# nlamprian/ICP

Hardware: AMD Instinct MI355X
Metric: ICP iterations/sec at |F|=|M|=16384, |R|=256 (higher is better)
Workload: dtype f32

## Files before the change

### icp_amd/__init__.py

```python
import ctypes as C
import os

import numpy as np

__all__ = ["ICP", "ICPStep", "ICPError", "Memory", "Quality", "Pairs", "PAIR", "ErrorMetric", "Normals", "ICPStepConfigT", "ICPStepConfigW",
           "PowerMode", "ReduceMode", "TransformKind", "ICPBatch", "batch_partition", "power_method", "KernelObject", "kernel_lms", "kernel_reps", "kernel_weights", "kernel_mean", "kernel_devs", "kernel_s", "ReduceScan", "lib", "lib_path", "reduce", "scan", "ReduceConfig", "synth_pair", "synth_cloud_vga", "punch_holes", "HOLES_SCATTERED", "HOLES_CONTIGUOUS", "synth_pair_scene", "SCENE_CURVED", "SCENE_WALL", "device_count", "DIST_ID"]

_HERE = os.path.dirname(os.path.abspath(__file__))
_SO = os.environ.get("ICP_AMD_LIB", os.path.join(_HERE, "libicp_amd.so"))

DIST_ID = np.dtype([("dist", np.float32), ("id", np.uint32)])


class ICPError(RuntimeError):
    def __init__(self, code, msg):
        super().__init__("icp_amd error %d: %s" % (code, msg))
        self.code = code


class ICPStepConfigT:
    EIGEN = 0
    POWER_METHOD = 1


# ... 46 lines not shown
    QUATERNION = 0
    QUATERNION_2 = 1
    MATRIX = 2


class Memory:
    F, M, T, TK, MEANS, S, NN_ID, W, SUM_W, REPS, RBC_N, RBC_O, RBC_PERM, RBC_OWNER, RBC_XP, RID, R, RK, NN, QT, TRIM, \
        NORMALS_F, PLANE_SYSTEM, COLOR_GRAD_F, NORMALS_M, UNIQUE, PAIR_FILTER, RECIPROCAL, REVERSE_ID = range(29)
    D_IN_F, D_IN_M, D_IO_T, H_IO_T = F, M, T, T


class _State(C.Structure):
    _fields_ = [("R", C.c_float * 9), ("q", C.c_float * 4), ("t", C.c_float * 3), ("s", C.c_float),
                ("Rk", C.c_float * 9), ("qk", C.c_float * 4), ("tk", C.c_float * 3), ("sk", C.c_float),
                ("k", C.c_uint32), ("converged", C.c_uint32), ("power_iterations", C.c_uint32),
                ("reserved", C.c_uint32)]


class Quality(C.Structure):
    _fields_ = [("fitness", C.c_double), ("inlier_rmse", C.c_double), ("sum_geo", C.c_double), ("information", C.c_double * 36),
                ("n", C.c_uint32), ("n_moving", C.c_uint32), ("n_inliers", C.c_uint32), ("reserved", C.c_uint32)]

    def information_matrix(self):
        return np.array(self.information, np.float64).reshape(6, 6)


class Pairs:
    EVALUATED = 0
    LAST_ITERATION = 1


PAIR = np.dtype([("moving", "<u4"), ("fixed", "<u4"), ("geo", "<f4"), ("weight", "<f4")])


class _Pair(C.Structure):
    _fields_ = [("moving", C.c_uint32), ("fixed", C.c_uint32), ("geo", C.c_float), ("weight", C.c_float)]


_lib = None


def lib_path():
    return _SO


def lib():
    global _lib
    if _lib is not None:
        return _lib
    if not os.path.exists(_SO):
        raise ICPError(-1, "%s not found: build it with `make` (hipcc --offload-arch=gfx950); "
                           "there is no CPU fallback" % _SO)
    L = C.CDLL(_SO)
    vp, u32, i32, f32, f64 = C.c_void_p, C.c_uint32, C.c_int, C.c_float, C.c_double

    def sig(name, res, *args):
        f = getattr(L, name, None)
        if f is None:
            if "ICP_AMD_LIB" in os.environ:
                return
            raise AttributeError("%s does not export %s" % (_SO, name))
        f.restype = res
        f.argtypes = list(args)

    sig("icp_create", i32, C.POINTER(vp), i32, i32, i32)
    sig("icp_destroy", i32, vp)
    sig("icp_init", i32, vp, u32, u32, f32, f32, u32, f64, f64)
    sig("icp_init_batched", i32, vp, u32, u32, u32, f32, f32, u32, f64, f64)
    sig("icp_write", i32, vp, i32, vp, i32)
    sig("icp_write_b", i32, vp, u32, i32, vp, i32)
    sig("icp_read", i32, vp, i32, vp, C.c_size_t)
    sig("icp_read_b", i32, vp, u32, i32, vp, C.c_size_t)
    sig("icp_mem_size", C.c_size_t, vp, i32)
    sig("icp_device_ptr", i32, vp, i32, C.POINTER(vp))
    sig("icp_adopt_device_buffer", i32, vp, i32, vp)
    sig("icp_build_rbc", i32, vp)
    sig("icp_step", i32, vp, i32)
    sig("icp_run", i32, vp, C.POINTER(u32))
    sig("icp_run_stats", i32, vp, C.POINTER(u32), C.POINTER(u32), C.POINTER(u32))
    sig("icp_set_run_depth", i32, vp, u32, i32)
    sig("icp_run_timeline", i32, vp, C.POINTER(f64))
    sig("icp_set_output_mode", i32, vp, i32)
    sig("icp_launch_stats", i32, vp, C.POINTER(f64), C.POINTER(C.c_uint64), C.POINTER(C.c_uint64), i32)
    sig("icp_run_fixed", i32, vp, u32)
    sig("icp_run_fixed_fresh", i32, vp, u32)
    sig("icp_sync", i32, vp)
    sig("icp_get_alpha", i32, vp, C.POINTER(f32))
    sig("icp_set_alpha", i32, vp, f32)
    sig("icp_get_scaling", i32, vp, C.POINTER(f32))
    sig("icp_set_scaling", i32, vp, f32)
    sig("icp_set_metric_scale", i32, vp, f32)
    sig("icp_get_metric_scale", i32, vp, C.POINTER(f32))
    sig("icp_set_rejection", i32, vp, i32, f32)
    sig("icp_get_rejection", i32, vp, C.POINTER(i32), C.POINTER(f32))
    sig("icp_set_trimming", i32, vp, f32)
    sig("icp_get_trimming", i32, vp, C.POINTER(f32))
    sig("icp_set_unique", i32, vp, i32)
    sig("icp_get_unique", i32, vp, C.POINTER(i32))
    sig("icp_set_reciprocal", i32, vp, i32, C.c_float)
    sig("icp_get_reciprocal", i32, vp, C.POINTER(i32), C.POINTER(C.c_float))
    sig("icp_set_normal_rejection", i32, vp, i32, f32)
    sig("icp_get_normal_rejection", i32, vp, C.POINTER(i32), C.POINTER(f32))
    sig("icp_set_boundary_rejection", i32, vp, u32)
    sig("icp_get_boundary_rejection", i32, vp, C.POINTER(u32))
    sig("icp_set_robust_loss", i32, vp, i32, f32)
    sig("icp_get_robust_loss", i32, vp, C.POINTER(i32), C.POINTER(f32))
    sig("icp_set_error_metric", i32, vp, i32, f32)
    sig("icp_get_error_metric", i32, vp, C.POINTER(i32), C.POINTER(f32))
    sig("icp_set_normals", i32, vp, i32, u32)
    sig("icp_get_normals", i32, vp, C.POINTER(i32), C.POINTER(u32))
    sig("icp_set_color_weight", i32, vp, f32)
    sig("icp_get_color_weight", i32, vp, C.POINTER(f32))
    sig("icp_set_plane_to_plane", i32, vp, f32)
    sig("icp_get_plane_to_plane", i32, vp, C.POINTER(f32))
    sig("icp_set_symmetric", i32, vp, i32)
    sig("icp_get_symmetric", i32, vp, C.POINTER(i32))
    sig("icp_get_max_iterations", i32, vp, C.POINTER(u32))
    sig("icp_set_max_iterations", i32, vp, u32)
    sig("icp_get_angle_threshold", i32, vp, C.POINTER(f64))
    sig("icp_set_angle_threshold", i32, vp, f64)
    sig("icp_get_translation_threshold", i32, vp, C.POINTER(f64))
    sig("icp_set_translation_threshold", i32, vp, f64)
    sig("icp_set_power_mode", i32, vp, i32)
    sig("icp_set_reduce_mode", i32, vp, i32)
    sig("icp_state", i32, vp, C.POINTER(_State))
    sig("icp_state_b", i32, vp, u32, C.POINTER(_State))
    sig("icp_evaluate", i32, vp, f32, C.POINTER(Quality), u32)
    sig("icp_batch_evaluate", i32, vp, u32, f32, C.POINTER(Quality))
    sig("icp_correspondences", i32, vp, i32, f32, C.POINTER(u32), u32)
    sig("icp_correspondences_read", i32, vp, u32, vp, u32, C.POINTER(u32))
    sig("icp_correspondences_device_ptr", i32, vp, u32, C.POINTER(vp), C.POINTER(vp))
    sig("icp_batch_correspondences", i32, vp, u32, i32, f32, vp, u32, C.POINTER(u32))
    sig("icp_write_cloud", i32, vp, i32, vp, i32)
    sig("icp_transform_cloud", i32, vp, vp, vp, u32)
    sig("icp_transform_cloud_ex", i32, vp, i32, vp, vp, vp, u32)
    sig("icp_track_next", i32, vp, vp, i32, C.POINTER(u32), C.POINTER(i32))
    sig("icp_track_reset", i32, vp)
    sig("icp_track_form", i32, vp, C.POINTER(i32))
    sig("icp_track_submit", i32, vp, vp, i32)
    sig("icp_track_collect", i32, vp, C.POINTER(u32), vp, C.POINTER(i32))
    sig("icp_track_staging", i32, vp, u32, C.POINTER(vp))
    sig("icp_batch_create", i32, C.POINTER(vp), C.POINTER(i32), i32, i32, i32)
    sig("icp_batch_destroy", i32, vp)
    sig("icp_batch_init", i32, vp, u32, u32, u32, f32, f32, u32, f64, f64)
    sig("icp_batch_set_modes", i32, vp, i32, i32)
    sig("icp_batch_set_rejection", i32, vp, i32, f32)
    sig("icp_batch_set_trimming", i32, vp, f32)
    sig("icp_batch_set_unique", i32, vp, i32)
    sig("icp_batch_set_reciprocal", i32, vp, i32, C.c_float)
    sig("icp_batch_set_normal_rejection", i32, vp, i32, f32)
    sig("icp_batch_set_boundary_rejection", i32, vp, u32)
    sig("icp_batch_set_robust_loss", i32, vp, i32, f32)
    sig("icp_batch_set_error_metric", i32, vp, i32, f32)
    sig("icp_batch_set_normals", i32, vp, i32, u32)
    sig("icp_batch_set_color_weight", i32, vp, f32)
    sig("icp_batch_set_plane_to_plane", i32, vp, f32)
    sig("icp_batch_set_symmetric", i32, vp, i32)
    sig("icp_batch_write", i32, vp, u32, i32, vp)
    sig("icp_batch_build_rbc", i32, vp)
    sig("icp_batch_run", i32, vp)
    sig("icp_batch_run_fixed", i32, vp, u32, i32)
    sig("icp_batch_state", i32, vp, u32, C.POINTER(_State))
    sig("icp_batch_read", i32, vp, u32, i32, vp, C.c_size_t)
    sig("icp_batch_size", i32, vp, C.POINTER(u32), C.POINTER(u32))
    sig("icp_batch_time_run_fixed", i32, vp, u32, u32, C.POINTER(f64))
    sig("icp_batch_time_run_fixed_slots", i32, vp, u32, u32, u32, C.POINTER(f64), vp)
# ... 668 lines not shown
            for k, name in enumerate(("search", "means", "sij", "finalize")):
                c = t[:, k] * 1e3
                print(" %-10s %10.2f %10.2f %10.2f %10.3f" % (name, c.mean(), c.min(), c.max(), c.sum() / 1e3))
            s = t.sum(1) * 1e3
            print(" %-10s %10.2f %10.2f %10.2f %10.3f" % ("step", s.mean(), s.min(), s.max(), s.sum() / 1e3))
        return t, tot.value

    def time_kernels(self, reps):
        out = (C.c_float * 4)()
        self._chk(self._L.icp_time_kernels(self._h, reps, out))
        return dict(zip(("search", "means", "sij", "finalize"), [float(v) for v in out]))

    def state(self, batch_index=0):
        st = _State()
        self._chk(self._L.icp_state_b(self._h, batch_index, C.byref(st)))
        return st

    def evaluate(self, max_dist=0.0, count=None):
        n = self.batch if count is None else int(count)
        out = (Quality * max(n, 1))()
        self._chk(self._L.icp_evaluate(self._h, _max_dist_arg(max_dist), out, n))
        return list(out)[:n]

    def correspondences(self, source=Pairs.EVALUATED, max_dist=0.0, batch_index=0):
        counts = (C.c_uint32 * self.batch)()
        self._chk(self._L.icp_correspondences(self._h, source, _max_dist_arg(max_dist), counts, self.batch))
        return self.correspondences_read(batch_index)

    def correspondences_read(self, batch_index=0):
        n = C.c_uint32()
        rc = self._L.icp_correspondences_read(self._h, batch_index, None, 0, C.byref(n))
        if rc and not (rc == 1 and n.value):
            self._chk(rc)
        out = np.empty(n.value, PAIR)
        if n.value:
            self._chk(self._L.icp_correspondences_read(self._h, batch_index, _p(out), n.value, C.byref(n)))
        return out

    def _vec(self, name, shape=None):
        a = np.array(getattr(self.state(), name), dtype=np.float32)
        return a.reshape(shape) if shape else a

    R = property(lambda s: s._vec("R", (3, 3)))
    Rk = property(lambda s: s._vec("Rk", (3, 3)))
    q = property(lambda s: s._vec("q"))
    qk = property(lambda s: s._vec("qk"))
    t = property(lambda s: s._vec("t"))
    tk = property(lambda s: s._vec("tk"))
    s = property(lambda s: float(s.state().s))
    sk = property(lambda s: float(s.state().sk))
    k = property(lambda s: int(s.state().k))


class ICP(ICPStep):

    def init(self, m, nr, a=1e2, c=1e-6, max_iterations=40, angle_threshold=0.001,
             translation_threshold=0.01, batch=1):
        self._max_it, self._ang, self._tra = max_iterations, angle_threshold, translation_threshold
        super().init(m, nr, a, c, batch)

    def run(self):
        k = C.c_uint32()
        self._chk(self._L.icp_run(self._h, C.byref(k)))
        return k.value

    def step(self, config=False):
        ICPStep.run(self, config)

    def run_stats(self):
        n, k, d = C.c_uint32(), C.c_uint32(), C.c_uint32()
        self._chk(self._L.icp_run_stats(self._h, C.byref(n), C.byref(k), C.byref(d)))
        return n.value, k.value, d.value

    def run_timeline(self):
        t = (C.c_double * 6)()
        self._chk(self._L.icp_run_timeline(self._h, t))
        return [float(x) for x in t]

    def launch_stats(self, reset=False):
        mx, slow, tot = C.c_double(), C.c_uint64(), C.c_uint64()
        self._chk(self._L.icp_launch_stats(self._h, C.byref(mx), C.byref(slow), C.byref(tot), int(reset)))
        return mx.value, slow.value, tot.value

    def set_output_mode(self, every_iteration=False):
        self._chk(self._L.icp_set_output_mode(self._h, int(every_iteration)))

    def set_run_depth(self, depth=3, adaptive=True):
        self._chk(self._L.icp_set_run_depth(self._h, depth, int(adaptive)))

    def getMaxIterations(self):
        v = C.c_uint32()
        self._chk(self._L.icp_get_max_iterations(self._h, C.byref(v)))
        return v.value

    def setMaxIterations(self, n):
        self._chk(self._L.icp_set_max_iterations(self._h, n))
        self._max_it = n

    def getAngleThreshold(self):
        v = C.c_double()
        self._chk(self._L.icp_get_angle_threshold(self._h, C.byref(v)))
        return v.value

    def setAngleThreshold(self, deg):
        self._chk(self._L.icp_set_angle_threshold(self._h, deg))
        self._ang = deg

    def getTranslationThreshold(self):
        v = C.c_double()
        self._chk(self._L.icp_get_translation_threshold(self._h, C.byref(v)))
        return v.value

    def setTranslationThreshold(self, mm):
        self._chk(self._L.icp_set_translation_threshold(self._h, mm))
        self._tra = mm


def batch_partition(registrations, n_slots, i):
    slot, idx, cnt = C.c_uint32(), C.c_uint32(), C.c_uint32()
    rc = lib().icp_batch_partition(registrations, n_slots, i, C.byref(slot), C.byref(idx), C.byref(cnt))
    if rc:
        raise ICPError(rc, "icp_batch_partition: bad arguments")
    return slot.value, idx.value, cnt.value


class ICPBatch:

    def __init__(self, devices, CR=ICPStepConfigT.POWER_METHOD, CW=ICPStepConfigW.WEIGHTED):
        self._L = lib()
        self._b = C.c_void_p()
        devs = (C.c_int * len(devices))(*devices)
        rc = self._L.icp_batch_create(C.byref(self._b), devs, len(devices), CR, CW)
        if rc:
            msg = self._L.icp_batch_last_error(None).decode()
            self._b = None
            raise ICPError(rc, msg)
        self.m = 0

    def _chk(self, rc):
        if rc:
            raise ICPError(rc, self._L.icp_batch_last_error(self._b).decode())

    def slot_cpus(self, slot):
        buf = C.create_string_buffer(16384)
        self._chk(self._L.icp_batch_slot_cpus(self._b, slot, buf, len(buf)))
        return [int(x) for x in buf.value.decode().split(",") if x]

    def close(self):
        if getattr(self, "_b", None):
            self._L.icp_batch_destroy(self._b)
            self._b = None

    def __del__(self):
        try:
            self.close()
        except Exception:
            pass

    def init(self, registrations, m, nr, a=1e2, c=1e-6, max_iterations=40, angle_threshold=0.001, translation_threshold=0.01):
        self._chk(self._L.icp_batch_init(self._b, registrations, m, nr, a, c, max_iterations, angle_threshold, translation_threshold))
        self.m, self.registrations = m, registrations

    def set_modes(self, reduce_mode, power_mode):
        self._chk(self._L.icp_batch_set_modes(self._b, reduce_mode, power_mode))

    def set_rejection(self, invalid=False, max_dist=None):
# ... 264 lines not shown
```

### icp_amd/csrc/icp_build.hip

```cpp
#include "icp_kernels.h"

static __device__ __forceinline__ void state_restart (icp_reg_state *st) { st->k = 0; st->done = 0; st->pm_iters = 0; }
static __device__ __forceinline__ void state_rotation_from (icp_reg_state *st, const float *T) { float R[9]; icp_quat_to_rot (T, R); for (int i = 0; i < 9; ++i) st->R[i] = R[i]; }

__global__ void k_reset_state (icp_params p, int reset_T)
{
    uint32_t b = blockIdx.x * blockDim.x + threadIdx.x;
    if (b >= p.batch) return;
    icp_reg_state *st = p.st + b;
    if (reset_T) {
        const float T0[8] = { 0, 0, 0, 1, 0, 0, 0, 1 };
        const float I3[9] = { 1, 0, 0, 0, 1, 0, 0, 0, 1 };
        for (int i = 0; i < 8; ++i) { st->T[i] = T0[i]; st->Tk[i] = T0[i]; }
        for (int i = 0; i < 9; ++i) { st->R[i] = I3[i]; st->Rk[i] = I3[i]; }
        for (int i = 0; i < 11; ++i) st->S[i] = 0.f;
        for (int i = 0; i < 8; ++i) st->means[i] = 0.f;
        st->sum_w = 0.0;
    }
    state_restart (st);
}

__global__ void k_set_T (icp_reg_state *st, const float *T8, int reset_k)
{
    if (threadIdx.x != 0) return;
// ... 672 lines not shown
{
    if (threadIdx.x != 0) return;
    bool open = false;
    for (uint32_t spin = 0; spin < max_spins && !open; ++spin) {
        const uint32_t v = __hip_atomic_load (seq, __ATOMIC_ACQUIRE, __HIP_MEMORY_SCOPE_AGENT);
        open = (int32_t) (v - want) >= 0;
        if (!open) __builtin_amdgcn_s_sleep (8);
    }
    if (!open) {
        if (run_flag) *run_flag = epoch;
        if (flag) __hip_atomic_store (flag, 1u, __ATOMIC_RELAXED, __HIP_MEMORY_SCOPE_SYSTEM);
        return;
    }
    if (warm) {
        state_restart (warm);
        float T[4]; for (int i = 0; i < 4; ++i) T[i] = warm->T[i];
        state_rotation_from (warm, T);
    }
}

void icp_launch_gate (const uint32_t *seq, uint32_t want, uint32_t *host_timeout_flag, hipStream_t s, uint32_t max_spins, icp_reg_state *warm, uint32_t *run_flag, uint32_t epoch)
{
    hipLaunchKernelGGL (k_gate, dim3 (1), dim3 (64), 0, s, seq, want, host_timeout_flag, max_spins, warm, run_flag, epoch);
}

__global__ void k_seq_set (uint32_t *seq, uint32_t v) { if (threadIdx.x == 0) __hip_atomic_store (seq, v, __ATOMIC_RELEASE, __HIP_MEMORY_SCOPE_AGENT); }
void icp_launch_seq_set (uint32_t *seq, uint32_t v, hipStream_t s) { hipLaunchKernelGGL (k_seq_set, dim3 (1), dim3 (64), 0, s, seq, v); }

void icp_launch_get_lms (const float *cloud, float *lms, hipStream_t s)
{
    hipLaunchKernelGGL (k_get_lms, dim3 (16384 * 2 / 256), dim3 (256), 0, s,
                        reinterpret_cast<const float4 *> (cloud), reinterpret_cast<float4 *> (lms));
}

void icp_launch_get_lms_band (const float *band, float *lms, hipStream_t s)
{
    hipLaunchKernelGGL (k_get_lms_band, dim3 (16384 * 2 / 256), dim3 (256), 0, s,
                        reinterpret_cast<const float4 *> (band), reinterpret_cast<float4 *> (lms));
}

void icp_launch_transform_cloud (const float *in, float *out, const icp_reg_state *st, uint32_t n, hipStream_t s)
{
    hipLaunchKernelGGL (k_transform_cloud, dim3 ((n + 255) / 256), dim3 (256), 0, s,
                        reinterpret_cast<const float4 *> (in), reinterpret_cast<float4 *> (out), st, n);
}

void icp_launch_transform_cloud_ex (int kind, const float *in, float *out, const float *T, uint32_t n, hipStream_t s)
{
    icp_T16 t {};
    for (int i = 0; i < (kind == 2 ? 16 : 8); ++i) t.v[i] = T[i];
    const float4 *i4 = reinterpret_cast<const float4 *> (in); float4 *o4 = reinterpret_cast<float4 *> (out);
    const dim3 grid ((n + 255) / 256), block (256);
    if (kind == 0) hipLaunchKernelGGL (k_transform_cloud_ex<0>, grid, block, 0, s, i4, o4, t, n);
    else if (kind == 1) hipLaunchKernelGGL (k_transform_cloud_ex<1>, grid, block, 0, s, i4, o4, t, n);
    else hipLaunchKernelGGL (k_transform_cloud_ex<2>, grid, block, 0, s, i4, o4, t, n);
}

static void build_rbc_lists (const icp_params &p, hipStream_t s)
{
    if (icp_build_lists (p)) {
        icp_launch_owner_search (p, s);
        hipLaunchKernelGGL (k_place_lists, dim3 ((p.nb + 3u) / 4u, p.batch), dim3 (256), 0, s, p);
        hipLaunchKernelGGL (k_list_boxes, dim3 (p.nr, p.batch), dim3 (256), 0, s, p);
        return;
    }
    {
        const uint32_t nbr = (p.nr + 63u) / 64u, nbg = (p.n16 + 63u) / 64u, nbt = p.nr > p.tbox ? p.n1k : 0u;
        const uint32_t nblk = (nbr + nbg + nbt + (nbr <= ICP_ORIGIN_SOLO ? 1u : 0u)) * p.batch;
        uint32_t sort_cap = 0u;
        if (p.nr >= 256u && nblk <= 2048u) { sort_cap = 256u; while (sort_cap < p.nr && sort_cap < ICP_OL_SORT_MAX) sort_cap <<= 1; }
        hipLaunchKernelGGL (k_reps_and_boxes, dim3 (nbr + nbg + nbt + (nbr <= ICP_ORIGIN_SOLO ? 1u : 0u), p.batch), dim3 (64), sort_cap * 20u, s, p, nbr, nbg, sort_cap);
    }
    icp_launch_owner_search (p, s);
    hipLaunchKernelGGL (k_chunk_hist, dim3 (p.nchunk, p.batch), dim3 (256), p.nr * sizeof (uint32_t), s, p);
    if (p.nr <= 1024u) hipLaunchKernelGGL (k_count_offsets, dim3 (1, p.batch), dim3 (1024), 0, s, p);
    else {
        hipLaunchKernelGGL (k_count, dim3 ((p.nr + 63) / 64, p.batch), dim3 (1024), 0, s, p);
        hipLaunchKernelGGL (k_offsets, dim3 (1, p.batch), dim3 (1024), 0, s, p);
    }
    hipLaunchKernelGGL (k_place, dim3 (p.nchunk, p.batch), dim3 (1024), 0, s, p);
    hipLaunchKernelGGL (k_list_boxes, dim3 (p.nr, p.batch), dim3 (256), 0, s, p);
}

void icp_launch_build_rbc (const icp_params &p, hipStream_t s)
{
    build_rbc_lists (p, s);
    if (p.nrm_grid) icp_launch_normals_grid (p, s);
}
```

### icp_amd/csrc/icp_capi.hip

```cpp
#include "icp_host.h"

using namespace icp_host;

namespace {

void free_all (icp_context *h)
{
    drop_graphs (h);
    for (void *q : h->dev_allocs) (void) hipFree (q);
    h->dev_allocs.clear ();
    if (h->hF) (void) hipHostFree (h->hF);
    if (h->hM) (void) hipHostFree (h->hM);
    if (h->hT) (void) hipHostFree (h->hT);
    if (h->hState) (void) hipHostFree (h->hState);
    if (h->hMirror) (void) hipHostFree (h->hMirror);
    if (h->hTrackMirror) (void) hipHostFree (h->hTrackMirror);
    h->hState = nullptr; h->hMirror = h->hTrackMirror = nullptr; h->hstate_fresh = false;
    h->run = run_ctl {}; h->track_k_hist[0] = h->track_k_hist[1] = 0; h->track_hist_frame = 0;
    if (h->dCloud) (void) hipFree (h->dCloud);
    if (h->dCloudOut) (void) hipFree (h->dCloudOut);
    h->hF = h->hM = h->hT = nullptr; h->dCloud = h->dCloudOut = nullptr; h->cloud_cap = 0;
    h->dF = h->dM = nullptr; h->ownF = h->ownM = true;
    h->quality = icp_context::quality_buffers {};
    h->pairs = icp_context::pairs_buffers {};
// ... 228 lines not shown
    *out = h;
    return ICP_OK;
}
ICP_CATCH_ALL

int icp_destroy (icp_handle h) try
{
    if (!h) return ICP_EINVAL;
    keeper_stop (h);
    (void) hipSetDevice (h->device);
    if (h->run.active || h->run2.active) (void) run_close_all (h);
    if (h->stream2) (void) hipStreamSynchronize (h->stream2);
    if (h->copy_stream) (void) hipStreamSynchronize (h->copy_stream);
    if (h->stream) (void) hipStreamSynchronize (h->stream);
    free_all (h);
    if (h->dTin) (void) hipFree (h->dTin);
    if (h->ev0) (void) hipEventDestroy (h->ev0);
    if (h->ev1) (void) hipEventDestroy (h->ev1);
    for (int k = 0; k < 2; ++k) if (h->evUp[k]) (void) hipEventDestroy (h->evUp[k]);
    for (int k = 0; k < 2; ++k) if (h->evFrame[k]) (void) hipEventDestroy (h->evFrame[k]);
    for (int k = 0; k < 4; ++k) if (h->evDone[k]) (void) hipEventDestroy (h->evDone[k]);
    for (int k = 0; k < 3; ++k) if (h->evStage[k]) (void) hipEventDestroy (h->evStage[k]);
    if (h->copy_stream) (void) hipStreamDestroy (h->copy_stream);
    if (h->stream2) (void) hipStreamDestroy (h->stream2);
    if (h->stream) (void) hipStreamDestroy (h->stream);
    delete h;
    return ICP_OK;
}
ICP_CATCH_ALL

int icp_init_batched (icp_handle h, uint32_t batch, uint32_t m, uint32_t nr, float a, float c,
                      uint32_t max_iterations, double angle_threshold, double translation_threshold) try
{
    api_guard guard_ (h);
    if (!h) return ICP_EINVAL;
    if (m == 0) return fail (h, ICP_EINVAL, "The sets of landmarks cannot have zero points");
    if (nr == 0) return fail (h, ICP_EINVAL, "The sets of representatives cannot have zero points");
    if (a == 0.f) return fail (h, ICP_EINVAL, "The alpha parameter cannot be equal to zero");
    if (m % 2) return fail (h, ICP_EINVAL, "The number of points in the array must be a multiple of 2");
    if (batch == 0 || batch > 65535u) return fail (h, ICP_EINVAL, "batch must be in [1, 65535]");
    if (max_iterations == 0) return fail (h, ICP_EINVAL, "max_iterations must be positive");
    uint32_t nrx, nry, side;
    if (!reps_grid (m, nr, &nrx, &nry, &side))
        return fail (h, ICP_EINVAL, "nr must be a power of two whose grid tiles the sqrt(m) x sqrt(m) landmark grid");
    if (nr > 32768u) return fail (h, ICP_EINVAL, "nr must be <= 32768");
    if (m > (1u << 20)) return fail (h, ICP_EINVAL, "m must be <= 2^20");
    int rc = set_device (h); if (rc) return rc;
    if ((rc = run_close_all (h))) return rc;
    if (h->copy_stream) HIPCHK (h, hipStreamSynchronize (h->copy_stream));
    if (h->stream2) HIPCHK (h, hipStreamSynchronize (h->stream2));
    if (h->stream) HIPCHK (h, hipStreamSynchronize (h->stream));
    free_all (h);
    icp_params &p = h->p;
    p = icp_params {};
    derive_params (h->opt, p);
    p.check = 0; p.emit = 1;
    p.m = m; p.nr = nr; p.batch = batch; p.side = side; p.nrx = nrx; p.nry = nry;
    p.a = a; p.c = c;
    {
        auto magic = [] (uint32_t d) { return d > 1u ? (uint32_t) ((1ull << 32) / d + 1ull) : 0u; };
        p.side_magic = magic (side); p.cellw_magic = magic (side / nrx); p.cellh_magic = magic (side / nry);
    }
    h->max_iterations = max_iterations; h->angle_threshold = angle_threshold; h->translation_threshold = translation_threshold;
    p.tan_half_thr = std::tan (angle_threshold * M_PI / 360.0);
    p.trans_thr = translation_threshold;
    p.nwg = (m + 127u) / 128u;
    p.nwp = p.nwg; if (p.nwp != 1 && (p.nwp % 4)) p.nwp += 4 - p.nwp % 4;
    uint32_t n4 = m; if (n4 % 4) n4 += 4 - n4 % 4;
    p.G = n4 / 4;
    p.nsp = (p.G + 511u) / 512u; if (p.nsp != 1 && (p.nsp % 4)) p.nsp += 4 - p.nsp % 4;
    p.nchunk = (m + ICP_CHUNK - 1) / ICP_CHUNK;
    p.nb = (m + 63u) / 64u;
    { const uint32_t ng = (p.nb + 127u) / 128u; p.ng_magic = ng > 1u ? (uint32_t) ((1ull << 32) / ng + 1ull) : 0u; }

    const size_t B = batch;
    float *F = nullptr, *M = nullptr;
    if ((rc = dalloc (h, &F, B * m * 8))) return rc;
    if ((rc = dalloc (h, &M, B * m * 8))) return rc;
    h->dF = F; h->dM = M; p.F = F; p.M = M; h->lm[0] = F; h->lm[1] = M;
    p.n16 = (nr + 15u) / 16u;
    p.tbox = icp_tbox_of (p); p.n1k = (nr + p.tbox - 1u) / p.tbox;
    p.s2wave = icp_s2_wave_of (p);
    { const char *e = std::getenv ("ICP_AMD_XCDMAP"); p.xcdmap = e ? (e[0] == '1') : (B == 1u); }
    { const char *e = std::getenv ("ICP_AMD_WARM_SEED"); p.warm_seed = (e && e[0] == '1') ? 1u : 0u; }
    p.gtile = 0u;
    if (nrx % 4u == 0u && nry % 4u == 0u && !std::getenv ("ICP_AMD_STRIP_GROUPS")) { uint32_t lg = 0; while ((4u << lg) < nrx) ++lg; p.gtile = lg + 1u; }
    p.nlb = m / 16u + 2u;
    {
        icp_rbc_set s;
        if ((rc = icp_rbc_for_each (s, p, [&] (const char *, void **q, size_t bytes) { return dalloc (h, reinterpret_cast<char **> (q), bytes); }))) return rc;
        icp_rbc_into (p, s);
    }
    if ((rc = dalloc (h, &p.rid, B * m))) return rc;
    if ((rc = dalloc (h, &p.nn_id, B * m))) return rc;
    if ((rc = dalloc (h, &p.PF, B * m))) return rc;
    if ((rc = dalloc (h, &p.PM, B * m))) return rc;
    if ((rc = dalloc (h, &p.wpart, B * 2 * p.nwp))) return rc;
    if ((rc = dalloc (h, &p.mpart, B * 2 * p.nwg))) return rc;
    if ((rc = dalloc (h, &p.mscr, B * 2 * ((p.nwg + 127u) / 128u)))) return rc;
    if ((rc = dalloc (h, &p.spart, B * 11 * p.nsp * 8))) return rc;
    if ((rc = dalloc (h, &p.mom, icp_mom_layout_of (batch, m, p.nb).total))) return rc;
    if ((rc = write_words (h, OPT_WORDS))) return rc;
    HIPCHK (h, hipMemsetAsync (icp_unique_claims (p), 0xFF, sizeof (unsigned long long) * B * m, h->stream));
    if ((rc = dalloc (h, &p.ml1, B * 18 * ((p.nb + 127u) / 128u)))) return rc;
    if ((rc = dalloc (h, &p.cst, B * 2))) return rc;
    if ((rc = dalloc (h, &p.st, B))) return rc;
    if ((rc = dalloc (h, &p.st_prev, B))) return rc;
    if (!h->dTin) HIPCHK (h, hipMalloc ((void **) &h->dTin, 8 * sizeof (float)));
    HIPCHK (h, hipHostMalloc ((void **) &h->hF, B * m * 8 * sizeof (float), hipHostMallocDefault));
    HIPCHK (h, hipHostMalloc ((void **) &h->hM, B * m * 8 * sizeof (float), hipHostMallocDefault));
    HIPCHK (h, hipHostMalloc ((void **) &h->hT, 64 * sizeof (float), hipHostMallocDefault));
    HIPCHK (h, hipHostMalloc ((void **) &h->hState, B * sizeof (icp_reg_state), hipHostMallocMapped | hipHostMallocCoherent));
    HIPCHK (h, hipHostMalloc ((void **) &h->hMirror, B * sizeof (unsigned long long), hipHostMallocMapped | hipHostMallocCoherent));
    std::memset (h->hMirror, 0, B * sizeof (unsigned long long));
    icp_launch_reset_state (p, h->stream, 1);
    HIPCHK (h, hipGetLastError ());
    HIPCHK (h, hipStreamSynchronize (h->stream));
    h->inited = true; h->built = false;
    return ICP_OK;
}
ICP_CATCH_ALL

int icp_init (icp_handle h, uint32_t m, uint32_t nr, float a, float c, uint32_t max_iterations,
              double angle_threshold, double translation_threshold) try
{
    api_guard guard_ (h);
    return icp_init_batched (h, 1, m, nr, a, c, max_iterations, angle_threshold, translation_threshold);
}
ICP_CATCH_ALL

struct mem_desc { const void *ptr; size_t bytes; const char *plain_write; };
static mem_desc mem_of (const icp_context *h, uint32_t b, int mem)
{
    const icp_params &p = h->p;
    const size_t m = p.m, nr = p.nr;
    const char *st = reinterpret_cast<const char *> (p.st + b);
    switch (mem) {
        case ICP_MEM_F: return { h->dF + b * m * 8, m * 32, nullptr };
        case ICP_MEM_M: return { h->dM + b * m * 8, m * 32, nullptr };
        case ICP_MEM_RBC_XP: return { p.XP + b * m * 8, m * 32, nullptr };
        case ICP_MEM_T: return { st + offsetof (icp_reg_state, T), 32, nullptr };
        case ICP_MEM_TK: return { st + offsetof (icp_reg_state, Tk), 32, nullptr };
        case ICP_MEM_MEANS: return { st + offsetof (icp_reg_state, means), 32, nullptr };
        case ICP_MEM_S: return { st + offsetof (icp_reg_state, S), 44, nullptr };
        case ICP_MEM_SUM_W: return { st + offsetof (icp_reg_state, sum_w), 8, nullptr };
        case ICP_MEM_R: return { st + offsetof (icp_reg_state, R), 36, nullptr };
        case ICP_MEM_RK: return { st + offsetof (icp_reg_state, Rk), 36, nullptr };
        case ICP_MEM_NN_ID: return { p.nn_id + b * m, m * 8, nullptr };
        case ICP_MEM_RBC_PERM: return { p.perm + b * m, m * 4, nullptr };
        case ICP_MEM_RBC_OWNER: return { p.owner + b * m, m * 4, nullptr };
        case ICP_MEM_RID: return { p.rid + b * m, m * 4, nullptr };
        case ICP_MEM_REPS: return { p.R + b * nr * 8, nr * 32, nullptr };
        case ICP_MEM_RBC_N: return { ICP_N_FULL (p, b), nr * 4, nullptr };
        case ICP_MEM_RBC_O: return { p.O + b * nr, nr * 4, nullptr };
        case ICP_MEM_NN: return { p.PF + b * m, m * 16, nullptr };
        case ICP_MEM_QT: return { p.PM + b * m, m * 16, nullptr };
        case ICP_MEM_W: return { reinterpret_cast<const float *> (p.PF + b * m) + 3, m * 4, nullptr };
        case ICP_MEM_TRIM: return { icp_trim_area (p) + 4u * b, 16, nullptr };
        case ICP_MEM_UNIQUE: return { icp_unique_area (p) + 2u * b, 8, nullptr };
        case ICP_MEM_PAIR_FILTER: return { icp_pair_filter_area (p) + 4u * b, 16, nullptr };
        case ICP_MEM_RECIPROCAL: return { icp_reciprocal_area (p) + 4u * b, 16, nullptr };
        case ICP_MEM_REVERSE_ID: return { h->recip.nn_id ? h->recip.nn_id + b * m : nullptr, m * 8, nullptr };
        case ICP_MEM_NORMALS_F: return { icp_normals_f (p) + b * m, m * 16, "ICP_MEM_NORMALS_F" };
        case ICP_MEM_COLOR_GRAD_F: return { icp_color_grad_f (p) + b * m, m * 16, "ICP_MEM_COLOR_GRAD_F" };
        case ICP_MEM_NORMALS_M: return { icp_normals_m (p) + b * m, m * 16, "ICP_MEM_NORMALS_M" };
        case ICP_MEM_PLANE_SYSTEM: return { icp_p2pl_area (p) + (size_t) ICP_P2PL_SYS * b, ICP_P2PL_SYS * sizeof (double), nullptr };
        default: return { nullptr, 0, nullptr };
    }
}

int icp_write_b (icp_handle h, uint32_t b, int mem, const void *host_ptr, int block) try
{
    api_guard guard_ (h);
    int rc = need (h, false); if (rc) return rc;
    if (b >= h->p.batch) return fail (h, ICP_EINVAL, "batch index out of range");
    if ((rc = set_device (h))) return rc;
// ... 7 lines not shown
            note_inputs_change (h);
            HIPCHK (h, hipEventSynchronize (ev));
            if (host_ptr) std::memcpy (stage, host_ptr, fm);
            HIPCHK (h, hipMemcpyAsync (dst, stage, fm, hipMemcpyHostToDevice, h->stream));
            HIPCHK (h, hipEventRecord (ev, h->stream));
            if (mem == ICP_MEM_M) { normals_m_follow (h, b, 1u); HIPCHK (h, hipGetLastError ()); }
            break;
        }
        case ICP_MEM_T: {
            HIPCHK (h, hipEventSynchronize (h->evStage[2]));
            if (host_ptr) std::memcpy (h->hT, host_ptr, 8 * sizeof (float));
            HIPCHK (h, hipMemcpyAsync (h->dTin, h->hT, 8 * sizeof (float), hipMemcpyHostToDevice, h->stream));
            HIPCHK (h, hipEventRecord (h->evStage[2], h->stream));
            { const long long kb = h->k_base; note_enqueue (h); h->k_base = kb; }
            icp_launch_set_T (h->p, b, h->dTin, h->stream);
            HIPCHK (h, hipGetLastError ());
            break;
        }
        default: {
            const mem_desc d = mem_of (h, b, mem);
            if (!d.plain_write)
                return fail (h, ICP_EINVAL, "icp_write: mem must be ICP_MEM_F, ICP_MEM_M, ICP_MEM_T, ICP_MEM_NORMALS_F, ICP_MEM_COLOR_GRAD_F or ICP_MEM_NORMALS_M");
            if (!host_ptr) return fail (h, ICP_EINVAL, std::string ("icp_write: ") + d.plain_write + " needs a source");
            note_inputs_change (h);
            HIPCHK (h, hipStreamSynchronize (h->stream));
            HIPCHK (h, hipMemcpy (const_cast<void *> (d.ptr), host_ptr, d.bytes, hipMemcpyHostToDevice));
        }
    }
    if (block) HIPCHK (h, hipStreamSynchronize (h->stream));
    return ICP_OK;
}
ICP_CATCH_ALL

int icp_write (icp_handle h, int mem, const void *host_ptr, int block) try { api_guard guard_ (h); return icp_write_b (h, 0, mem, host_ptr, block); } ICP_CATCH_ALL

size_t icp_mem_size (icp_handle h, int mem) { return h && h->inited ? mem_of (h, 0, mem).bytes : 0; }

int icp_read_b (icp_handle h, uint32_t b, int mem, void *host_dst, size_t bytes) try
{
    api_guard guard_ (h);
    int rc = need (h, false); if (rc) return rc;
    if (!host_dst) return fail (h, ICP_EINVAL, "icp_read: null destination");
    if (b >= h->p.batch) return fail (h, ICP_EINVAL, "batch index out of range");
    const mem_desc d = mem_of (h, b, mem);
    if (!d.bytes) return fail (h, ICP_EINVAL, "unknown icp_mem value");
    if (bytes > d.bytes) return fail (h, ICP_EINVAL, "icp_read: more bytes requested than the object holds");
    if (!d.ptr) return fail (h, ICP_ESTATE, "icp_read: ICP_MEM_REVERSE_ID: no back search has run since icp_init (icp_set_reciprocal)");
    if ((rc = set_device (h))) return rc;
    const void *src = d.ptr;
    if ((rc = materialize_outputs (h, mem))) return rc;
    if (mem == ICP_MEM_W) {
        size_t rows = bytes / 4;
        HIPCHK (h, hipMemcpy2DAsync (host_dst, 4, src, 16, 4, rows, hipMemcpyDeviceToHost, h->stream));
    } else
        HIPCHK (h, hipMemcpyAsync (host_dst, src, bytes, hipMemcpyDeviceToHost, h->stream));
    HIPCHK (h, hipStreamSynchronize (h->stream));
    return ICP_OK;
}
ICP_CATCH_ALL

int icp_read (icp_handle h, int mem, void *host_dst, size_t bytes) try { api_guard guard_ (h); return icp_read_b (h, 0, mem, host_dst, bytes); } ICP_CATCH_ALL

int icp_device_ptr (icp_handle h, int mem, void **dptr) try
{
    api_guard guard_ (h);
    int rc = need (h, false); if (rc) return rc;
    if (!dptr) return fail (h, ICP_EINVAL, "null pointer");
    const mem_desc d = mem_of (h, 0, mem);
    if (!d.bytes) return fail (h, ICP_EINVAL, "unknown icp_mem value");
    if (!d.ptr) return fail (h, ICP_ESTATE, "icp_device_ptr: ICP_MEM_REVERSE_ID: no back search has run since icp_init (icp_set_reciprocal)");
    if ((rc = set_device (h))) return rc;
    if ((rc = materialize_outputs (h, mem))) return rc;
    *dptr = const_cast<void *> (d.ptr);
    return ICP_OK;
}
ICP_CATCH_ALL

int icp_adopt_device_buffer (icp_handle h, int mem, void *dptr) try
{
    api_guard guard_ (h);
    int rc = need (h, false); if (rc) return rc;
    if (!dptr) return fail (h, ICP_EINVAL, "null pointer");
    if (mem == ICP_MEM_F) { h->dF = static_cast<float *> (dptr); h->p.F = h->dF; h->ownF = false; h->built = false; }
    else if (mem == ICP_MEM_M) { h->dM = static_cast<float *> (dptr); h->p.M = h->dM; h->ownM = false; h->recip.stale = true; }
    else return fail (h, ICP_EINVAL, "only ICP_MEM_F and ICP_MEM_M can be adopted");
    note_inputs_change (h);
    drop_graphs (h);
    return ICP_OK;
}
ICP_CATCH_ALL

int icp_build_rbc (icp_handle h) try
{
    api_guard guard_ (h);
    int rc = need (h, false); if (rc) return rc;
    if ((rc = set_device (h))) return rc;
    if (h->p.nrm_grid && h->p.m % h->p.nrm_grid)
        return fail (h, ICP_ESTATE, "icp_build_rbc: ICP_NORMALS_GRID: m is not a multiple of the grid width");
    if (h->opt.boundary_gw && h->p.m % h->opt.boundary_gw)
        return fail (h, ICP_ESTATE, "icp_build_rbc: icp_set_boundary_rejection: m is not a multiple of the grid width");
    note_inputs_change (h);
    note_enqueue (h);
    icp_launch_build_rbc (h->p, h->stream);
    HIPCHK (h, hipGetLastError ());
    h->built = true; h->k_base = 0;
    if (icp_reciprocal (h->p)) { h->recip.stale = true; if ((rc = reciprocal_ready (h))) return rc; }
    return ICP_OK;
}
ICP_CATCH_ALL

int icp_step (icp_handle h, int config) try
{
    api_guard guard_ (h);
    (void) config;
    int rc = need (h, true); if (rc) return rc;
    if ((rc = set_device (h))) return rc;
    icp_params p = h->p; p.check = 0; p.hmirror = nullptr; p.hstate = nullptr;
    { const long long kb = h->k_base; note_enqueue (h); if (kb >= 0) h->k_base = kb + 1; }
    note_outputs_stored (h);
    icp_launch_iteration (p, h->stream, &h->recip);
    HIPCHK (h, hipGetLastError ());
    return ICP_OK;
}
ICP_CATCH_ALL

int icp_run_fixed (icp_handle h, uint32_t iterations) try
{
    api_guard guard_ (h);
    int rc = need (h, true); if (rc) return rc;
    if (iterations == 0) return ICP_OK;
    if ((rc = set_device (h))) return rc;
    return launch_run (h, iterations, 0);
}
ICP_CATCH_ALL

int icp_run_fixed_fresh (icp_handle h, uint32_t iterations) try
{
    api_guard guard_ (h);
    int rc = need (h, true); if (rc) return rc;
    if (iterations == 0) return icp_reset_transform (h);
    if ((rc = set_device (h))) return rc;
    return launch_run (h, iterations, 0, true);
}
ICP_CATCH_ALL

int icp_run (icp_handle h, uint32_t *k) try
{
    api_guard guard_ (h);
    int rc = need (h, true); if (rc) return rc;
    if ((rc = set_device (h))) return rc;
    if (!h->run_adaptive) {
        if ((rc = launch_run (h, h->max_iterations, 1))) return rc;
        if ((rc = settle (h))) return rc;
        h->stat_launches = h->max_iterations; h->stat_k = h->hState[0].k; h->stat_dead = 0;
    } else {
        if ((rc = run_begin (h, h->run, h->stream, h->p, false, false, h->run_depth + 1u, h->hMirror, h->hState, -1))) return rc;
        if ((rc = run_finish (h))) return rc;
        if ((rc = run_wait_final (h, h->hMirror, h->p.batch, h->run.p.epoch))) return rc;
        h->stat_t[5] = now_s ();
        h->hstate_fresh = true; h->hstate_here = true;
        if (h->p.batch == 1u) h->k_base = h->hState[0].k;
        {
            uint32_t kmax = 0u, all_done = 1u;
            for (uint32_t b = 0; b < h->p.batch; ++b) { kmax = std::max (kmax, h->hState[b].k); all_done &= h->hState[b].done ? 1u : 0u; }
            h->stat_k = kmax;
            const uint32_t ran = kmax > h->run.k0 ? kmax - h->run.k0 : 0u;
            h->stat_dead = all_done ? h->run.enq - std::min (h->run.enq, ran + 1u) : 0u;
        }
    }
    if (k) {
        if (h->hstate_fresh) *k = h->hState[0].k;
        else {
            icp_reg_state st;
            HIPCHK (h, hipMemcpy (&st, h->p.st, sizeof st, hipMemcpyDeviceToHost));
            *k = st.k;
        }
    }
    return ICP_OK;
}
ICP_CATCH_ALL

int icp_run_stats (icp_handle h, uint32_t *launches, uint32_t *k, uint32_t *dead) try
{
    api_guard guard_ (h);
    if (!h) return ICP_EINVAL;
    if (launches) *launches = h->stat_launches;
    if (k) *k = h->stat_k;
    if (dead) *dead = h->stat_dead;
    return ICP_OK;
}
ICP_CATCH_ALL

int icp_launch_stats (icp_handle h, double *max_us, uint64_t *slower_than_10us, uint64_t *total, int reset) try
{
    api_guard guard_ (h);
    if (!h) return ICP_EINVAL;
    if (max_us) *max_us = h->stat_launch_max_us;
    if (slower_than_10us) *slower_than_10us = h->stat_launch_slow;
    if (total) *total = h->stat_launch_total;
    if (reset) { h->stat_launch_max_us = 0.0; h->stat_launch_slow = h->stat_launch_total = 0; }
    return ICP_OK;
}
ICP_CATCH_ALL

int icp_set_output_mode (icp_handle h, int mode) try
{
    api_guard guard_ (h);
    if (!h) return ICP_EINVAL;
    if (mode != ICP_OUTPUTS_LAZY && mode != ICP_OUTPUTS_EVERY_ITERATION) return fail (h, ICP_EINVAL, "unknown output mode");
    h->outputs_lazy = mode == ICP_OUTPUTS_LAZY;
    return ICP_OK;
}
ICP_CATCH_ALL

int icp_run_timeline (icp_handle h, double *us6) try
{
    api_guard guard_ (h);
    if (!h || !us6) return ICP_EINVAL;
    for (int i = 0; i < 6; ++i) us6[i] = (h->stat_t[i] - h->stat_t[0]) * 1e6;
    return ICP_OK;
}
ICP_CATCH_ALL

int icp_set_run_depth (icp_handle h, uint32_t depth, int adaptive) try
{
    api_guard guard_ (h);
    if (!h) return ICP_EINVAL;
    if (depth == 0 || depth > 64u) return fail (h, ICP_EINVAL, "icp_set_run_depth: depth must be in [1, 64]");
    { int rc = set_device (h); if (rc) return rc; if ((rc = run_close_all (h))) return rc; }
    h->run_depth = depth; h->run_adaptive = adaptive ? 1 : 0;
    return ICP_OK;
}
ICP_CATCH_ALL

int icp_sync (icp_handle h) try
{
    api_guard guard_ (h);
    if (!h) return ICP_EINVAL;
    int rc = set_device (h); if (rc) return rc;
    return settle (h);
}
ICP_CATCH_ALL

int icp_get_alpha (icp_handle h, float *a) try { api_guard guard_ (h); if (!h || !a) return ICP_EINVAL; *a = h->p.a; return ICP_OK; } ICP_CATCH_ALL
int icp_set_alpha (icp_handle h, float a) try
{
    api_guard guard_ (h);
    if (!h) return ICP_EINVAL;
    if (a == 0.f) return fail (h, ICP_EINVAL, "The alpha parameter cannot be equal to zero");
    { int rc = outputs_before_change (h); if (rc) return rc; }
    h->p.a = a; ++h->param_gen; return ICP_OK;
}
ICP_CATCH_ALL
int icp_set_metric_scale (icp_handle h, float f_g) try
{
    api_guard guard_ (h);
    if (!h) return ICP_EINVAL;
    if (!(f_g > 0.f) || !std::isfinite (f_g)) return fail (h, ICP_EINVAL, "the metric scale must be positive and finite");
    { int rc = outputs_before_change (h); if (rc) return rc; }
    h->opt.metric_scale = f_g;
    return commit (h, OPT_PARAMS);
}
ICP_CATCH_ALL
int icp_get_metric_scale (icp_handle h, float *f_g) try { api_guard guard_ (h); if (!h || !f_g) return ICP_EINVAL; *f_g = h->opt.metric_scale; return ICP_OK; } ICP_CATCH_ALL
int icp_set_rejection (icp_handle h, int flags, float max_dist) try
{
    api_guard guard_ (h);
    if (flags & ~reject_user_flags) return fail (h, ICP_EINVAL, "icp_set_rejection: unknown flag bits");
    if (!(max_dist >= 0.f)) return fail (h, ICP_EINVAL, "icp_set_rejection: max_dist must be >= 0 (0 or +inf: no distance test)");
    if (!h) return fail (h, ICP_EINVAL, "icp_set_rejection: null handle");
    { int rc = outputs_before_change (h); if (rc) return rc; }
    h->opt.reject_flags = flags; h->opt.reject_max_dist = max_dist;
    return commit (h, OPT_PARAMS);
}
ICP_CATCH_ALL
int icp_get_rejection (icp_handle h, int *flags, float *max_dist) try
{
    api_guard guard_ (h);
    if (!h) return ICP_EINVAL;
    if (flags) *flags = h->opt.reject_flags;
    if (max_dist) *max_dist = h->opt.reject_max_dist;
    return ICP_OK;
}
ICP_CATCH_ALL
int icp_set_trimming (icp_handle h, float keep_fraction) try
{
    api_guard guard_ (h);
// ... 233 lines not shown
    if (!h) return ICP_EINVAL;
    h->angle_threshold = d; h->p.tan_half_thr = std::tan (d * M_PI / 360.0); ++h->param_gen; return ICP_OK;
}
ICP_CATCH_ALL
int icp_get_translation_threshold (icp_handle h, double *d) try { api_guard guard_ (h); if (!h || !d) return ICP_EINVAL; *d = h->translation_threshold; return ICP_OK; } ICP_CATCH_ALL
int icp_set_translation_threshold (icp_handle h, double d) try
{
    api_guard guard_ (h);
    if (!h) return ICP_EINVAL;
    h->translation_threshold = d; h->p.trans_thr = d; ++h->param_gen; return ICP_OK;
}
ICP_CATCH_ALL
int icp_set_power_mode (icp_handle h, int mode) try
{
    api_guard guard_ (h);
    if (!h) return ICP_EINVAL;
    if (mode != ICP_POWER_LITERAL && mode != ICP_POWER_SQUARED) return fail (h, ICP_EINVAL, "unknown power mode");
    h->opt.power_mode = mode;
    return commit (h, OPT_PARAMS);
}
ICP_CATCH_ALL

int icp_set_reduce_mode (icp_handle h, int mode) try
{
    api_guard guard_ (h);
    if (!h) return ICP_EINVAL;
    if (mode != ICP_REDUCE_REFERENCE_ORDER && mode != ICP_REDUCE_FUSED) return fail (h, ICP_EINVAL, "unknown reduce mode");
    { int rc = outputs_before_change (h); if (rc) return rc; }
    h->opt.reduce_mode = mode;
    return commit (h, OPT_ROUTE);
}
ICP_CATCH_ALL

int icp_state_b (icp_handle h, uint32_t b, icp_state_t *out) try
{
    api_guard guard_ (h);
    int rc = need (h, false); if (rc) return rc;
    if (!out) return fail (h, ICP_EINVAL, "null pointer");
    if (b >= h->p.batch) return fail (h, ICP_EINVAL, "batch index out of range");
    if ((rc = set_device (h))) return rc;
    icp_reg_state st;
    if (h->hstate_fresh) {
        if (!h->hstate_here) HIPCHK (h, hipStreamSynchronize (h->stream));
        st = h->hState[b];
    } else {
        HIPCHK (h, hipMemcpyAsync (&st, h->p.st + b, sizeof st, hipMemcpyDeviceToHost, h->stream));
        HIPCHK (h, hipStreamSynchronize (h->stream));
    }
    std::memcpy (out->R, st.R, sizeof st.R); std::memcpy (out->Rk, st.Rk, sizeof st.Rk);
    std::memcpy (out->q, st.T, 16); std::memcpy (out->t, st.T + 4, 12); out->s = st.T[7];
    std::memcpy (out->qk, st.Tk, 16); std::memcpy (out->tk, st.Tk + 4, 12); out->sk = st.Tk[7];
    out->k = st.k; out->converged = st.done; out->power_iterations = st.pm_iters; out->reserved = 0;
    return ICP_OK;
}
ICP_CATCH_ALL

int icp_state (icp_handle h, icp_state_t *out) try { api_guard guard_ (h); return icp_state_b (h, 0, out); } ICP_CATCH_ALL

static int evaluation_ready (icp_context *h, const char *who, uint32_t count)
{
    const std::string w (who);
    if (count == 0) return fail (h, ICP_EINVAL, w + ": count must be at least 1");
    int rc = need (h, false); if (rc) return rc;
    if (count > h->p.batch) return fail (h, ICP_EINVAL, w + ": count is above the handle's batch");
    if (h->track_submitted) return fail (h, ICP_ESTATE, w + ": the handle has tracked frames (the quality of tracked frames is not provided): icp_init or icp_track_reset first");
    if (!h->built) return fail (h, ICP_ESTATE, "icp_build_rbc has not been called");
    return set_device (h);
}

static int evaluation_search (icp_context *h)
{
    const icp_params &p = h->p;
    const size_t n = (size_t) p.batch * p.m;
    icp_context::quality_buffers &Q = h->quality;
    int rc;
    if (!Q.nn_id && (rc = dalloc (h, &Q.nn_id, n))) return rc;
    if (!Q.PF && (rc = dalloc (h, &Q.PF, n))) return rc;
    if (!Q.PM && (rc = dalloc (h, &Q.PM, n))) return rc;
    if (!Q.rid && (rc = dalloc (h, &Q.rid, n))) return rc;
    icp_params q = p;
    q.check = 0; q.emit = 1; q.fused = 0; q.weighted = 0; q.hmirror = nullptr; q.hstate = nullptr; q.dbg = nullptr;
    q.reject = 0u; q.reject_d2 = 0.f; q.reject_max_dist = 0.f; q.trim_keep = 0.f; q.metric = ICP_METRIC_POINT_TO_POINT; q.p2pl_mu = 0.f; q.gicp = 0u;
    q.nn_id = Q.nn_id; q.PF = Q.PF; q.PM = Q.PM; q.rid = Q.rid;
    if (icp_dense (q)) HIPCHK (h, hipMemcpyAsync (Q.rid, p.rid, n * sizeof (uint32_t), hipMemcpyDeviceToDevice, h->stream));
    icp_launch_search (q, h->stream);
    return ICP_OK;
}

int icp_evaluate (icp_handle h, float max_dist, icp_quality_t *out, uint32_t count) try
{
    api_guard guard_ (h);
    if (!h) return ICP_EINVAL;
    if (!out) return fail (h, ICP_EINVAL, "icp_evaluate: null output");
    if (!(max_dist >= 0.f)) return fail (h, ICP_EINVAL, "icp_evaluate: max_dist must be >= 0 (0 or +inf: no distance test)");
    int rc = evaluation_ready (h, "icp_evaluate", count); if (rc) return rc;
    const icp_params &p = h->p;
    const size_t B = p.batch, nblk = icp_p2pl_nblk (p.m);
    icp_context::quality_buffers &Q = h->quality;
    if ((rc = evaluation_search (h))) return rc;
    if (!Q.part && (rc = dalloc (h, &Q.part, B * ICP_QUALITY_TERMS * nblk))) return rc;
    if (!Q.cnt && (rc = dalloc (h, &Q.cnt, B * 2 * nblk))) return rc;
    if (!Q.res && (rc = dalloc (h, &Q.res, B * ICP_QUALITY_RES))) return rc;
    const bool dist_on = max_dist > 0.f && !std::isinf (max_dist);
    icp_launch_quality (Q.PF, Q.PM, p.M, p.m, p.batch, dist_on, dist_on ? (float) ((double) max_dist * (double) max_dist) : 0.f, Q.part, Q.cnt, Q.res, h->stream);
    HIPCHK (h, hipGetLastError ());
    std::vector<double> res (B * ICP_QUALITY_RES);
    HIPCHK (h, hipMemcpyAsync (res.data (), Q.res, res.size () * sizeof (double), hipMemcpyDeviceToHost, h->stream));
    HIPCHK (h, hipStreamSynchronize (h->stream));
    for (uint32_t b = 0; b < count; ++b) {
        const double *r = res.data () + (size_t) b * ICP_QUALITY_RES;
        icp_quality_t &o = out[b];
        uint32_t c[2];
        std::memcpy (c, r + ICP_QUALITY_TERMS, sizeof c);
        o.n = p.m; o.n_moving = c[0]; o.n_inliers = c[1]; o.reserved = 0u;
        o.sum_geo = r[21];
        o.fitness = c[0] ? (double) c[1] / (double) c[0] : 0.0;
        o.inlier_rmse = c[1] ? std::sqrt (r[21] / (double) c[1]) : 0.0;
        int t = 0;
        for (int a = 0; a < 6; ++a)
            for (int cc = a; cc < 6; ++cc, ++t) { o.information[a * 6 + cc] = r[t]; o.information[cc * 6 + a] = r[t]; }
    }
    return ICP_OK;
}
ICP_CATCH_ALL

int icp_correspondences (icp_handle h, int source, float max_dist, uint32_t *counts, uint32_t count) try
{
    api_guard guard_ (h);
    if (!h) return ICP_EINVAL;
    if (source != ICP_PAIRS_EVALUATED && source != ICP_PAIRS_LAST_ITERATION) return fail (h, ICP_EINVAL, "icp_correspondences: unknown source");
    if (!counts) return fail (h, ICP_EINVAL, "icp_correspondences: null counts");
    if (!(max_dist >= 0.f)) return fail (h, ICP_EINVAL, "icp_correspondences: max_dist must be >= 0 (0 or +inf: no distance test)");
    if (source == ICP_PAIRS_LAST_ITERATION && max_dist != 0.f)
        return fail (h, ICP_EINVAL, "icp_correspondences: ICP_PAIRS_LAST_ITERATION takes the pairs the iteration used: max_dist must be 0");
    int rc = evaluation_ready (h, "icp_correspondences", count); if (rc) return rc;
    const icp_params &p = h->p;
    const size_t B = p.batch;
    icp_context::pairs_buffers &P = h->pairs;
    static_assert (sizeof (icp_pair_t) == sizeof (uint4) && sizeof (icp_pair_t) == 16, "a record is one 16-byte store");
    if (source == ICP_PAIRS_LAST_ITERATION && (rc = materialize_outputs (h, ICP_MEM_W))) return rc;
    if (!P.blk && (rc = dalloc (h, &P.blk, B * icp_p2pl_nblk (p.m)))) return rc;
    if (!P.rec && (rc = dalloc (h, &P.rec, B * p.m))) return rc;
    if (!P.count && (rc = dalloc (h, &P.count, B))) return rc;
    P.valid = false;
    if (source == ICP_PAIRS_EVALUATED) {
        if ((rc = evaluation_search (h))) return rc;
        const icp_context::quality_buffers &Q = h->quality;
        const bool dist_on = max_dist > 0.f && !std::isinf (max_dist);
        icp_launch_pairs (source, Q.PF, Q.PM, p.M, Q.nn_id, p.m, p.batch, dist_on, dist_on ? (float) ((double) max_dist * (double) max_dist) : 0.f, P.blk, P.rec, P.count, h->stream);
    } else
        icp_launch_pairs (source, p.PF, p.PM, nullptr, p.nn_id, p.m, p.batch, false, 0.f, P.blk, P.rec, P.count, h->stream);
    HIPCHK (h, hipGetLastError ());
    P.n.assign (B, 0u);
    HIPCHK (h, hipMemcpyAsync (P.n.data (), P.count, B * sizeof (uint32_t), hipMemcpyDeviceToHost, h->stream));
    HIPCHK (h, hipStreamSynchronize (h->stream));
    for (uint32_t b = 0; b < count; ++b) counts[b] = P.n[b];
    P.valid = true;
    return ICP_OK;
}
ICP_CATCH_ALL

int icp_correspondences_read (icp_handle h, uint32_t b, icp_pair_t *host_dst, uint32_t capacity, uint32_t *n) try
{
    api_guard guard_ (h);
    int rc = need (h, false); if (rc) return rc;
    if (b >= h->p.batch) return fail (h, ICP_EINVAL, "batch index out of range");
// ... 288 lines not shown
```

### icp_amd/csrc/icp_host.h

```cpp
#pragma once

#include "../../include/icp_amd.h"
#include "icp_kernels.h"
#include "icp_rbc_set.h"
#include "icp_cguard.h"

#include <atomic>
#include <thread>
#include <mutex>
#include <condition_variable>
#include <chrono>
#include <cmath>
#include <cstdio>
#include <cstdlib>
#include <cstring>
#include <map>
#include <string>
#include <vector>
#include <immintrin.h>

namespace icp_host __attribute__ ((visibility ("hidden"))) {

inline thread_local std::string g_create_error;

// ... 8 lines not shown
    bool end_enqueued = false;
    volatile unsigned long long *mirror = nullptr;
    int track_slot = -1;
    hipStream_t stream = nullptr;
    double t[5] = { 0, 0, 0, 0, 0 };
    double launch_max_us = 0.0; uint32_t launch_slow = 0;
};

struct track_keeper {
    std::thread th;
    std::mutex mx;
    std::condition_variable cv;
    std::atomic<int> state { 0 };
    std::atomic<bool> pause { false }, quit { false };
    bool started = false;
    std::thread::id tid;
    int rc = 0; std::string err;
};
constexpr int ICP_KEEPER_ABORTED = -77;

inline double now_s () { return std::chrono::duration<double> (std::chrono::steady_clock::now ().time_since_epoch ()).count (); }

struct icp_options {
    int rot = ICP_ROT_POWER_METHOD, weighted = 1, power_mode = ICP_POWER_SQUARED, reduce_mode = ICP_REDUCE_FUSED;
    int chain = 1;
    float metric_scale = 1.f;
    int reject_flags = 0; float reject_max_dist = 0.f;
    float trim_keep = 1.f;
    bool unique = false;
    bool reciprocal = false; float reciprocal_gap = 0.f;
    bool normal_on = false; float normal_min_cos = 0.f;
    uint32_t boundary_gw = 0;
    int robust = ICP_ROBUST_NONE; float robust_scale = 0.f;
    int metric = ICP_METRIC_POINT_TO_POINT; float p2pl_mu = 0.f;
    float color_kappa = 0.f;
    float gicp_eps = 0.f;
    bool symmetric = false;
    uint32_t nrm_grid = 0;
};

}

struct icp_context {
    int device = 0;
    hipStream_t stream = nullptr;
    bool inited = false, built = false;
    icp_params p {};
    uint32_t max_iterations = 40;
    double angle_threshold = 0.001, translation_threshold = 0.01;
    std::string err;
    std::vector<void *> dev_allocs;
    float *dF = nullptr, *dM = nullptr;
    bool ownF = true, ownM = true;
    float *hF = nullptr, *hM = nullptr, *hT = nullptr;
    icp_reg_state *hState = nullptr;
    bool hstate_fresh = false;
    bool hstate_here = false;
    unsigned long long *hMirror = nullptr;
    uint32_t epoch = 0;
    long long k_base = 0;
    uint32_t run_depth = 3;
    int run_adaptive = 1;
    icp_host::run_ctl run;
    icp_host::run_ctl run2;
    int api_depth = 0;
    icp_host::track_keeper *keeper = nullptr;
    int outputs_lazy = 1;
    bool outputs_stale = false, outputs_lost = false;
    uint32_t stat_launches = 0, stat_k = 0, stat_dead = 0;
    double stat_t[6] = { 0, 0, 0, 0, 0, 0 };
    double stat_launch_max_us = 0.0; uint64_t stat_launch_slow = 0, stat_launch_total = 0;
    icp_host::icp_options opt;
    uint64_t graph_clock = 0, param_gen = 0;
    float *dTin = nullptr;
    struct quality_buffers {
        icp_dist_id *nn_id = nullptr; float4 *PF = nullptr, *PM = nullptr; uint32_t *rid = nullptr;
        double *part = nullptr; uint32_t *cnt = nullptr; double *res = nullptr;
    } quality;
    struct pairs_buffers {
        uint32_t *blk = nullptr; uint4 *rec = nullptr; uint32_t *count = nullptr;
        std::vector<uint32_t> n; bool valid = false;
    } pairs;
    icp_reciprocal_set recip;
    float *dCloud = nullptr, *dCloudOut = nullptr; uint32_t cloud_cap = 0;
    std::map<uint64_t, icp_host::graph_entry> graphs;
    uint32_t parity = 0;
    float *lm[3] = { nullptr, nullptr, nullptr };
    float *hBand[2] = { nullptr, nullptr }, *dBand[2] = { nullptr, nullptr };
    float *hFrame[2] = { nullptr, nullptr };
    struct host_range { const char *base; size_t bytes; };
    std::vector<host_range> sources;
    icp_reg_state *hTrack = nullptr;
    unsigned long long *hTrackMirror = nullptr;
    uint32_t track_epoch[4] = { 0, 0, 0, 0 };
    uint32_t track_k_hist[2] = { 0, 0 };
    uint64_t track_hist_frame = 0;
    hipStream_t copy_stream = nullptr;
    hipStream_t stream2 = nullptr;
    int track_gate = 1;
    uint32_t *dSeq = nullptr, *dRunFlag = nullptr, *hGateFlag = nullptr;
    bool stream2_dirty = false;
    icp_rbc_set rbc[2];
    bool rbc2_ready = false;
    bool track_last_gated = false;
    hipEvent_t evUp[2] = { nullptr, nullptr }, evDone[4] = { nullptr, nullptr, nullptr, nullptr };
    hipEvent_t evFrame[2] = { nullptr, nullptr };
    hipEvent_t evStage[3] = { nullptr, nullptr, nullptr };
    uint64_t track_submitted = 0, track_collected = 0;
    hipEvent_t ev0 = nullptr, ev1 = nullptr;
};

namespace icp_host __attribute__ ((visibility ("hidden"))) {

inline int fail (icp_context *h, int code, const std::string &msg)
{
    if (h) h->err = msg; else g_create_error = msg;
    return code;
}

#define HIPCHK(h, expr)                                                                         \
    do {                                                                                        \
        hipError_t e_ = (expr);                                                                 \
        if (e_ != hipSuccess)                                                                   \
            return fail ((h), ICP_EHIP, std::string (#expr) + ": " + hipGetErrorString (e_));   \
    } while (0)

template <typename T>
int dalloc (icp_context *h, T **ptr, size_t count, bool zero = true)
{
    void *q = nullptr;
    size_t bytes = (count ? count : 1) * sizeof (T);
    hipError_t e = hipMalloc (&q, bytes);
    if (e != hipSuccess) return fail (h, ICP_ENOMEM, std::string ("hipMalloc: ") + hipGetErrorString (e));
    h->dev_allocs.push_back (q);
    if (zero) {
        e = hipMemsetAsync (q, 0, bytes, h->stream);
        if (e != hipSuccess) return fail (h, ICP_EHIP, std::string ("hipMemsetAsync: ") + hipGetErrorString (e));
    }
    *ptr = static_cast<T *> (q);
    return ICP_OK;
}

void drop_graphs (icp_context *h);
int need (icp_context *h, bool built, bool keep_run = false);
int set_device (icp_context *h);
int get_graph (icp_context *h, uint32_t iterations, int check, hipGraphExec_t *out, bool fresh = false, bool with_build = false);
void run_launch_one (icp_context *h, run_ctl &r);
void run_enqueue_end (icp_context *h, run_ctl &r);
bool run_pump (icp_context *h, run_ctl &r);
int run_finish (icp_context *h, run_ctl &r, run_ctl *other);
inline int run_finish (icp_context *h) { return run_finish (h, h->run, h->run2.active ? &h->run2 : nullptr); }
int run_wait_final (icp_context *h, volatile unsigned long long *mirror, uint32_t n, uint32_t epoch, bool tracked = false);
int run_close_all (icp_context *h);
inline bool on_keeper_thread (const icp_context *h) { return h->keeper && h->keeper->started && std::this_thread::get_id () == h->keeper->tid; }
void keeper_quiesce (icp_context *h);
void keeper_kick (icp_context *h);
void keeper_stop (icp_context *h);
struct api_guard {
    icp_context *h;
    explicit api_guard (icp_context *h_) : h (h_) { if (h && h->api_depth++ == 0 && h->keeper) keeper_quiesce (h); }
    ~api_guard () { if (h && --h->api_depth == 0 && h->keeper) keeper_kick (h); }
    api_guard (const api_guard &) = delete; api_guard &operator= (const api_guard &) = delete;
};
int launch_run (icp_context *h, uint32_t iterations, int check, bool fresh = false, bool with_build = false);
int settle (icp_context *h);
void note_enqueue (icp_context *h);
void note_inputs_change (icp_context *h);
void note_outputs_stored (icp_context *h);
int materialize_outputs (icp_context *h, int mem);
void normals_m_follow (icp_context *h, uint32_t b0, uint32_t nb);
int reciprocal_ready (icp_context *h);

template <typename Fn>
int capture_graph (icp_context *h, Fn &&launches, graph_entry *out, bool instantiate = true)
{
    graph_entry ge;
    HIPCHK (h, hipStreamBeginCapture (h->stream, hipStreamCaptureModeThreadLocal));
    launches ();
    const hipError_t le = hipGetLastError ();
    hipError_t e = hipStreamEndCapture (h->stream, &ge.graph);
    if (e == hipSuccess && le != hipSuccess) e = le;
    if (e != hipSuccess) {
        if (ge.graph) (void) hipGraphDestroy (ge.graph);
        return fail (h, ICP_EHIP, std::string ("graph capture: ") + hipGetErrorString (e));
    }
    if (instantiate) {
        e = hipGraphInstantiate (&ge.exec, ge.graph, nullptr, nullptr, 0);
        if (e != hipSuccess) {
            (void) hipGraphDestroy (ge.graph);
            return fail (h, ICP_EHIP, std::string ("hipGraphInstantiate: ") + hipGetErrorString (e));
        }
    }
    *out = ge;
    return ICP_OK;
}

struct run_no_hook { int operator() () const { return ICP_OK; } };
template <typename BETWEEN = run_no_hook>
int run_begin (icp_context *h, run_ctl &r, hipStream_t stream, const icp_params &p, bool fresh, bool with_build, uint32_t blind,
               unsigned long long *mirror, icp_reg_state *hstate, int track_slot, BETWEEN between = BETWEEN (), run_ctl *other = nullptr)
{
    r = run_ctl {};
    r.stream = stream;
    r.t[0] = now_s ();
    r.p = p; r.p.check = 1;
    const icp_route route = icp_route_of (p);
    r.p.emit = (h->outputs_lazy && p.fused && !route.stored) ? 0 : 1;
    h->outputs_stale = r.p.emit == 0; h->outputs_lost = false;
    if (++h->epoch == 0u) h->epoch = 1u;
    r.p.epoch = h->epoch; r.p.hmirror = mirror; r.p.hstate = hstate;
    r.mirror = mirror; r.track_slot = track_slot;
    for (uint32_t b = 0; b < p.batch; ++b) mirror[b] = 0ull;
    std::atomic_thread_fence (std::memory_order_seq_cst);
    r.chained = route.chained; r.fresh = fresh;
    r.k0 = (fresh || with_build || h->k_base < 0) ? 0u : (uint32_t) h->k_base;
    r.maxit = h->max_iterations; r.depth = h->run_depth ? h->run_depth : 1u;
    if (other && other->active) (void) run_pump (h, *other);
    if (with_build) icp_launch_build_rbc (r.p, r.stream);
    if (other && other->active) (void) run_pump (h, *other);
    { int rc = between (); if (rc) return rc; }
    if (fresh && !r.chained) icp_launch_reset_state (r.p, r.stream, 1);
    r.active = true;
    const uint32_t n = std::min (std::max (blind, 1u), r.maxit);
    while (r.enq < n) {
        run_launch_one (h, r);
        if (other && other->active && (r.enq & 1u) == 0u) (void) run_pump (h, *other);
    }
    if (r.enq >= r.maxit) { r.decided = true; r.k_final = r.maxit + r.k0; run_enqueue_end (h, r); }
    HIPCHK (h, hipGetLastError ());
    h->hstate_fresh = false; h->hstate_here = false; h->k_base = -1;
    r.t[1] = now_s ();
    return ICP_OK;
}

}
```

### icp_amd/csrc/icp_kernels.h

```cpp
#pragma once
#include <hip/hip_runtime.h>
#include <stdint.h>
#include "icp_device.h"
#include "icp_search_select.h"

#ifndef ICP_L1_MIN_GROUPS
#define ICP_L1_MIN_GROUPS 2u
#endif
#define ICP_BAND_ROW0 49u
#define ICP_BAND_ROW_STEP 3u
#define ICP_BAND_ROWS 128u
#define ICP_BAND_COL0 65u
#define ICP_BAND_COLS 509u
#define ICP_BAND_ROW_BYTES (ICP_BAND_COLS * 32u)
#define ICP_BAND_BYTES ((size_t) ICP_BAND_ROWS * ICP_BAND_ROW_BYTES)
#define ICP_TBOX 1024u
#ifndef ICP_OL_BOXED_MIN
#define ICP_OL_BOXED_MIN 128u
#endif
#define ICP_OL_MASKS(nr) ((nr) + 1u + 2u * (((nr) + 7u) / 8u))
#define ICP_OL_STRIDE(nr) (ICP_OL_MASKS (nr) + ((nr) + 127u) / 128u)
#define ICP_CHUNK 1024u

struct icp_params {
    uint32_t m, nr, batch;
    uint32_t side, nrx, nry;
    uint32_t ng_magic;
    uint32_t side_magic, cellw_magic, cellh_magic;
    float a, c;
    float dist_scale;
    int weighted, rot, power_mode, check;
    int chain;
    int fused;
    int emit;
    double tan_half_thr, trans_thr;
    uint32_t nwg;
    uint32_t nwp;
    uint32_t G;
    uint32_t nsp;
    uint32_t nchunk;
    uint32_t nb;
    const float *F, *M;
    float *R;
    float4 *GB;
    uint32_t n16, n1k;
    uint32_t tbox;
    uint32_t gtile;
    uint32_t xcdmap;
    uint32_t warm_seed;
    uint32_t s2wave;
    uint32_t nrm_grid;
    float *XP;
    float *XQ;
    float4 *OL;
    float4 *LB;
    uint32_t nlb;
    uint32_t metric;
    uint32_t *rep_src, *owner, *N, *O, *perm, *chunk_hist;
    uint2 *blist; uint32_t *bn; uint8_t *brank;
    uint32_t *rid;
    icp_dist_id *nn_id;
    float4 *PF, *PM;
    float *wpart;
    float4 *mpart;
    float4 *mscr;
    float *spart;
    double *mom;
    double *ml1;
    icp_reg_state *cst;
    uint32_t slot;
    float p2pl_mu;
    icp_reg_state *st;
    icp_reg_state *st_prev;
    unsigned long long *dbg;
    unsigned long long *hmirror;
    icp_reg_state *hstate;
    uint32_t epoch;
    uint32_t gicp;
    uint32_t *run_flag;
    uint32_t *track_seq;
    uint32_t seq_value;
    uint32_t no_state_reset;
    uint32_t reject;
    float reject_d2;
    float reject_max_dist;
    float trim_keep;
};
#define ICP_REJECT_DIST_ON 0x80000000u
#define ICP_REJECT_TRIM_ON 0x40000000u
#define ICP_REJECT_ROBUST_SHIFT 28u
#define ICP_REJECT_ROBUST_MASK 0x30000000u
#define ICP_REJECT_UNIQUE_ON 0x08000000u
#define ICP_REJECT_BOUNDARY_ON 0x04000000u
#define ICP_REJECT_NORMAL_ON 0x02000000u
#define ICP_REJECT_FILTER_MASK (ICP_REJECT_BOUNDARY_ON | ICP_REJECT_NORMAL_ON)
#define ICP_REJECT_RECIPROCAL_ON 0x01000000u
static_assert (sizeof (icp_params) == 480, "icp_params grew: the hidden kernel arguments of every kernel would move");

static __host__ __device__ __forceinline__ bool icp_rejecting (const icp_params &p) { return p.reject != 0u; }
static __host__ __device__ __forceinline__ bool icp_trimming (const icp_params &p) { return (p.reject & ICP_REJECT_TRIM_ON) != 0u; }
static __host__ __device__ __forceinline__ bool icp_unique (const icp_params &p) { return (p.reject & ICP_REJECT_UNIQUE_ON) != 0u; }
static __host__ __device__ __forceinline__ bool icp_pair_filter (const icp_params &p) { return (p.reject & ICP_REJECT_FILTER_MASK) != 0u; }
static __host__ __device__ __forceinline__ bool icp_reciprocal (const icp_params &p) { return (p.reject & ICP_REJECT_RECIPROCAL_ON) != 0u; }
static __host__ __device__ __forceinline__ bool icp_moving_normals (const icp_params &p) { return p.gicp != 0u || (p.reject & ICP_REJECT_NORMAL_ON) != 0u; }
static __host__ __device__ __forceinline__ uint32_t icp_robust (const icp_params &p) { return (p.reject & ICP_REJECT_ROBUST_MASK) >> ICP_REJECT_ROBUST_SHIFT; }
static __host__ __device__ __forceinline__ double icp_robust_omega (uint32_t loss, double u)
{
    if (u != u) return 0.0;
    if (loss == 1u) return u <= 1.0 ? 1.0 : 1.0 / sqrt (u);
    if (loss == 2u) return 1.0 / (1.0 + u);
    return u < 1.0 ? (1.0 - u) * (1.0 - u) : 0.0;
}
#define ICP_TRIM_ONE_BLOCK_MAX 16384u
#define ICP_TRIM_BINS 2048u

#define ICP_P2PL_BLOCK 256u
#define ICP_P2PL_TERMS 27u
#define ICP_P2PL_SYS 28u
#define ICP_METRIC_COLORED_ 2u
static __host__ __device__ __forceinline__ bool icp_p2pl (const icp_params &p) { return p.metric != 0u; }
static __host__ __device__ __forceinline__ bool icp_colored (const icp_params &p) { return p.metric == ICP_METRIC_COLORED_; }
static __host__ __device__ __forceinline__ bool icp_gicp (const icp_params &p) { return p.gicp == 1u && p.metric == 1u; }
#define ICP_MOVING_NORMALS_SYM 2u
static __host__ __device__ __forceinline__ bool icp_sym (const icp_params &p) { return p.gicp == ICP_MOVING_NORMALS_SYM && p.metric == 1u; }
static __host__ __device__ __forceinline__ uint32_t icp_p2pl_nblk (uint32_t m) { return (m + ICP_P2PL_BLOCK - 1u) / ICP_P2PL_BLOCK; }

#define ICP_QUALITY_TERMS 22u
#define ICP_QUALITY_RES 24u

struct icp_mom_layout {
    size_t trim;
    size_t sys;
    size_t part;
    size_t kappa;
    size_t robust;
    size_t gicp;
    size_t uniq;
    size_t filt;
    size_t recip;
    size_t total;
};
static __host__ __device__ inline icp_mom_layout icp_mom_layout_of (uint32_t batch, uint32_t m, uint32_t nb)
{
    const size_t B = batch, trim_words = B * (8u + ICP_TRIM_BINS) + (m > ICP_TRIM_ONE_BLOCK_MAX ? B * m : 0u);
    icp_mom_layout l;
    l.trim = B * 2 * 18 * nb;
    l.sys = l.trim + (trim_words + 1u) / 2u;
    l.part = l.sys + B * ICP_P2PL_SYS;
    l.kappa = l.part + B * ICP_P2PL_TERMS * icp_p2pl_nblk (m);
    l.robust = l.kappa + 1u;
    l.gicp = l.robust + 1u;
    l.uniq = l.gicp + 1u;
    l.filt = l.uniq + B + B * m;
    l.recip = l.filt + 6u * B + 1u;
    l.total = l.recip + 2u * B + 1u;
    return l;
}
static __host__ __device__ inline icp_mom_layout icp_mom_layout_of (const icp_params &p) { return icp_mom_layout_of (p.batch, p.m, p.nb); }
static inline uint32_t *icp_trim_area (const icp_params &p) { return reinterpret_cast<uint32_t *> (p.mom + icp_mom_layout_of (p).trim); }
static inline double *icp_p2pl_area (const icp_params &p) { return p.mom + icp_mom_layout_of (p).sys; }
static inline double *icp_p2pl_part (const icp_params &p) { return p.mom + icp_mom_layout_of (p).part; }
static inline float *icp_color_kappa (const icp_params &p) { return reinterpret_cast<float *> (p.mom + icp_mom_layout_of (p).kappa); }
static __host__ __device__ inline float *icp_robust_scale (const icp_params &p) { return reinterpret_cast<float *> (p.mom + icp_mom_layout_of (p).robust); }
static __host__ __device__ inline float *icp_gicp_eps (const icp_params &p) { return reinterpret_cast<float *> (p.mom + icp_mom_layout_of (p).gicp); }
static inline uint32_t *icp_unique_area (const icp_params &p) { return reinterpret_cast<uint32_t *> (p.mom + icp_mom_layout_of (p).uniq); }
static inline unsigned long long *icp_unique_claims (const icp_params &p)
{
    return reinterpret_cast<unsigned long long *> (p.mom + icp_mom_layout_of (p).uniq + (size_t) p.batch);
}
static inline uint32_t *icp_pair_filter_area (const icp_params &p) { return reinterpret_cast<uint32_t *> (p.mom + icp_mom_layout_of (p).filt); }
static inline uint32_t *icp_pair_filter_counts (const icp_params &p) { return icp_pair_filter_area (p) + 4u * (size_t) p.batch; }
static inline uint32_t *icp_pair_filter_settings (const icp_params &p) { return icp_pair_filter_area (p) + 12u * (size_t) p.batch; }
static inline uint32_t *icp_reciprocal_area (const icp_params &p) { return reinterpret_cast<uint32_t *> (p.mom + icp_mom_layout_of (p).recip); }
static inline uint32_t *icp_reciprocal_gap (const icp_params &p) { return icp_reciprocal_area (p) + 4u * (size_t) p.batch; }

struct icp_xp_layout {
    size_t normals, color_grad, normals_m, total;
};
static __host__ __device__ __forceinline__ icp_xp_layout icp_xp_layout_of (uint32_t batch, uint32_t m)
{
    const size_t n = (size_t) batch * m;
    return { n * 8, n * 12, n * 16, n * 20 };
}
static __host__ __device__ __forceinline__ float4 *icp_normals_f (const icp_params &p)
{
    return reinterpret_cast<float4 *> (p.XP + icp_xp_layout_of (p.batch, p.m).normals);
}
static __host__ __device__ __forceinline__ float4 *icp_color_grad_f (const icp_params &p)
{
    return reinterpret_cast<float4 *> (p.XP + icp_xp_layout_of (p.batch, p.m).color_grad);
}
static __host__ __device__ __forceinline__ float4 *icp_normals_m (const icp_params &p)
{
    return reinterpret_cast<float4 *> (p.XP + icp_xp_layout_of (p.batch, p.m).normals_m);
}

#define ICP_N_FULL(p, b) ((p).N + ((size_t) (p).batch + (b)) * (p).nr)

#define ICP_MIRROR_FINAL (1ull << 30)
#define ICP_MIRROR_DONE (1ull << 31)
#define ICP_MIRROR_WORD(epoch, k, done) (((unsigned long long) (epoch) << 32) | ((done) ? ICP_MIRROR_DONE : 0ull) | (unsigned long long) ((k) & 0xFFFFFFu))

static __device__ __forceinline__ uint32_t rep_src_index (const icp_params &p, uint32_t r)
{
    uint32_t gX = r % p.nrx, gY = r / p.nrx;
    uint32_t stepX = p.side / p.nrx, stepY = p.side / p.nry;
    uint32_t xi = (stepX == 1) ? gX : gX * stepX + (stepX >> 1) - 1;
    uint32_t yi = (stepY == 1) ? gY : gY * stepY + (stepY >> 1) - 1;
    return yi * p.side + xi;
}

struct rep_src_map {
    uint32_t nrx, side, stepX, stepY, offX, offY, lgx;
    __device__ __forceinline__ explicit rep_src_map (const icp_params &p)
        : nrx (p.nrx), side (p.side), stepX (p.side / p.nrx), stepY (p.side / p.nry), lgx (31u - (uint32_t) __builtin_clz (p.nrx | 1u))
    {
        offX = (stepX == 1u) ? 0u : (stepX >> 1) - 1u; offY = (stepY == 1u) ? 0u : (stepY >> 1) - 1u;
    }
    __device__ __forceinline__ uint32_t operator() (uint32_t r) const
    {
        return ((r >> lgx) * stepY + offY) * side + (r & (nrx - 1u)) * stepX + offX;
    }
};


static __device__ __forceinline__ uint32_t icp_other_kind_near (const unsigned long long *MK, uint32_t nr, uint32_t r, bool r_at_origin, uint32_t fallback)
{
    const uint32_t nw = (nr + 63u) / 64u, w = r >> 6, l = r & 63u;
    auto other = [&] (uint32_t ww) -> unsigned long long {
        const uint32_t left = nr - 64u * ww;
        const unsigned long long m = MK[ww];
        return (r_at_origin ? ~m : m) & (left < 64u ? (1ull << left) - 1ull : ~0ull);
    };
    const unsigned long long o = other (w), below = o & ((1ull << l) - 1ull), above = l < 63u ? o & ~((2ull << l) - 1ull) : 0ull;
    uint32_t best_d = 0xFFFFFFFFu, best = fallback;
    if (below) { const uint32_t q = 63u - (uint32_t) __builtin_clzll (below); best_d = l - q; best = 64u * w + q; }
    if (above) { const uint32_t q = (uint32_t) __builtin_ctzll (above); if (q - l < best_d) { best_d = q - l; best = 64u * w + q; } }
    if (best_d != 0xFFFFFFFFu) return best;
    for (uint32_t d = 1; d <= 4u; ++d) {
        if (w >= d) { const unsigned long long ol = other (w - d); if (ol) return 64u * (w - d) + 63u - (uint32_t) __builtin_clzll (ol); }
        if (w + d < nw) { const unsigned long long orr = other (w + d); if (orr) return 64u * (w + d) + (uint32_t) __builtin_ctzll (orr); }
    }
    return fallback;
}

enum icp_apply_kind { ICP_APPLY_NONE = 0, ICP_APPLY_PLAIN, ICP_APPLY_ROBUST };
enum icp_tail_kind { ICP_TAIL_FUSED = 0, ICP_TAIL_FUSED_L1, ICP_TAIL_REFERENCE, ICP_TAIL_PLANE };
struct icp_route {
    bool chained;
    bool stored;
    bool ref_search;
    bool filter;
    bool reciprocal;
    bool unique;
    uint32_t select;
    icp_apply_kind apply;
    icp_tail_kind tail;
    uint32_t launches;
};
icp_route icp_route_of (const icp_params &p);

void icp_launch_build_rbc (const icp_params &p, hipStream_t s);
void icp_launch_search (const icp_params &p, hipStream_t s);
struct icp_reciprocal_set;
void icp_launch_iteration (const icp_params &p, hipStream_t s, const icp_reciprocal_set *rs = nullptr);
void icp_launch_masked (const icp_params &p, hipStream_t s, unsigned mask, const icp_reciprocal_set *rs = nullptr);
void icp_launch_chain (const icp_params &p, hipStream_t s, uint32_t iterations, bool fresh = false);
void icp_launch_chain_one (const icp_params &p, hipStream_t s, uint32_t j, bool fresh, bool emit);
void icp_launch_chain_end (const icp_params &p, hipStream_t s, uint32_t launches);
void icp_launch_publish_state (const icp_params &p, hipStream_t s);
bool icp_build_lists (const icp_params &p);
bool icp_dense (const icp_params &p);
uint32_t icp_dense_tile (const icp_params &p);
void icp_launch_owner_search (const icp_params &p, hipStream_t s);
void icp_launch_search_dense (const icp_params &p, hipStream_t s);
void icp_launch_search_rej (const icp_params &p, hipStream_t s);
void icp_launch_chain_one_rej (const icp_params &p, hipStream_t s, uint32_t j, bool fresh, bool emit);
void icp_launch_trim_select (const icp_params &p, hipStream_t s, uint32_t launches);
void icp_launch_trim_apply (const icp_params &p, hipStream_t s);
void icp_launch_unique (const icp_params &p, hipStream_t s);
void icp_launch_reciprocal (const icp_params &p, hipStream_t s, const icp_reciprocal_set *rs);
void icp_launch_reciprocal_build (const icp_params &p, hipStream_t s, const icp_reciprocal_set &rs);
void icp_launch_pair_filter (const icp_params &p, hipStream_t s);
void icp_launch_robust_apply (const icp_params &p, hipStream_t s);
void icp_launch_plane_moments_robust (const icp_params &p, hipStream_t s, double *part, uint32_t nblk);
void icp_launch_p2pl_solve (const icp_params &p, hipStream_t s);
void icp_launch_normals_grid (const icp_params &p, hipStream_t s);
void icp_launch_normals_m (const icp_params &p, hipStream_t s, uint32_t b0, uint32_t nb);
void icp_launch_gicp_moments (const icp_params &p, hipStream_t s, double *part, uint32_t nblk);
void icp_launch_sym_moments (const icp_params &p, hipStream_t s, double *part, uint32_t nblk);
void icp_launch_owner_search_dense (const icp_params &p, hipStream_t s);
void icp_launch_quality (const float4 *PF, const float4 *PM, const float *M, uint32_t m, uint32_t batch, bool dist_on, float d2, double *part, uint32_t *cnt,
                         double *res, hipStream_t s);
void icp_launch_pairs (int source, const float4 *PF, const float4 *PM, const float *M, const icp_dist_id *nn_id, uint32_t m, uint32_t batch, bool dist_on, float d2,
                       uint32_t *blk_cnt, uint4 *pairs, uint32_t *count, hipStream_t s);
uint32_t icp_tbox_of (const icp_params &p);
uint32_t icp_s2_wave_of (const icp_params &p);
void icp_search_layout_of (const icp_params &p, int *dense, int *tile, int *stage2);
void icp_launch_reset_state (const icp_params &p, hipStream_t s, int reset_T);
void icp_launch_set_T (const icp_params &p, uint32_t b, const float *dT8, hipStream_t s, int reset_k = 0);
void icp_launch_gate (const uint32_t *seq, uint32_t want, uint32_t *host_timeout_flag, hipStream_t s, uint32_t max_spins = 1u << 21, icp_reg_state *warm = nullptr,
                      uint32_t *run_flag = nullptr, uint32_t epoch = 0u);
void icp_launch_seq_set (uint32_t *seq, uint32_t v, hipStream_t s);
void icp_launch_rotation_solver (int rot, int power_mode, const float *din19, float *dout18, hipStream_t s);
void icp_launch_get_lms (const float *cloud, float *lms, hipStream_t s);
void icp_launch_get_lms_band (const float *band, float *lms, hipStream_t s);
void icp_launch_transform_cloud (const float *in, float *out, const icp_reg_state *st, uint32_t n, hipStream_t s);
void icp_launch_transform_cloud_ex (int kind, const float *in, float *out, const float *T, uint32_t n, hipStream_t s);
```

### icp_amd/csrc/icp_reciprocal.hip

```cpp
#include "icp_rbc_set.h"
#include <cstdio>
#include <cstdlib>

namespace {

constexpr uint32_t RECIPROCAL_BLOCK = 256u;

#define RECIPROCAL_GUARD reserved1

__global__ __launch_bounds__ (64) void k_reciprocal_state (icp_params p, icp_reg_state *rst, uint32_t *result)
{
    const uint32_t b = blockIdx.x, t = threadIdx.x;
    const icp_reg_state *st = p.st + b;
    icp_reg_state *out = rst + b;
    constexpr uint32_t T0 = offsetof (icp_reg_state, T) / 4u, G0 = offsetof (icp_reg_state, RECIPROCAL_GUARD) / 4u;
    if (t < sizeof (icp_reg_state) / 4u && !(t >= T0 && t < T0 + 8u) && t != G0)
        reinterpret_cast<uint32_t *> (out)[t] = reinterpret_cast<const uint32_t *> (st)[t];
    if (t != 0u) return;
    if (!(p.check && st->done)) { uint32_t *w = result + 4u * b; w[0] = 0u; w[1] = 0u; w[2] = 0u; w[3] = 0u; }
    const double x = (double) st->T[0], y = (double) st->T[1], z = (double) st->T[2], w = (double) st->T[3];
    const double tx = (double) st->T[4], ty = (double) st->T[5], tz = (double) st->T[6];
    const float s = st->T[7];
    const double xx = x * x, yy = y * y, zz = z * z, xy = x * y, xz = x * z, yz = y * z, wx = w * x, wy = w * y, wz = w * z;
    const double R00 = 1.0 - 2.0 * (yy + zz), R01 = 2.0 * (xy - wz), R02 = 2.0 * (xz + wy);
    const double R10 = 2.0 * (xy + wz), R11 = 1.0 - 2.0 * (xx + zz), R12 = 2.0 * (yz - wx);
    const double R20 = 2.0 * (xz - wy), R21 = 2.0 * (yz + wx), R22 = 1.0 - 2.0 * (xx + yy);
    const double si = 1.0 / (double) s;
    const double u0 = (R00 * tx + R10 * ty) + R20 * tz, u1 = (R01 * tx + R11 * ty) + R21 * tz, u2 = (R02 * tx + R12 * ty) + R22 * tz;
    float Ti[8] = { -st->T[0], -st->T[1], -st->T[2], st->T[3], (float) -(u0 * si), (float) -(u1 * si), (float) -(u2 * si), (float) si };
    bool ok = isfinite (s) && s > 0.f;
#pragma unroll
    for (int k = 0; k < 8; ++k) ok = ok && isfinite (Ti[k]);
    if (!ok) { Ti[0] = Ti[1] = Ti[2] = 0.f; Ti[3] = 1.f; Ti[4] = Ti[5] = Ti[6] = 0.f; Ti[7] = 1.f; }
#pragma unroll
    for (int k = 0; k < 8; ++k) out->T[k] = Ti[k];
    out->RECIPROCAL_GUARD = ok ? 0u : 1u;
}

__global__ __launch_bounds__ (RECIPROCAL_BLOCK) void k_reciprocal (icp_params p, const icp_dist_id *rev, const icp_reg_state *rst, uint32_t *result,
                                                                   const uint32_t *gap)
{
    __shared__ uint32_t s_cnt[RECIPROCAL_BLOCK / 64u][3];
    const uint32_t b = blockIdx.y, t = threadIdx.x, i = blockIdx.x * RECIPROCAL_BLOCK + t;
    if (p.check && p.st[b].done) return;
    const float max_gap = __uint_as_float (gap[0]);
    const float gap2 = (float) ((double) max_gap * (double) max_gap);
    const bool guard = rst[b].RECIPROCAL_GUARD != 0u;
    bool cand = false, exact = false, near = false;
    if (i < p.m) {
        const size_t o = (size_t) b * p.m, e = o + i;
        const uint32_t j = p.nn_id[e].id;
        cand = p.PF[e].w != 0.f && j < p.m;
        if (cand) {
            if (!guard) {
                const uint32_t i2 = rev[o + j].id;
                exact = i2 == i;
                if (!exact && max_gap > 0.f && i2 < p.m) {
                    const float4 a = p.PM[e], c = p.PM[o + i2];
                    const float gx = a.x - c.x, gy = a.y - c.y, gz = a.z - c.z;
                    const float g = (gx * gx + gy * gy) + gz * gz;
                    near = isfinite (g) && g <= gap2;
                }
            }
            if (!exact && !near) reinterpret_cast<float *> (p.PF + e)[3] = 0.f;
        }
    }
    const uint32_t wn = (uint32_t) __popcll (__ballot (cand)), we = (uint32_t) __popcll (__ballot (exact)), wr = (uint32_t) __popcll (__ballot (near));
    if ((t & 63u) == 0u) { s_cnt[t >> 6][0] = wn; s_cnt[t >> 6][1] = we; s_cnt[t >> 6][2] = wr; }
    __syncthreads ();
    if (t == 0u) {
        uint32_t sn = 0u, se = 0u, sr = 0u;
#pragma unroll
        for (uint32_t v = 0; v < RECIPROCAL_BLOCK / 64u; ++v) { sn += s_cnt[v][0]; se += s_cnt[v][1]; sr += s_cnt[v][2]; }
        uint32_t *out = result + 4u * b;
        if (sn) __hip_atomic_fetch_add (out + 0, sn, __ATOMIC_RELAXED, __HIP_MEMORY_SCOPE_AGENT);
        if (se) __hip_atomic_fetch_add (out + 1, se, __ATOMIC_RELAXED, __HIP_MEMORY_SCOPE_AGENT);
        if (sr) __hip_atomic_fetch_add (out + 2, sr, __ATOMIC_RELAXED, __HIP_MEMORY_SCOPE_AGENT);
        if (se + sr) __hip_atomic_fetch_add (out + 3, se + sr, __ATOMIC_RELAXED, __HIP_MEMORY_SCOPE_AGENT);
    }
}

icp_params reciprocal_params (const icp_params &p, const icp_reciprocal_set &rs)
{
    icp_params q = p;
    q.F = p.M; q.M = p.F;
    icp_rbc_into (q, rs.rbc);
    q.st = rs.st; q.nn_id = rs.nn_id; q.PF = rs.PF; q.PM = rs.PM; q.rid = rs.rid;
    q.fused = 0; q.weighted = 0; q.emit = 1; q.hmirror = nullptr; q.hstate = nullptr; q.dbg = nullptr;
    q.reject = 0u; q.reject_d2 = 0.f; q.reject_max_dist = 0.f; q.trim_keep = 0.f; q.metric = 0u; q.p2pl_mu = 0.f; q.gicp = 0u; q.nrm_grid = 0u;
    q.run_flag = nullptr; q.track_seq = nullptr;
    return q;
}

}

void icp_launch_reciprocal_build (const icp_params &p, hipStream_t s, const icp_reciprocal_set &rs)
{
    icp_params q = reciprocal_params (p, rs);
    q.check = 0; q.no_state_reset = 1u;
    icp_launch_build_rbc (q, s);
}

void icp_launch_reciprocal (const icp_params &p, hipStream_t s, const icp_reciprocal_set *rs)
{
    if (!rs || !rs->st) {
        std::fprintf (stderr, "icp_amd: reciprocal correspondences are on and the launch has no moving set\n");
        std::abort ();
    }
    hipLaunchKernelGGL (k_reciprocal_state, dim3 (p.batch), dim3 (64), 0, s, p, rs->st, icp_reciprocal_area (p));
    icp_launch_search (reciprocal_params (p, *rs), s);
    const dim3 grid ((p.m + RECIPROCAL_BLOCK - 1u) / RECIPROCAL_BLOCK, p.batch);
    hipLaunchKernelGGL (k_reciprocal, grid, dim3 (RECIPROCAL_BLOCK), 0, s, p, (const icp_dist_id *) rs->nn_id, (const icp_reg_state *) rs->st,
                        icp_reciprocal_area (p), (const uint32_t *) icp_reciprocal_gap (p));
}
```

### icp_amd/csrc/icp_run.hip

```cpp
#include "icp_host.h"

namespace icp_host {

void drop_graphs (icp_context *h)
{
    for (auto &kv : h->graphs) {
        if (kv.second.exec) (void) hipGraphExecDestroy (kv.second.exec);
        if (kv.second.graph) (void) hipGraphDestroy (kv.second.graph);
    }
    h->graphs.clear ();
}

int need (icp_context *h, bool built, bool keep_run)
{
    if (!h) return ICP_EINVAL;
    if (!h->inited) return fail (h, ICP_ESTATE, "icp_init has not been called");
    if (built && !h->built) return fail (h, ICP_ESTATE, "icp_build_rbc has not been called");
    if (built && h->opt.gicp_eps > 0.f && icp_colored (h->p))
        return fail (h, ICP_ESTATE, "icp_set_plane_to_plane does not combine with ICP_METRIC_COLORED (icp_set_error_metric): switch one of them off");
    if (built && h->opt.symmetric && icp_colored (h->p))
        return fail (h, ICP_ESTATE, "icp_set_symmetric does not combine with ICP_METRIC_COLORED (icp_set_error_metric): switch one of them off");
    if (built && h->opt.symmetric && h->opt.gicp_eps > 0.f && icp_p2pl (h->p))
        return fail (h, ICP_ESTATE, "icp_set_symmetric does not combine with icp_set_plane_to_plane: switch one of them off");
    if (!keep_run && (h->run.active || h->run2.active || h->stream2_dirty)) {
        if (hipSetDevice (h->device) != hipSuccess) return fail (h, ICP_EHIP, "hipSetDevice");
        int rc = run_close_all (h); if (rc) return rc;
    }
    if (built && !keep_run && icp_reciprocal (h->p)) return reciprocal_ready (h);
    return ICP_OK;
}

int set_device (icp_context *h)
{
    HIPCHK (h, hipSetDevice (h->device));
    return ICP_OK;
}

#define ICP_GRAPH_CACHE 8u

static hipError_t enqueue_fixed_run (icp_context *h, uint32_t iterations, int check, bool fresh, bool with_build)
{
    icp_params p = h->p;
    p.check = check; p.hmirror = nullptr; p.hstate = nullptr;
    if (with_build) icp_launch_build_rbc (p, h->stream);
    if (icp_route_of (p).chained) icp_launch_chain (p, h->stream, iterations, fresh);
    else {
        if (fresh) icp_launch_reset_state (p, h->stream, 1);
        for (uint32_t k = 0; k < iterations; ++k) {
            p.emit = (check || k + 1 == iterations) ? 1 : 0;
            icp_launch_iteration (p, h->stream, &h->recip);
        }
    }
    return check ? hipMemcpyAsync (h->hState, p.st, sizeof (icp_reg_state) * p.batch, hipMemcpyDeviceToHost, h->stream) : hipSuccess;
}

int get_graph (icp_context *h, uint32_t iterations, int check, hipGraphExec_t *out, bool fresh, bool with_build)
{
    uint64_t key = ((uint64_t) iterations << 3) | (uint64_t) (check ? 4 : 0) | (uint64_t) h->parity | ((uint64_t) (fresh ? 1 : 0) << 62) | ((uint64_t) (with_build ? 1 : 0) << 61);
    auto it = h->graphs.find (key);
    if (it != h->graphs.end () && it->second.gen == h->param_gen) { it->second.used = ++h->graph_clock; *out = it->second.exec; return ICP_OK; }
    auto launches = [&] { (void) enqueue_fixed_run (h, iterations, check, fresh, with_build); };
    if (it != h->graphs.end ()) {
        graph_entry ng;
        int rc = capture_graph (h, launches, &ng, false);
        if (rc) return rc;
        hipGraphNode_t bad = nullptr; hipGraphExecUpdateResult res = hipGraphExecUpdateSuccess;
        hipError_t e = hipGraphExecUpdate (it->second.exec, ng.graph, &bad, &res);
        if (e != hipSuccess || res != hipGraphExecUpdateSuccess) {
            (void) hipGetLastError ();
            (void) hipGraphExecDestroy (it->second.exec); it->second.exec = nullptr;
            e = hipGraphInstantiate (&it->second.exec, ng.graph, nullptr, nullptr, 0);
            if (e != hipSuccess) {
                (void) hipGraphDestroy (ng.graph); (void) hipGraphDestroy (it->second.graph);
                h->graphs.erase (it);
                return fail (h, ICP_EHIP, std::string ("hipGraphInstantiate: ") + hipGetErrorString (e));
            }
        }
        (void) hipGraphDestroy (it->second.graph);
        it->second.graph = ng.graph; it->second.gen = h->param_gen; it->second.used = ++h->graph_clock;
        *out = it->second.exec;
        return ICP_OK;
    }
    graph_entry ge;
    int rc = capture_graph (h, launches, &ge);
    if (rc) return rc;
    ge.gen = h->param_gen; ge.used = ++h->graph_clock;
    if (h->graphs.size () >= ICP_GRAPH_CACHE) {
        auto lru = h->graphs.begin ();
        for (auto jt = h->graphs.begin (); jt != h->graphs.end (); ++jt) if (jt->second.used < lru->second.used) lru = jt;
        if (lru->second.exec) (void) hipGraphExecDestroy (lru->second.exec);
        if (lru->second.graph) (void) hipGraphDestroy (lru->second.graph);
        h->graphs.erase (lru);
    }
    h->graphs[key] = ge;
    *out = ge.exec;
    return ICP_OK;
}


void run_launch_one (icp_context *h, run_ctl &r)
{
    const double t0 = now_s ();
    if (r.chained) icp_launch_chain_one (r.p, r.stream, r.enq, r.fresh, r.p.emit != 0);
    else icp_launch_iteration (r.p, r.stream, &h->recip);
    const double us = (now_s () - t0) * 1e6;
    if (us > r.launch_max_us) r.launch_max_us = us;
    if (us > 10.0) ++r.launch_slow;
    ++r.enq;
}

void run_enqueue_end (icp_context *h, run_ctl &r)
{
    (void) h;
    if (r.end_enqueued || r.final_seen) return;
    if (r.chained) icp_launch_chain_end (r.p, r.stream, r.enq);
    else icp_launch_publish_state (r.p, r.stream);
    r.end_enqueued = true;
}

bool run_pump (icp_context *h, run_ctl &r)
{
    if (r.decided) return true;
    uint32_t kmin = 0xFFFFFFFFu, kmax = 0u; bool all_done = true, all_final = true;
    for (uint32_t b = 0; b < r.p.batch; ++b) {
        const unsigned long long w = r.mirror[b];
        const bool mine = (uint32_t) (w >> 32) == r.p.epoch;
        const uint32_t kabs = mine ? (uint32_t) (w & 0xFFFFFFull) : 0u, k = kabs > r.k0 ? kabs - r.k0 : 0u;
// ... 10 lines not shown
    return r.decided;
}

int run_finish (icp_context *h, run_ctl &r, run_ctl *other)
{
    if (!r.active) return ICP_OK;
    uint32_t spins = 0, k_last = 0xFFFFFFFFu;
    auto t_last = std::chrono::steady_clock::now ();
    while (!run_pump (h, r)) {
        if (on_keeper_thread (h) && h->keeper->pause.load (std::memory_order_relaxed)) return ICP_KEEPER_ABORTED;
        if (other && other->active) { const uint32_t ko = other->k_seen; (void) run_pump (h, *other); if (other->k_seen != ko || other->decided) t_last = std::chrono::steady_clock::now (); }
        _mm_pause ();
        if ((++spins & 0x3FFu) == 0u) {
            const auto now = std::chrono::steady_clock::now ();
            if (r.k_seen != k_last) { k_last = r.k_seen; t_last = now; }
            else if (r.k0 && std::chrono::duration<double> (now - t_last).count () > 0.05) { r.k0 = 0u; t_last = now; }
            else if (r.track_slot >= 0 && h->hGateFlag && *h->hGateFlag) {
                r.active = false;
                return fail (h, ICP_EHIP, "tracking: the device made no progress for ~0.5 s (a frame's gate gave up; the frames behind it were skipped): icp_track_reset starts a new sequence");
            }
            else if (std::chrono::duration<double> (now - t_last).count () > 20.0) {
                r.active = false;
                return fail (h, ICP_EHIP, "checked run: the device has published no progress for 20 s");
            }
        }
    }
    r.t[3] = now_s ();
    run_enqueue_end (h, r);
    r.t[4] = now_s ();
    for (int i = 0; i < 5; ++i) h->stat_t[i] = r.t[i];
    h->stat_launch_max_us = std::max (h->stat_launch_max_us, r.launch_max_us); h->stat_launch_slow += r.launch_slow; h->stat_launch_total += r.enq;
    r.active = false;
    h->stat_launches = r.enq; h->stat_k = r.k_final;
    h->stat_dead = r.done_seen ? r.enq - std::min (r.enq, r.k_final - r.k0 + 1u) : 0u;
    HIPCHK (h, hipGetLastError ());
    return ICP_OK;
}

int run_wait_final (icp_context *h, volatile unsigned long long *mirror, uint32_t n, uint32_t epoch, bool tracked)
{
    uint32_t spins = 0;
    const auto t0 = std::chrono::steady_clock::now ();
    for (uint32_t b = 0; b < n; ++b) {
        for (;;) {
            const unsigned long long w = mirror[b];
            if ((uint32_t) (w >> 32) == epoch && (w & ICP_MIRROR_FINAL)) break;
            _mm_pause ();
            if ((++spins & 0x3FFFu) == 0u && tracked && h->hGateFlag && *h->hGateFlag)
                return fail (h, ICP_EHIP, "tracking: the device made no progress for ~0.5 s (a frame's gate gave up; the frames behind it were skipped): icp_track_reset starts a new sequence");
            if ((spins & 0x3FFFu) == 0u && std::chrono::duration<double> (std::chrono::steady_clock::now () - t0).count () > 60.0) {
                const hipError_t e = hipStreamQuery (h->stream);
                if (e != hipSuccess && e != hipErrorNotReady) return fail (h, ICP_EHIP, std::string ("checked run: ") + hipGetErrorString (e));
                return fail (h, ICP_EHIP, "checked run: the final state has not arrived after 60 s");
            }
        }
    }
    std::atomic_thread_fence (std::memory_order_acquire);
    return ICP_OK;
}

int run_close_all (icp_context *h)
{
    run_ctl *a = &h->run, *b = &h->run2;
    if (a->active && b->active && b->p.seq_value < a->p.seq_value) std::swap (a, b);
    int rc;
    if (a->active && (rc = run_finish (h, *a, b->active ? b : nullptr))) return rc;
    if (b->active && (rc = run_finish (h, *b, nullptr))) return rc;
    if (h->stream2_dirty && h->stream2) { HIPCHK (h, hipStreamSynchronize (h->stream2)); h->stream2_dirty = false; }
    return ICP_OK;
}

int launch_run (icp_context *h, uint32_t iterations, int check, bool fresh, bool with_build)
{
    static const char *e = std::getenv ("ICP_AMD_RUN_GRAPH");
    if (e && e[0] == '0') {
        HIPCHK (h, enqueue_fixed_run (h, iterations, check, fresh, with_build));
        HIPCHK (h, hipGetLastError ());
    } else {
        hipGraphExec_t exec;
        int rc = get_graph (h, iterations, check, &exec, fresh, with_build);
        if (rc) return rc;
        HIPCHK (h, hipGraphLaunch (exec, h->stream));
    }
    h->hstate_fresh = check != 0; h->hstate_here = false;
    h->k_base = check ? -1 : (fresh || with_build) ? (long long) iterations : (h->k_base >= 0 ? h->k_base + iterations : -1);
    note_outputs_stored (h);
    return ICP_OK;
}

int settle (icp_context *h)
{
    HIPCHK (h, hipStreamSynchronize (h->stream));
    return ICP_OK;
}

void note_enqueue (icp_context *h) { h->hstate_fresh = false; h->hstate_here = false; h->k_base = -1; }

void note_inputs_change (icp_context *h) { if (h->outputs_stale) { h->outputs_stale = false; h->outputs_lost = true; } }
void note_outputs_stored (icp_context *h) { h->outputs_stale = false; h->outputs_lost = false; }

static bool is_query_output (int mem) { return mem == ICP_MEM_NN_ID || mem == ICP_MEM_W || mem == ICP_MEM_NN || mem == ICP_MEM_QT || mem == ICP_MEM_RID; }

int materialize_outputs (icp_context *h, int mem)
{
    if (!is_query_output (mem)) return ICP_OK;
    if (h->outputs_lost)
        return fail (h, ICP_ESTATE, "the per-query outputs of the last checked run were not stored (lazy outputs) and its inputs have changed since: "
                                    "read them before F / M / the RBC change, or switch to icp_set_output_mode (h, ICP_OUTPUTS_EVERY_ITERATION)");
    if (!h->outputs_stale) return ICP_OK;
    icp_params q = h->p;
    q.st = q.st_prev; q.check = 0; q.emit = 1; q.hmirror = nullptr; q.hstate = nullptr;
    icp_launch_masked (q, h->stream, 1u, &h->recip);
    HIPCHK (h, hipGetLastError ());
    h->outputs_stale = false;
    return ICP_OK;
}

}
```

### icp_amd/csrc/icp_search.h

```cpp
#pragma once
#include "icp_kernels.h"

static __device__ __forceinline__ float sum4 (float4 v) { return ((v.x + v.y) + v.z) + v.w; }
static __device__ __forceinline__ uint32_t ks_hole_bit (float4 mg) { return (mg.x == 0.f && mg.y == 0.f && mg.z == 0.f) ? 0x80000000u : 0u; }

#define KS_SPLIT LPQ
#define KS_QPW (64 / KS_SPLIT)
#define KS_TILE 1024u
#ifndef ICP_S2_DEPTH16
#define ICP_S2_DEPTH16 8u
#endif
#ifndef ICP_S2_UNCOND
#define ICP_S2_UNCOND 128u
#endif
#ifndef ICP_OL_STAGED_MIN
#define ICP_OL_STAGED_MIN 32u
#endif
#ifndef ICP_S1_REJECT_MIN_NR
#define ICP_S1_REJECT_MIN_NR 1024u
#endif

typedef float float2v __attribute__ ((ext_vector_type (2)));

struct k_search_args {
// ... 32 lines not shown
#ifndef KS_KEEP
#define KS_KEEP(a, b)
#endif

#define KS_MIN_DPP(v, CTRL) asm ("s_nop 1\n\tv_min_f32_dpp %0, %1, %1 " CTRL " row_mask:0xf bank_mask:0xf bound_ctrl:1" : "=v"(v) : "v"(v))
template <int LPQ> static __device__ __forceinline__ float ks_grp_min_f (float v)
{
    KS_MIN_DPP (v, "quad_perm:[1,0,3,2]");
    KS_MIN_DPP (v, "quad_perm:[2,3,0,1]");
    KS_MIN_DPP (v, "row_half_mirror");
    if (LPQ == 16) KS_MIN_DPP (v, "row_mirror");
    return v;
}
template <int LPQ> static __device__ __forceinline__ uint32_t ks_grp_min_u (uint32_t v)
{
    v = min (v, (uint32_t) __builtin_amdgcn_update_dpp (0, (int) v, 0xB1, 0xF, 0xF, true));
    v = min (v, (uint32_t) __builtin_amdgcn_update_dpp (0, (int) v, 0x4E, 0xF, 0xF, true));
    v = min (v, (uint32_t) __builtin_amdgcn_update_dpp (0, (int) v, 0x141, 0xF, 0xF, true));
    if (LPQ == 16) v = min (v, (uint32_t) __builtin_amdgcn_update_dpp (0, (int) v, 0x140, 0xF, 0xF, true));
    return v;
}

static __device__ __forceinline__ void ks_seed_against_invalid (uint32_t sfl, const float4 *s_count, uint32_t nr, uint32_t b, const float4 *R4, uint32_t &seed,
                                                                float &sx, float &sy, float &sz, float &sr, float &sg, float &sb)
{
    if (__builtin_expect (__ballot (sfl != 0u) == 0ull, 1)) return;
    const bool hq = (sfl & 2u) != 0u;
    const bool s0 = sx == 0.f && sy == 0.f && sz == 0.f;
    if (__ballot (hq != s0) == 0ull) return;
    if (__builtin_amdgcn_readfirstlane ((int) __float_as_uint (s_count->w)) == 0) return;
    const icp_params *po = ks_params_from_kernarg ();
    typedef float4 __attribute__ ((address_space (1))) *gf4;
    const float4 *OLb = (const float4 *) (gf4) po->OL + (size_t) b * ICP_OL_STRIDE (nr);
    if (hq != s0) {
        uint32_t s2 = icp_other_kind_near (reinterpret_cast<const unsigned long long *> (OLb + ICP_OL_MASKS (nr)), nr, seed, s0, hq ? __float_as_uint (OLb[1].w) : seed);
        s2 = min (s2, nr - 1u);
        const float4 g = R4[2 * (size_t) s2], c = R4[2 * (size_t) s2 + 1];
        seed = s2; sx = g.x; sy = g.y; sz = g.z; sr = c.x; sg = c.y; sb = c.z;
    }
}

template <int LPQ>
static __device__ __forceinline__ void ks_origin_list (const float4 *ent, const float4 *box, uint32_t n_e, bool boxed, float qq, bool need, float qr, float qg, float qb, float alpha,
                                                       float lim, uint32_t lane, uint32_t ss, float &best, uint32_t &bid)
{
    if (!boxed) {
        for (uint32_t e0 = 0; e0 < n_e; e0 += 4u * (uint32_t) LPQ) {
            float4 v[4];
#pragma unroll
            for (uint32_t k = 0; k < 4u; ++k) v[k] = ent[min (e0 + ss + k * (uint32_t) LPQ, n_e - 1u)];
#pragma unroll
            for (uint32_t k = 0; k < 4u; ++k) {
                const float dr_ = qr - v[k].x, dg_ = qg - v[k].y, db_ = qb - v[k].z;
                const float d = __builtin_fmaf (alpha, __builtin_fmaf (db_, db_, __builtin_fmaf (dg_, dg_, dr_ * dr_)), qq);
                const uint32_t idx = __float_as_uint (v[k].w);
                if (need && (d < best || (d == best && idx < bid))) { best = d; bid = idx; }
            }
        }
        return;
    }
    const uint32_t n_oc = (n_e + 7u) >> 3;
    for (uint32_t cb = 0; cb < n_oc; cb += (uint32_t) LPQ) {
        const uint32_t c = min (cb + ss, n_oc - 1u);
        const float4 lo = box[2u * c], hi = box[2u * c + 1u];
        const float er = fmaxf (fmaxf (lo.x - qr, qr - hi.x), 0.f), eg = fmaxf (fmaxf (lo.y - qg, qg - hi.y), 0.f), eb = fmaxf (fmaxf (lo.z - qb, qb - hi.z), 0.f);
        const float bound = __builtin_fmaf (alpha, __builtin_fmaf (eb, eb, __builtin_fmaf (eg, eg, er * er)), qq);
        const float lim2 = fminf (lim, ks_grp_min_f<LPQ> (best));
        const bool pass = need && cb + ss < n_oc && bound <= lim2;
        const unsigned long long bal = __ballot (pass);
        uint32_t mask = (uint32_t) (bal >> (lane & (64u - (uint32_t) LPQ))) & ((1u << LPQ) - 1u);
        while (__ballot (mask != 0u)) {
            const bool live = mask != 0u;
            const uint32_t e = 8u * (cb + (live ? (uint32_t) __builtin_ctz (mask) : 0u)) + (ss & 7u);
            mask &= mask - 1u;
            const float4 v = ent[min (e, n_e - 1u)];
            const float dr_ = qr - v.x, dg_ = qg - v.y, db_ = qb - v.z;
            const float d = __builtin_fmaf (alpha, __builtin_fmaf (db_, db_, __builtin_fmaf (dg_, dg_, dr_ * dr_)), qq);
            const uint32_t idx = __float_as_uint (v.w);
            if (live && (d < best || (d == best && idx < bid))) { best = d; bid = idx; }
        }
    }
}

template <int LPQ, uint32_t PB_>
static __device__ __forceinline__ void ks_origin_section (float4 *s_pair, uint32_t *s_ovote, uint32_t n_origin, uint32_t nr, uint32_t b, uint32_t slice, uint32_t tid,
                                                          float qx, float qy, float qz, float qr, float qg, float qb, float alpha, float s1_lim,
                                                          uint32_t lane, uint32_t ss, float &best, uint32_t &bid)
{
    const float qq = __builtin_fmaf (qz, qz, __builtin_fmaf (qy, qy, qx * qx));
    const bool need = qq <= s1_lim;
    auto list_base = [&] () -> const float4 * {
        const icp_params *po = ks_params_from_kernarg ();
        typedef float4 __attribute__ ((address_space (1))) *gf4;
        return (const float4 *) (gf4) po->OL + (size_t) b * ICP_OL_STRIDE (nr);
    };
    constexpr uint32_t OE = ((PB_ * 4u / 5u) / 8u) * 8u;
    const bool boxed = n_origin > ICP_OL_BOXED_MIN;
    if (n_origin > ICP_OL_STAGED_MIN && n_origin <= OE) {
        if (need) *s_ovote = 1u;
        __syncthreads ();
        if (*s_ovote) {
            const float4 *OLb = list_base ();
            if constexpr (OE <= 64u * LPQ) {
                const uint32_t tl = slice * 64u + __builtin_amdgcn_mbcnt_hi (~0u, __builtin_amdgcn_mbcnt_lo (~0u, 0u));
                if (tl < n_origin) s_pair[tl] = OLb[1u + tl];
                if (boxed && tl < 2u * ((n_origin + 7u) >> 3)) s_pair[OE + tl] = OLb[1u + nr + tl];
            } else {
                for (uint32_t k = tid; k < n_origin; k += 64u * LPQ) s_pair[k] = OLb[1u + k];
                if (boxed) for (uint32_t k = tid; k < 2u * ((n_origin + 7u) >> 3); k += 64u * LPQ) s_pair[OE + k] = OLb[1u + nr + k];
            }
            __syncthreads ();
            if (__ballot (need)) ks_origin_list<LPQ> (s_pair, s_pair + OE, n_origin, boxed, qq, need, qr, qg, qb, alpha, s1_lim, lane, ss, best, bid);
        }
    } else if (__ballot (need)) {
        const float4 *OLb = list_base ();
        ks_origin_list<LPQ> (OLb + 1u, OLb + 1u + nr, n_origin, boxed, qq, need, qr, qg, qb, alpha, s1_lim, lane, ss, best, bid);
    }
}

#define KS_CAND(G, C, J)                                                                              \
    {                                                                                                 \
        const float2v d1_ = vq_xr - float2v { (G).x, (G).y }, d2_ = vq_yg - float2v { (G).z, (G).w }, \
                      d3_ = vq_zb - float2v { (C).x, (C).y };                                         \
        const float2v gp_ = __builtin_elementwise_fma (d3_, d3_, __builtin_elementwise_fma (d2_, d2_, d1_ * d1_)); \
        const float d_ = __builtin_fmaf (alpha, gp_.y, gp_.x);                                        \
        if (d_ < best2) { best2 = d_; bj = (J); }                                                     \
    }

#define KS_CAND_IF(G, C, J, LIVE)                                                                     \
    {                                                                                                 \
        const float2v d1_ = vq_xr - float2v { (G).x, (G).y }, d2_ = vq_yg - float2v { (G).z, (G).w }, \
                      d3_ = vq_zb - float2v { (C).x, (C).y };                                         \
        const float2v gp_ = __builtin_elementwise_fma (d3_, d3_, __builtin_elementwise_fma (d2_, d2_, d1_ * d1_)); \
        const float d_ = __builtin_fmaf (alpha, gp_.y, gp_.x);                                        \
        if (d_ < best2 && (LIVE)) { best2 = d_; bj = (J); }                                           \
    }

#define KS_PAIR(P3, R0)                                                                                                                  \
    {                                                                                                                                    \
        float4 A = s_pair[P3], B = s_pair[(P3) + 1], C = s_pair[(P3) + 2];                                                                \
        float2v x = { A.x, A.y }, y = { A.z, A.w }, z = { B.x, B.y }, r = { B.z, B.w }, g = { C.x, C.y }, bb = { C.z, C.w };              \
        float2v dx = vqx - x, dy = vqy - y, dz = vqz - z, dr = vqr - r, dg = vqg - g, db = vqb - bb;                                      \
        float2v geo = __builtin_elementwise_fma (dz, dz, __builtin_elementwise_fma (dy, dy, dx * dx));                                    \
        float2v pho = __builtin_elementwise_fma (db, db, __builtin_elementwise_fma (dg, dg, dr * dr));                                    \
        float2v d = __builtin_elementwise_fma (va, pho, geo);                                                                             \
        const uint32_t r0 = (R0);                                                                                                         \
        if (d.x < best) { best = d.x; bid = r0; }                                                                                         \
        if (d.y < best) { best = d.y; bid = r0 + 1u; }                                                                                    \
    }

#define ICP_NMOM 18

#ifdef ICP_DBG_STAMPS
#define FF_STAMP(k)                                                                                       \
    {                                                                                                     \
        unsigned long long t_;                                                                            \
        asm volatile ("s_waitcnt vmcnt(0) lgkmcnt(0)\n\ts_memtime %0\n\ts_waitcnt lgkmcnt(0)" : "=s"(t_) :: "memory"); \
        if (threadIdx.x == 0 && p.dbg) p.dbg[(size_t) (blockIdx.y * gridDim.x + blockIdx.x) * 16 + (k)] = t_;    \
    }
#else
#define FF_STAMP(k)
#endif

static __device__ __forceinline__ uint32_t ks_tile_of_block (uint32_t bx, uint32_t nbx)
{
    return (nbx & 7u) == 0u ? (bx & 7u) * (nbx >> 3) + (bx >> 3) : bx;
}

static __device__ __forceinline__ uint32_t fused_query_index (uint32_t m, uint32_t side, uint32_t tpr_magic, uint32_t b, uint32_t e)
{
    const uint32_t tpr = side >> 3, ty = __umulhi (b, tpr_magic), tx = b - ty * tpr;
    const uint32_t tiled = (8u * ty + (e >> 3)) * side + 8u * tx + (e & 7u);
    return (side && (side & 7u) == 0u && side * side == m) ? tiled : b * 64u + e;
// ... 589 lines not shown
#pragma unroll 1
        for (uint32_t t = 0, g = ss; g < ngt; ++t, g += KS_SPLIT) test (t, g);
    } else
        for (uint32_t t = 0, g = ss; g < ngt; ++t, g += KS_SPLIT) test (t, g);
    return cm;
}

template <int LPQ>
static __device__ __forceinline__ void ks_fine_pass (const float4 *s_pair, uint32_t pair0, float qx, float qy, float qz, float qr, float qg, float qb, float alpha,
                                                     uint32_t gt_lg1, uint32_t ss, uint32_t t0_, uint32_t npair_, uint32_t cmask_, float &best, uint32_t &bid)
{
    const uint32_t ngt_ = (npair_ + KS_SPLIT - 1u) / KS_SPLIT;
    const float2v vqx = { qx, qx }, vqy = { qy, qy }, vqz = { qz, qz }, vqr = { qr, qr }, vqg = { qg, qg }, vqb = { qb, qb };
    const float2v va = { alpha, alpha };
    for (uint32_t t = 0; t * KS_SPLIT < ngt_; ++t) {
        unsigned long long bal = __ballot ((cmask_ >> t) & 1u);
        if (bal == 0ull) continue;
        bal |= bal >> 32; bal |= bal >> 16;
        if (KS_SPLIT == 8) bal |= bal >> 8;
        uint32_t need = (uint32_t) bal & ((1u << KS_SPLIT) - 1u);
        while (need) {
            const uint32_t sg = (uint32_t) __builtin_ctz (need);
            need &= need - 1u;
            const uint32_t gl = sg + KS_SPLIT * t;
            const uint32_t P = (KS_SPLIT == 8 && gt_lg1) ? (((4u * (gl >> (gt_lg1 - 1u)) + (ss >> 1)) << gt_lg1) + 2u * (gl & ((1u << (gt_lg1 - 1u)) - 1u)) + (ss & 1u))
                                                          : gl * KS_SPLIT + ss;
            if (P < npair_) {
                const uint32_t P3 = pair0 + __umul24 (P, 3u);
                float4 A = s_pair[P3], B = s_pair[P3 + 1], C = s_pair[P3 + 2];
                float2v x = { A.x, A.y }, y = { A.z, A.w }, z = { B.x, B.y }, r = { B.z, B.w }, g = { C.x, C.y }, bb = { C.z, C.w };
                float2v dx = vqx - x, dy = vqy - y, dz = vqz - z, dr = vqr - r, dg = vqg - g, db = vqb - bb;
                float2v geo = __builtin_elementwise_fma (dz, dz, __builtin_elementwise_fma (dy, dy, dx * dx));
                float2v pho = __builtin_elementwise_fma (db, db, __builtin_elementwise_fma (dg, dg, dr * dr));
                float2v d = __builtin_elementwise_fma (va, pho, geo);
                const uint32_t r0 = t0_ + 2u * P;
                if (d.x < best) { best = d.x; bid = r0; }
                if (d.y < best) { best = d.y; bid = r0 + 1u; }
            }
        }
    }
}

template <int MINW, bool MASKED, uint32_t KT>
static __device__ __forceinline__ uint2 ks_winner_list (const uint2 *s_on, const uint32_t *gO, const uint32_t *gN, uint32_t rstar, uint32_t nr, uint32_t ht)
{
    uint32_t o, n;
    if (MINW == 2 || (MASKED ? rstar / KT == ht : nr <= KT)) {
        const uint2 on = s_on[rstar - (MASKED ? ht * KT : 0u)]; o = on.x; n = on.y;
        if constexpr (MINW != 2) asm volatile ("" : "+v"(o), "+v"(n));
    } else { o = gO[rstar]; n = gN[rstar]; }
    return make_uint2 (o, n);
}

template <bool FUSED, bool CHAIN, int MINW, int LPQ, bool OWNER = false, int ROT = 1, int TILE = 1024, bool SINGLE = false, bool S2W = false, bool HOSTRUN = false,
          bool REJ = false>
__global__ __launch_bounds__ (64 * LPQ, TILE == 256 ? 8 : MINW) void k_search (const float *gM, const float *gR, icp_reg_state *gst, const double *gmom,
                                                              uint32_t m, uint32_t nr, uint32_t side, uint32_t tpr_magic,
                                                              uint32_t nb, uint32_t check_flags, icp_params p)
{
    constexpr uint32_t KT = (uint32_t) TILE;
    constexpr bool MASKED = (TILE == 256) && !SINGLE && (MINW == 4);
    constexpr bool ONE_TILE = SINGLE || CHAIN;
    if constexpr (ONE_TILE) __builtin_assume (nr <= KT);
    if constexpr (MASKED) __builtin_assume (nr > KT && nr <= 32u * KT);
    const uint32_t b = blockIdx.y, check = check_flags & 1u;
    icp_reg_state *st = (CHAIN && !(check_flags & 2u)) ? gst + (size_t) b * 2 : gst + b;
#ifdef ICP_DBG_STAMPS
    { const uint32_t tid = threadIdx.x; unsigned long long t_; asm volatile ("s_memtime %0\n\ts_waitcnt lgkmcnt(0)" : "=s"(t_) :: "memory");
      KS_STAMP_STORE (8) }
#endif

    constexpr uint32_t NBUF = MASKED ? 2u : 1u, PB = 3u * KT / 2u, BB = 2u * (KT / 16u);
    __shared__ float4 s_pair[NBUF * PB];
    __shared__ uint2 s_on[(MASKED && OWNER) ? 1 : KT];
    __shared__ uint32_t s_tmask;
    __shared__ uint32_t s_ovote;
    __shared__ float4 s_box[NBUF * BB];
    __shared__ float4 s_tbox[(MINW == 4 && !SINGLE) ? 2 * 32 : 2];
    __shared__ float s_w[64];
    __shared__ float4 s_qc[64];
    __shared__ float4 s_qa[64];
    __shared__ uint4 s_qb[64];
    __shared__ uint32_t s_slot[MINW == 4 ? 64 : 1];
    __shared__ double s_mom[FUSED ? ICP_NMOM : 1][64];
    __shared__ icp_fin_result s_fin;
    __shared__ double s_l1[CHAIN ? ICP_NMOM : 1][CHAIN ? 32 : 1];
    __shared__ double s_t[ICP_NMOM];

    const uint32_t tid = threadIdx.x, lane = tid & 63u;
    const uint32_t slice = __builtin_amdgcn_readfirstlane (tid >> 6);
    const uint32_t qe = slice * KS_QPW + lane / KS_SPLIT, ss = lane & (KS_SPLIT - 1u);
    const bool qwave = CHAIN ? slice == 0u : slice == KS_SPLIT - 1u;
    constexpr bool OWNER_LISTS = OWNER && MINW == 2;
    const uint32_t tile_id = OWNER_LISTS ? blockIdx.x : (FUSED && (MINW == 2 || (check_flags & 64u))) ? ks_tile_of_block (blockIdx.x, nb) : blockIdx.x;
    const uint32_t iq = OWNER_LISTS ? blockIdx.x * 64u + lane :
                        FUSED ? fused_query_index (m, side, tpr_magic, tile_id, lane)
                              : (blockIdx.x >> 1) * 128u + 2u * lane + (blockIdx.x & 1u);

    const float4 *M4 = reinterpret_cast<const float4 *> (gM + (size_t) b * m * 8);
    const float4 *R4 = reinterpret_cast<const float4 *> (gR + (size_t) b * nr * 8);

    uint32_t sv = OWNER ? 0u : state_load_lanes (st);
    uint32_t run_over = 0u;
    if constexpr (CHAIN) {
        static_assert (ICP_ST_DW (T) == 0 && ICP_ST_DW (Tk) == 8 && ICP_ST_DW (R) == 16 && ICP_ST_DW (Rk) == 25 && ICP_ST_DW (reserved0) == 60, "state layout");
        if (check_flags & 16u) {
            constexpr unsigned long long ones = (1ull << 3) | (1ull << 7) | (1ull << 11) | (1ull << 15) | (1ull << 16) | (1ull << 20) | (1ull << 24) |
                                                (1ull << 25) | (1ull << 29) | (1ull << 33);
            if (lane < ICP_ST_DW (reserved0)) sv = ((ones >> lane) & 1ull) ? 0x3F800000u : 0u;
        }
    }
    double ma0[8];
    if constexpr (CHAIN) fused_moment_loads<64 * LPQ> (gmom + (size_t) b * 2 * ICP_NMOM * nb, nb, 0u, ma0);
    float *s_pairf = reinterpret_cast<float *> (s_pair);
    const uint32_t tn0 = min (KT, nr);
    float4 rg[2], rc[2]; uint2 ron[2];
    uint32_t ht = 0u, tnH = 0u;
#pragma unroll
    for (int u = 0; u < 2; ++u) {
        uint32_t k = tid + (uint32_t) u * 64u * KS_SPLIT;
        if (MASKED && u == 0) continue;
        rg[u] = make_float4 (0.f, 0.f, 0.f, 0.f); rc[u] = rg[u];
        if constexpr (OWNER_LISTS) {
            if (k < tn0) {
                const uint32_t src = rep_src_index (p, k);
                rg[u] = M4[2 * (size_t) src]; rc[u] = M4[2 * (size_t) src + 1];
                if (blockIdx.x == 0) {
                    float4 *Rw = reinterpret_cast<float4 *> (p.R + (size_t) b * nr * 8);
                    Rw[2 * (size_t) k] = rg[u]; Rw[2 * (size_t) k + 1] = rc[u];
                    p.rep_src[(size_t) b * nr + k] = src;
                }
            }
        } else if (!MASKED && k < tn0) { rg[u] = R4[2 * (size_t) k]; rc[u] = R4[2 * (size_t) k + 1]; }
    }
    const uint32_t ic = min (iq, m - 1u);
    typedef float ks_f4 __attribute__ ((ext_vector_type (4)));
    ks_f4 mgv = { 0.f, 0.f, 0.f, 1.f }, mcv = mgv;
    if (qwave) { mgv = *reinterpret_cast<const ks_f4 *> (M4 + 2 * (size_t) ic); mcv = *reinterpret_cast<const ks_f4 *> (M4 + 2 * (size_t) ic + 1); }
    if constexpr (MASKED) {
        const uint32_t i0 = (uint32_t) __builtin_amdgcn_readfirstlane ((int) min (FUSED ? fused_query_index (m, side, tpr_magic, tile_id, 0u) : (blockIdx.x >> 1) * 128u + (blockIdx.x & 1u), m - 1u));
        const uint32_t cell = p.side_magic ? cell_rep_of (p, i0) : 0u;
        ht = min (cell, nr - 1u) / KT; tnH = min (KT, nr - ht * KT);
        if (tid < tnH) { rg[0] = R4[2 * (size_t) (ht * KT + tid)]; rc[0] = R4[2 * (size_t) (ht * KT + tid) + 1]; }
    }
    const uint32_t *gO = p.O + (size_t) b * nr, *gN = p.N + (size_t) b * nr;
#pragma unroll
    for (int u = 0; u < 2; ++u) {
        uint32_t k = tid + (uint32_t) u * 64u * KS_SPLIT;
        ron[u] = make_uint2 (0u, 0u);
        if (!OWNER && !MASKED && k < tn0) ron[u] = make_uint2 (gO[k], gN[k]);
        if (!OWNER && MASKED && u == 0 && tid < tnH) ron[0] = make_uint2 (gO[ht * KT + tid], gN[ht * KT + tid]);
    }
    if constexpr (CHAIN && HOSTRUN) { if (p.run_flag) run_over = (p.run_flag[b] == p.epoch) ? 1u : 0u; }
    constexpr bool PRUNE = MINW == 4;
    const bool prune = PRUNE && p.a > 0.f;
    const uint32_t gt_lg1 = p.gtile;
    uint32_t seed = 0u, seed_cell = 0xFFFFFFFFu;
    if (qwave && prune && p.side_magic) seed_cell = cell_rep_of (p, ic);
    if constexpr (OWNER) seed = (seed_cell == 0xFFFFFFFFu ? 0u : seed_cell) | (PRUNE ? 0x40000000u : 0u);
    else if (qwave && prune) {
        seed = p.rid[(size_t) b * m + ic];
        if ((check_flags & 32u) || seed_cell == 0xFFFFFFFFu) seed_cell = 0xFFFFFFFFu;
    }
    const float4 *GBt = p.GB + (size_t) b * 2 * (p.n16 + p.n1k) + (KS_SPLIT == 8 ? 0u : 2u * p.n16);
    const uint32_t nbox0 = 2u * ((tn0 + 2u * KS_SPLIT - 1u) / (2u * KS_SPLIT));
    float4 boxv = make_float4 (0.f, 0.f, 0.f, 0.f);
    if (!MASKED && prune && tid < nbox0) boxv = GBt[tid];
    const uint32_t nboxH = 2u * ((tnH + 2u * KS_SPLIT - 1u) / (2u * KS_SPLIT));
    if (MASKED && prune && tid < nboxH) boxv = GBt[2u * (ht * KT / (2u * KS_SPLIT)) + tid];
    float T[8];
#pragma unroll
    for (int k = 0; k < 8; ++k) T[k] = state_lane_f (sv, ICP_ST_DW (T) + k);
    if constexpr (PRUNE && !OWNER) {
        if (seed_cell != 0xFFFFFFFFu && __builtin_amdgcn_readlane ((int) sv, (int) ICP_ST_DW (k)) == 0) seed = seed_cell | 0x40000000u;
    }
    icp_reg_state *sout = CHAIN ? p.cst + (size_t) b * 2 + (p.slot ^ 1u) : st;
    if constexpr (!OWNER && !CHAIN) {
        const uint32_t done_ = (uint32_t) __builtin_amdgcn_readlane ((int) sv, (int) ICP_ST_DW (done));
        if (p.hmirror && blockIdx.x == 0 && tid == 0 && !(FUSED && done_))
            icp_mirror_store (p.hmirror + b, ICP_MIRROR_WORD (p.epoch, (uint32_t) __builtin_amdgcn_readlane ((int) sv, (int) ICP_ST_DW (k)), done_));
    }
    if constexpr (CHAIN && HOSTRUN) { if (run_over) return; }
    if (!OWNER && check && __builtin_amdgcn_readlane ((int) sv, (int) ICP_ST_DW (done))) {
        if constexpr (CHAIN) {
            if (blockIdx.x == 0 && tid < sizeof (icp_reg_state) / 4) reinterpret_cast<uint32_t *> (sout)[tid] = sv;
        }
        return;
    }
    if constexpr (!S2W) asm volatile ("" : "+v"(mgv), "+v"(mcv));
    float4 mg = make_float4 (mgv.x, mgv.y, mgv.z, mgv.w), mc = make_float4 (mcv.x, mcv.y, mcv.z, mcv.w);
    if (iq >= m) { mg = make_float4 (0.f, 0.f, 0.f, 1.f); mc = mg; }
    uint32_t hbit = 0u;
    if constexpr (REJ && !OWNER) { hbit = ks_hole_bit (mg); if constexpr (CHAIN) asm volatile ("" : "+v"(hbit)); }
    const float4 *XQ4 = reinterpret_cast<const float4 *> (p.XQ + (size_t) b * m * 8);
    const char *XQb = reinterpret_cast<const char *> (XQ4);
#pragma unroll
    for (int u = 0; u < 2; ++u) {
        uint32_t k = tid + (uint32_t) u * 64u * KS_SPLIT;
        if (!MASKED && k < tn0) {
            ks_rep_to_lds (s_pairf, k, rg[u], rc[u]);
            if constexpr (!OWNER && !MASKED) s_on[k] = ron[u];
        }
    }
    if (!MASKED && prune && tid < nbox0) s_box[tid] = boxv;
    auto home_to_lds = [&] () {
        if (tid < tnH) ks_rep_to_lds (s_pairf + PB * 4u, tid, rg[0], rc[0]);
        if (prune && tid < nboxH) s_box[BB + tid] = boxv;
    };
    if constexpr (MASKED) {
        home_to_lds ();
        if constexpr (!OWNER) { if (tid < tnH) s_on[tid] = ron[0]; }
    }
    if (MASKED && tid == 0) s_tmask = 0u;
    if (PRUNE && tid == 0) s_ovote = 0u;
    if constexpr (MINW == 4 && !SINGLE) {
        if (prune && nr > KT && tid < 2u * p.n1k) s_tbox[tid] = p.GB[(size_t) b * 2 * (p.n16 + p.n1k) + 2u * p.n16 + tid];
    }
    bool handed = false;
    if constexpr (CHAIN) {
        const bool pending = __builtin_amdgcn_readlane ((int) sv, (int) ICP_ST_DW (pending)) != 0;
        if (pending) {
            auto hand_over = [&] (const float *Tn) {
                float tx, ty, tz;
                icp_transform_point (Tn, mg.x, mg.y, mg.z, tx, ty, tz);
                s_qa[lane] = make_float4 (tx, ty, tz, __uint_as_float (iq));
                s_qc[lane] = make_float4 (mc.x, mc.y, mc.z, __uint_as_float (seed | hbit));
            };
            fused_finalize_block<32, 64 * LPQ, ROT, true, REJ> (p, gmom + (size_t) b * 2 * ICP_NMOM * nb, nb, 0u, sv, ma0, &s_fin, s_l1, s_t, nullptr,
                                                           blockIdx.x == 0 ? sout : nullptr, hand_over, 1u,
                                                           (HOSTRUN && blockIdx.x == 0 && p.hmirror) ? p.hmirror + b : nullptr, HOSTRUN, HOSTRUN ? p.st + b : nullptr,
                                                           (HOSTRUN && p.hstate) ? p.hstate + b : nullptr, (HOSTRUN && p.st_prev) ? p.st_prev + b : nullptr);
            handed = true;
            KS_STAMP (9)
            if (s_fin.done) return;
        } else if (blockIdx.x == 0 && tid < sizeof (icp_reg_state) / 4) {
            reinterpret_cast<uint32_t *> (sout)[tid] = (tid == offsetof (icp_reg_state, pending) / 4) ? 1u : sv;
        }
    }
    if (qwave && !handed) {
        float tx = mg.x, ty = mg.y, tz = mg.z;
        if constexpr (!OWNER) icp_transform_point (T, mg.x, mg.y, mg.z, tx, ty, tz);
        if constexpr (PRUNE) {
            const bool hole = mg.x == 0.f && mg.y == 0.f && mg.z == 0.f;
            const float4 ha = make_float4 (tx, ty, tz, __uint_as_float (iq)), hc = make_float4 (mc.x, mc.y, mc.z, __uint_as_float (hole ? (seed | 0x80000000u) : seed));
            s_qa[lane] = ha; s_qc[lane] = hc; s_slot[lane] = lane;
            const unsigned long long hb = __ballot (hole);
            if (__builtin_expect (hb != 0ull, 0)) {
                const unsigned long long lt = (1ull << lane) - 1ull;
                const uint32_t pos = hole ? 64u - (uint32_t) __builtin_popcountll (hb) + (uint32_t) __builtin_popcountll (hb & lt) : (uint32_t) __builtin_popcountll (~hb & lt);
                s_qa[pos] = ha; s_qc[pos] = hc; s_slot[pos] = lane;
            }
        } else {
            s_qa[lane] = make_float4 (tx, ty, tz, __uint_as_float (iq));
            s_qc[lane] = make_float4 (mc.x, mc.y, mc.z, __uint_as_float (seed | hbit));
        }
    }
    float qx = 0.f, qy = 0.f, qz = 0.f, qr = 0.f, qg = 0.f, qb = 0.f;
    uint32_t i = 0u; bool valid = false;
    const float alpha = p.a;
    KS_STAMP (0)

    float best = __builtin_inff (), s1_lim = __builtin_inff (); uint32_t bid = 0xFFFFFFFFu;
    uint32_t n_origin = 0u;
    if constexpr (MASKED) {
        __syncthreads ();
        {
            const float4 a4 = s_qa[qe], c4 = s_qc[qe];
            if constexpr (PRUNE) { if (prune) n_origin = (uint32_t) __builtin_amdgcn_readfirstlane ((int) __float_as_uint (s_tbox[1].w)); }
            qx = a4.x; qy = a4.y; qz = a4.z; i = __float_as_uint (a4.w); valid = i < m;
            qr = c4.x; qg = c4.y; qb = c4.z; seed = __float_as_uint (c4.w);
        }
        const uint32_t ntile = (nr + KT - 1u) / KT;
        uint32_t qmask = 0xFFFFFFFFu >> (32u - ntile);
        if (prune) {
            const uint32_t sfl = seed >> 30;
            seed = min (seed & 0x3FFFFFFFu, nr - 1u);
            float sx, sy, sz, sr, sg, sb;
            if (seed / KT == ht) {
                const float *sp = s_pairf + PB * 4u + ((seed - ht * KT) >> 1) * 12u + (seed & 1u);
                sx = sp[0]; sy = sp[2]; sz = sp[4]; sr = sp[6]; sg = sp[8]; sb = sp[10];
                asm volatile ("" : "+v"(sx), "+v"(sy), "+v"(sz), "+v"(sr), "+v"(sg), "+v"(sb));
            } else {
                const float4 g = R4[2 * (size_t) seed], c = R4[2 * (size_t) seed + 1];
                sx = g.x; sy = g.y; sz = g.z; sr = c.x; sg = c.y; sb = c.z;
            }
            ks_seed_against_invalid (sfl, s_tbox + 1, nr, b, R4, seed, sx, sy, sz, sr, sg, sb);
            const float b0 = icp_metric8 (qx, qy, qz, qr, qg, qb, sx, sy, sz, sr, sg, sb, alpha);
            if (b0 >= 0.f && b0 < __builtin_inff ()) s1_lim = __uint_as_float (__float_as_uint (b0) + 1u);
            uint32_t tm = 0u;
#pragma unroll 1
            for (uint32_t t = ss; t < ntile; t += KS_SPLIT) {
                if (ks_box_bound (s_tbox[2u * t], s_tbox[2u * t + 1u], qx, qy, qz) < s1_lim) tm |= 1u << t;
            }
            tm |= (uint32_t) __builtin_amdgcn_update_dpp (0, (int) tm, 0xB1, 0xF, 0xF, true);
            tm |= (uint32_t) __builtin_amdgcn_update_dpp (0, (int) tm, 0x4E, 0xF, 0xF, true);
            tm |= (uint32_t) __builtin_amdgcn_update_dpp (0, (int) tm, 0x141, 0xF, 0xF, true);
            qmask = tm;
        }
        {
            uint32_t wm = qmask | (uint32_t) __builtin_amdgcn_update_dpp (0, (int) qmask, 0x140, 0xF, 0xF, true);
            wm = (uint32_t) __builtin_amdgcn_readlane ((int) wm, 0) | (uint32_t) __builtin_amdgcn_readlane ((int) wm, 16) |
                 (uint32_t) __builtin_amdgcn_readlane ((int) wm, 32) | (uint32_t) __builtin_amdgcn_readlane ((int) wm, 48);
            if (lane == 0) atomicOr (&s_tmask, wm);
        }
        __syncthreads ();
        KS_STAMP (10)
        uint32_t bm = s_tmask;
        bool used0 = false;
        while (bm) {
            const uint32_t tl = (uint32_t) __builtin_ctz (bm);
            bm &= bm - 1u;
            const uint32_t t0 = tl * KT, tn = min (KT, nr - t0), npair = (tn + 1u) >> 1;
            const uint32_t hb = tl == ht ? 1u : 0u;
            if (!hb) {
                if (used0) __syncthreads ();
                used0 = true;
                if (prune) {
                    const uint32_t nbx = 2u * ((tn + 2u * KS_SPLIT - 1u) / (2u * KS_SPLIT));
                    if (tid < nbx) s_box[tid] = GBt[2u * (t0 / (2u * KS_SPLIT)) + tid];
                }
                if (tid < tn) ks_rep_to_lds (s_pairf, tid, R4[2 * (size_t) (t0 + tid)], R4[2 * (size_t) (t0 + tid) + 1]);
                __syncthreads ();
            }
            if (prune) {
                const bool mine = ((qmask >> tl) & 1u) != 0u;
                uint32_t cmask = 0u;
                if (__ballot (mine)) cmask = ks_coarse_pass<LPQ, TILE> (s_box, hb * BB, qx, qy, qz, ss, tn, mine ? s1_lim : -__builtin_inff ());
                ks_fine_pass<LPQ> (s_pair, hb * PB, qx, qy, qz, qr, qg, qb, alpha, gt_lg1, ss, t0, npair, cmask, best, bid);
                s1_lim = fminf (s1_lim, ks_grp_min_f<KS_SPLIT> (best));
            } else {
                const float2v vqx = { qx, qx }, vqy = { qy, qy }, vqz = { qz, qz }, vqr = { qr, qr }, vqg = { qg, qg }, vqb = { qb, qb };
                const float2v va = { alpha, alpha };
                for (uint32_t P = ss; P < npair; P += KS_SPLIT) KS_PAIR (hb * PB + 3 * P, t0 + 2u * P)
            }
        }
    } else
    for (uint32_t t0 = 0; t0 < nr; t0 += KT) {
        const uint32_t tn = min (KT, nr - t0);
        uint32_t cmask = 0u;
        auto tile_near = [&] (float lim_) -> bool {
            if (ONE_TILE || nr <= KT) return true;
            return ks_box_bound (s_tbox[2u * (t0 / ICP_TBOX)], s_tbox[2u * (t0 / ICP_TBOX) + 1u], qx, qy, qz) < lim_;
        };
        if (t0) {
            __syncthreads ();
            if (prune) {
                const bool near = tile_near (s1_lim);
                if (!__syncthreads_or (near)) continue;
                const uint32_t nbx = 2u * ((tn + 2u * KS_SPLIT - 1u) / (2u * KS_SPLIT));
                for (uint32_t k = tid; k < nbx; k += 64 * KS_SPLIT) s_box[k] = GBt[2u * (t0 / (2u * KS_SPLIT)) + k];
                __syncthreads ();
                if (__ballot (near)) cmask = ks_coarse_pass<LPQ, TILE> (s_box, 0u, qx, qy, qz, ss, tn, s1_lim);
                if (!__syncthreads_or (cmask != 0u)) continue;
            }
            for (uint32_t k = tid; k < tn; k += 64 * KS_SPLIT) {
                ks_rep_to_lds (s_pairf, k, R4[2 * (size_t) (t0 + k)], R4[2 * (size_t) (t0 + k) + 1]);
                if constexpr (!OWNER) s_on[k] = make_uint2 (gO[t0 + k], gN[t0 + k]);
            }
        }
        if ((tn & 1u) && tid == 0) {
            const float qnan = __builtin_nanf ("");
            ks_rep_to_lds (s_pairf, tn, make_float4 (qnan, qnan, qnan, qnan), make_float4 (qnan, qnan, qnan, qnan));
        }
        if (!(CHAIN && handed && t0 == 0u && !(tn & 1u))) __syncthreads ();
        if (t0 == 0) {
            const float4 a4 = s_qa[qe], c4 = s_qc[qe];
            if constexpr (PRUNE) { if (prune) n_origin = (uint32_t) __builtin_amdgcn_readfirstlane ((int) __float_as_uint ((!SINGLE && nr > KT) ? s_tbox[1].w : s_box[1].w)); }
            qx = a4.x; qy = a4.y; qz = a4.z; i = __float_as_uint (a4.w); valid = i < m;
            qr = c4.x; qg = c4.y; qb = c4.z; seed = __float_as_uint (c4.w);
        }
        KS_STAMP (1)
        const uint32_t npair = (tn + 1u) >> 1;
        const float2v vqx = { qx, qx }, vqy = { qy, qy }, vqz = { qz, qz }, vqr = { qr, qr }, vqg = { qg, qg }, vqb = { qb, qb };
        const float2v va = { alpha, alpha };
        float lim = __builtin_inff ();
        if (t0 == 0 && prune) {
            const uint32_t sfl = seed >> 30;
            seed = min (seed & 0x3FFFFFFFu, nr - 1u);
            float sx, sy, sz, sr, sg, sb;
            if (MINW == 2 || nr <= KT) {
                const float *sp = s_pairf + (seed >> 1) * 12u + (seed & 1u);
                sx = sp[0]; sy = sp[2]; sz = sp[4]; sr = sp[6]; sg = sp[8]; sb = sp[10];
                asm volatile ("" : "+v"(sx), "+v"(sy), "+v"(sz), "+v"(sr), "+v"(sg), "+v"(sb));
            } else {
                const float4 g = R4[2 * (size_t) seed], c = R4[2 * (size_t) seed + 1];
                sx = g.x; sy = g.y; sz = g.z; sr = c.x; sg = c.y; sb = c.z;
            }
            if constexpr (MINW == 4)
                ks_seed_against_invalid (sfl, (!SINGLE && nr > KT) ? s_tbox + 1 : s_box + 1, nr, b, R4, seed, sx, sy, sz, sr, sg, sb);
            const float b0 = icp_metric8 (qx, qy, qz, qr, qg, qb, sx, sy, sz, sr, sg, sb, alpha);
            if (b0 >= 0.f && b0 < __builtin_inff ()) lim = __uint_as_float (__float_as_uint (b0) + 1u);
            s1_lim = lim;
        } else if (prune) lim = s1_lim;
        if (prune) {
            if (t0 == 0 && __ballot (tile_near (lim))) cmask = ks_coarse_pass<LPQ, TILE> (s_box, 0u, qx, qy, qz, ss, tn, lim);
            ks_fine_pass<LPQ> (s_pair, 0u, qx, qy, qz, qr, qg, qb, alpha, gt_lg1, ss, t0, npair, cmask, best, bid);
            s1_lim = fminf (lim, ks_grp_min_f<KS_SPLIT> (best));
        } else {
#pragma unroll 8
            for (uint32_t P = ss; P < npair; P += KS_SPLIT) KS_PAIR (3 * P, t0 + 2u * P)
        }
    }
    KS_STAMP (14)
    if constexpr (PRUNE) {
        if (prune && __builtin_expect (n_origin != 0u, 0))
            ks_origin_section<KS_SPLIT, PB> (s_pair, &s_ovote, n_origin, nr, b, slice, tid, qx, qy, qz, qr, qg, qb, alpha, s1_lim, lane, ss, best, bid);
    }
    KS_KEEP (best, bid)
    KS_STAMP (2)
    const float dr = ks_grp_min_f<KS_SPLIT> (best);
    const bool named = PRUNE ? (best == dr && dr < __builtin_inff ()) : (best == dr);
    uint32_t rstar = ks_grp_min_u<KS_SPLIT> (named ? bid : 0xFFFFFFFFu);
    if (rstar == 0xFFFFFFFFu) rstar = 0u;
    if constexpr (OWNER_LISTS) {
        ks_owner_lists_tail (p, s_qb, b, m, nb, lane, slice, qe, ss, valid, rstar);
        return;
    } else if constexpr (OWNER) {
        if (ss == 0u && valid) p.owner[(size_t) b * m + i] = rstar;
        return;
    }
    KS_KEEP (dr, rstar)
    KS_STAMP (3)
    const uint2 on = ks_winner_list<MINW, MASKED, KT> (s_on, gO, gN, rstar, nr, ht);
    const uint32_t o = on.x, n = on.y;

    float dmin; uint32_t jmin;
    if constexpr (S2W) {
        static_assert (MINW == 4 && LPQ == 8 && !OWNER, "lanes = candidates: the dense search variants");
        ks_stage2_wave (XQb, o, n, valid, rstar, qx, qy, qz, qr, qg, qb, alpha, dr, b, lane, s_qa, s_qc, qe, dmin, jmin);
    } else ks_stage2_lanes<LPQ> (XQb, o, n, valid, qx, qy, qz, qr, qg, qb, alpha, dr, b, lane, ss, dmin, jmin);
    KS_KEEP (dmin, jmin)
    KS_STAMP (5)
    ks_epilogue<FUSED, CHAIN, MINW, LPQ, OWNER, PRUNE, REJ> (p, s_qa, s_qb, s_qc, s_slot, s_mom, s_w, R4, XQb, b, m, nr, check_flags, tid, lane, slice, tile_id, qe, ss, i, valid, o, n, rstar, dr, dmin, jmin,
                                                        qx, qy, qz);
}


static inline uint32_t icp_tpr_magic (uint32_t side)
{
    const uint32_t tpr = side >> 3;
    return tpr ? (uint32_t) ((1ull << 32) / tpr + 1ull) : 0u;
}
#define KS_FLAGS(p) ((uint32_t) ((p).check ? 1u : 0u) | ((p).emit ? 8u : 0u) | ((p).warm_seed ? 32u : 0u) | ((p).xcdmap ? 64u : 0u))
#define KS_ARGS p.M, p.R, p.st, (const double *) p.mom, p.m, p.nr, p.side, icp_tpr_magic (p.side), p.nb, KS_FLAGS (p), p
#define KS_CHAIN_ARGS p.M, p.R, p.cst + p.slot, (const double *) p.mom + (size_t) p.slot * ICP_NMOM * p.nb, p.m, p.nr, p.side, icp_tpr_magic (p.side), p.nb, KS_FLAGS (p), p
#define KS_OWNER_ARGS p.F, p.R, p.st, (const double *) p.mom, p.m, p.nr, p.side, icp_tpr_magic (p.side), p.nb, 0u, p

typedef void (*ks_kernel) (const float *, const float *, icp_reg_state *, const double *, uint32_t, uint32_t, uint32_t, uint32_t, uint32_t, uint32_t, icp_params);
template <bool FUSED, bool REJ> constexpr ks_kernel ks_latency = k_search<FUSED, false, 2, 16, false, 1, 1024, false, false, false, REJ>;
template <bool FUSED, int TILE, bool SINGLE, bool S2W, bool REJ> constexpr ks_kernel ks_dense = k_search<FUSED, false, 4, 8, false, 1, TILE, SINGLE, S2W, false, REJ>;
template <int ROT, bool HOSTRUN, bool REJ> constexpr ks_kernel ks_chained = k_search<true, true, 2, 16, false, ROT, 1024, false, false, HOSTRUN, REJ>;
enum ks_owner_form { KS_OWNER_LATENCY, KS_OWNER_DENSE_1024, KS_OWNER_DENSE_256_SINGLE, KS_OWNER_DENSE_256_MASKED };
template <ks_owner_form F> constexpr ks_kernel ks_owner =
    k_search<true, false, F == KS_OWNER_LATENCY ? 2 : 4, F == KS_OWNER_LATENCY ? 16 : 8, true, 1, (F == KS_OWNER_DENSE_256_SINGLE || F == KS_OWNER_DENSE_256_MASKED) ? 256 : 1024,
             F == KS_OWNER_DENSE_256_SINGLE>;

template <bool FUSED, bool REJ>
static inline ks_kernel ks_dense_kernel (const ks_dense_form &f)
{
    if (f.masked) return f.s2w ? ks_dense<FUSED, 256, false, true, REJ> : ks_dense<FUSED, 256, false, false, REJ>;
    if (f.single) return f.s2w ? ks_dense<FUSED, 256, true, true, REJ> : ks_dense<FUSED, 256, true, false, REJ>;
    return f.s2w ? ks_dense<FUSED, 1024, false, true, REJ> : ks_dense<FUSED, 1024, false, false, REJ>;
}
template <bool REJ>
void ks_launch_dense (const icp_params &p, hipStream_t s)
{
    const ks_dense_form f = ks_dense_select (p.nr, p.nrx, p.s2wave);
    const ks_kernel k = p.fused ? ks_dense_kernel<true, REJ> (f) : ks_dense_kernel<false, REJ> (f);
    hipLaunchKernelGGL (k, dim3 (ks_dense_grid_x (p.fused, p.nb, p.nwg), p.batch), dim3 (KS_DENSE_THREADS), 0, s, KS_ARGS);
}

template <bool REJ>
void ks_launch_latency (const icp_params &p, hipStream_t s)
{
    if (p.fused) hipLaunchKernelGGL ((ks_latency<true, REJ>), dim3 (p.nb, p.batch), dim3 (1024), 0, s, KS_ARGS);
    else hipLaunchKernelGGL ((ks_latency<false, REJ>), dim3 (2 * p.nwg, p.batch), dim3 (1024), 0, s, KS_ARGS);
}

template <bool REJ>
void ks_launch_chain_one (const icp_params &p0, hipStream_t s, uint32_t j, bool fresh, bool emit)
{
    icp_params p = p0;
    p.slot = j & 1u;
    p.emit = emit ? 1 : 0;
    const uint32_t first_flags = 2u | (fresh ? 16u : 0u);
    const bool hostrun = p.hmirror != nullptr;
    const ks_kernel k = p.rot == 1 ? (hostrun ? ks_chained<1, true, REJ> : ks_chained<1, false, REJ>) : (hostrun ? ks_chained<0, true, REJ> : ks_chained<0, false, REJ>);
    if (j == 0) hipLaunchKernelGGL (k, dim3 (p.nb, p.batch), dim3 (1024), 0, s, p.M, p.R, p.st, (const double *) p.mom, p.m, p.nr, p.side, icp_tpr_magic (p.side), p.nb, KS_FLAGS (p) | first_flags, p);
    else hipLaunchKernelGGL (k, dim3 (p.nb, p.batch), dim3 (1024), 0, s, KS_CHAIN_ARGS);
}
```

### include/icp_amd.h

```cpp
#ifndef ICP_AMD_H
#define ICP_AMD_H

#include <stddef.h>
#include <stdint.h>

#ifdef __cplusplus
extern "C" {
#endif
#if defined(__GNUC__) || defined(__clang__)
#pragma GCC visibility push(default)
#endif

typedef struct icp_context *icp_handle;

typedef enum {
    ICP_OK = 0,
    ICP_EINVAL = 1,
    ICP_EHIP = 2,
    ICP_ENOMEM = 3,
    ICP_ESTATE = 4,
    ICP_ENODEVICE = 5
} icp_status;

typedef enum { ICP_ROT_EIGEN = 0, ICP_ROT_POWER_METHOD = 1 } icp_rot;
typedef enum { ICP_W_REGULAR = 0, ICP_W_WEIGHTED = 1 } icp_weighting;

typedef enum { ICP_POWER_LITERAL = 0, ICP_POWER_SQUARED = 1 } icp_power_mode;

typedef enum { ICP_REDUCE_REFERENCE_ORDER = 0, ICP_REDUCE_FUSED = 1 } icp_reduce_mode;

typedef enum {
    ICP_MEM_F = 0,
    ICP_MEM_M = 1,
    ICP_MEM_T = 2,
    ICP_MEM_TK = 3,
    ICP_MEM_MEANS = 4,
    ICP_MEM_S = 5,
    ICP_MEM_NN_ID = 6,
    ICP_MEM_W = 7,
    ICP_MEM_SUM_W = 8,
    ICP_MEM_REPS = 9,
    ICP_MEM_RBC_N = 10,
    ICP_MEM_RBC_O = 11,
    ICP_MEM_RBC_PERM = 12,
    ICP_MEM_RBC_OWNER = 13,
    ICP_MEM_RBC_XP = 14,
    ICP_MEM_RID = 15,
    ICP_MEM_R = 16,
    ICP_MEM_RK = 17,
    ICP_MEM_NN = 18,
    ICP_MEM_QT = 19,
    ICP_MEM_TRIM = 20,
    ICP_MEM_NORMALS_F = 21,
    ICP_MEM_PLANE_SYSTEM = 22,
    ICP_MEM_COLOR_GRAD_F = 23,
    ICP_MEM_NORMALS_M = 24,
    ICP_MEM_UNIQUE = 25,
    ICP_MEM_PAIR_FILTER = 26,
    ICP_MEM_RECIPROCAL = 27,
    ICP_MEM_REVERSE_ID = 28,
    ICP_MEM_COUNT_
} icp_mem;

typedef struct {
    float R[9], q[4], t[3], s;
    float Rk[9], qk[4], tk[3], sk;
    uint32_t k;
    uint32_t converged;
    uint32_t power_iterations;
    uint32_t reserved;
} icp_state_t;


int icp_create (icp_handle *h, int device, int rot, int weighted);
int icp_destroy (icp_handle h);

int icp_init (icp_handle h, uint32_t m, uint32_t nr, float a, float c,
              uint32_t max_iterations, double angle_threshold, double translation_threshold);
int icp_init_batched (icp_handle h, uint32_t batch, uint32_t m, uint32_t nr, float a, float c,
                      uint32_t max_iterations, double angle_threshold,
                      double translation_threshold);


int icp_write (icp_handle h, int mem, const void *host_ptr, int block);
int icp_write_b (icp_handle h, uint32_t batch_index, int mem, const void *host_ptr, int block);

int icp_read (icp_handle h, int mem, void *host_dst, size_t bytes);
int icp_read_b (icp_handle h, uint32_t batch_index, int mem, void *host_dst, size_t bytes);
size_t icp_mem_size (icp_handle h, int mem);

int icp_device_ptr (icp_handle h, int mem, void **dptr);
int icp_adopt_device_buffer (icp_handle h, int mem, void *dptr);


int icp_build_rbc (icp_handle h);

int icp_step (icp_handle h, int config);

int icp_run (icp_handle h, uint32_t *k);

int icp_run_stats (icp_handle h, uint32_t *launches, uint32_t *k, uint32_t *dead_launches);

int icp_launch_stats (icp_handle h, double *max_us, uint64_t *slower_than_10us, uint64_t *total, int reset);

typedef enum { ICP_OUTPUTS_LAZY = 0, ICP_OUTPUTS_EVERY_ITERATION = 1 } icp_output_mode;
int icp_set_output_mode (icp_handle h, int mode);

int icp_run_timeline (icp_handle h, double *us6);

int icp_set_run_depth (icp_handle h, uint32_t depth, int adaptive);

int icp_run_fixed (icp_handle h, uint32_t iterations);

int icp_reset_transform (icp_handle h);

int icp_run_fixed_fresh (icp_handle h, uint32_t iterations);

int icp_sync (icp_handle h);

int icp_get_alpha (icp_handle h, float *a);
int icp_set_alpha (icp_handle h, float a);
int icp_get_scaling (icp_handle h, float *c);
int icp_set_metric_scale (icp_handle h, float f_g);
int icp_get_metric_scale (icp_handle h, float *f_g);

#define ICP_REJECT_INVALID 1
int icp_set_rejection (icp_handle h, int flags, float max_dist);
int icp_get_rejection (icp_handle h, int *flags, float *max_dist);

int icp_set_trimming (icp_handle h, float keep_fraction);
int icp_get_trimming (icp_handle h, float *keep_fraction);

int icp_set_unique (icp_handle h, int on);
int icp_get_unique (icp_handle h, int *on);

int icp_set_reciprocal (icp_handle h, int on, float max_gap);
int icp_get_reciprocal (icp_handle h, int *on, float *max_gap);

int icp_set_normal_rejection (icp_handle h, int on, float min_cos);
int icp_get_normal_rejection (icp_handle h, int *on, float *min_cos);
int icp_set_boundary_rejection (icp_handle h, uint32_t grid_width);
int icp_get_boundary_rejection (icp_handle h, uint32_t *grid_width);

#define ICP_METRIC_POINT_TO_POINT 0
#define ICP_METRIC_POINT_TO_PLANE 1
#define ICP_METRIC_COLORED 2
int icp_set_error_metric (icp_handle h, int metric, float point_weight);
int icp_get_error_metric (icp_handle h, int *metric, float *point_weight);

int icp_set_color_weight (icp_handle h, float kappa);
int icp_get_color_weight (icp_handle h, float *kappa);

#define ICP_ROBUST_NONE 0
#define ICP_ROBUST_HUBER 1
#define ICP_ROBUST_CAUCHY 2
#define ICP_ROBUST_TUKEY 3
int icp_set_robust_loss (icp_handle h, int loss, float scale);
int icp_get_robust_loss (icp_handle h, int *loss, float *scale);

int icp_set_plane_to_plane (icp_handle h, float epsilon);
int icp_get_plane_to_plane (icp_handle h, float *epsilon);

int icp_set_symmetric (icp_handle h, int on);
int icp_get_symmetric (icp_handle h, int *on);

#define ICP_NORMALS_GIVEN 0
#define ICP_NORMALS_GRID 1
int icp_set_normals (icp_handle h, int source, uint32_t grid_width);
int icp_get_normals (icp_handle h, int *source, uint32_t *grid_width);
int icp_set_scaling (icp_handle h, float c);
int icp_get_max_iterations (icp_handle h, uint32_t *n);
int icp_set_max_iterations (icp_handle h, uint32_t n);
int icp_get_angle_threshold (icp_handle h, double *deg);
int icp_set_angle_threshold (icp_handle h, double deg);
int icp_get_translation_threshold (icp_handle h, double *mm);
int icp_set_translation_threshold (icp_handle h, double mm);
int icp_set_power_mode (icp_handle h, int mode);
int icp_set_reduce_mode (icp_handle h, int mode);

int icp_state (icp_handle h, icp_state_t *out);
int icp_state_b (icp_handle h, uint32_t batch_index, icp_state_t *out);

typedef struct {
    double fitness, inlier_rmse, sum_geo, information[36];
    uint32_t n, n_moving, n_inliers, reserved;
} icp_quality_t;
// ... 161 lines not shown
```

Baseline: 116,900.

## Precompute per-point origin-list nearest color entries to prune origin section search

Adds a build-time kernel that, for each hole point in M, scans the origin list once to record its nearest color entry and a lower bound over lower-indexed entries. The dense search kernel loads this cache and uses it to seed the best match and skip the per-iteration origin-list scan when the bound proves no other entry can win. The cache is invalidated when inputs change and is disabled for owner, reciprocal and adopted-M paths. It adds extra memory in the rid buffer, an extra kernel at build time, and shared memory in the search kernel.

```diff
diff --git a/icp_amd/__init__.py b/icp_amd/__init__.py
--- a/icp_amd/__init__.py
+++ b/icp_amd/__init__.py
@@ -152,6 +152,7 @@
     sig("icp_run_timeline", i32, vp, C.POINTER(f64))
     sig("icp_set_output_mode", i32, vp, i32)
     sig("icp_launch_stats", i32, vp, C.POINTER(f64), C.POINTER(C.c_uint64), C.POINTER(C.c_uint64), i32)
+    sig("icp_origin_cache_stats", i32, vp, C.POINTER(C.c_uint64), C.POINTER(C.c_uint64), i32)
     sig("icp_run_fixed", i32, vp, u32)
     sig("icp_run_fixed_fresh", i32, vp, u32)
     sig("icp_sync", i32, vp)
@@ -986,6 +987,11 @@
         self._chk(self._L.icp_launch_stats(self._h, C.byref(mx), C.byref(slow), C.byref(tot), int(reset)))
         return mx.value, slow.value, tot.value
 
+    def origin_cache_stats(self, reset=False):
+        f, n = C.c_uint64(), C.c_uint64()
+        self._chk(self._L.icp_origin_cache_stats(self._h, C.byref(f), C.byref(n), int(reset)))
+        return f.value, n.value
+
     def set_output_mode(self, every_iteration=False):
         self._chk(self._L.icp_set_output_mode(self._h, int(every_iteration)))
 
diff --git a/icp_amd/csrc/icp_build.hip b/icp_amd/csrc/icp_build.hip
--- a/icp_amd/csrc/icp_build.hip
+++ b/icp_amd/csrc/icp_build.hip
@@ -778,6 +778,53 @@
     hipLaunchKernelGGL (k_list_boxes, dim3 (p.nr, p.batch), dim3 (256), 0, s, p);
 }
 
+__global__ __launch_bounds__ (256) void k_origin_cache (const float *gM, const float4 *gOL, float4 *oc, uint32_t m, uint32_t nr)
+{
+    const uint32_t b = blockIdx.y, i = blockIdx.x * 256u + threadIdx.x;
+    const float4 *OLb = gOL + (size_t) b * ICP_OL_STRIDE (nr);
+    const uint32_t n = min (__float_as_uint (OLb[0].x), nr);
+    if (!n) return;
+    float4 rec = make_float4 (__uint_as_float (ICP_OC_NONE), __builtin_inff (), __builtin_inff (), 0.f);
+    bool hole = false;
+    float qr = 0.f, qg = 0.f, qb = 0.f;
+    if (i < m) {
+        const float4 *M4 = reinterpret_cast<const float4 *> (gM) + 2 * ((size_t) b * m + i);
+        const float4 g = M4[0], c = M4[1];
+        hole = g.x == 0.f && g.y == 0.f && g.z == 0.f;
+        qr = c.x; qg = c.y; qb = c.z;
+    }
+    __shared__ float4 s_e[1024];
+    const bool busy = __ballot (hole) != 0ull;
+    float pho0 = __builtin_inff (), pho_lo = __builtin_inff (); uint32_t e0 = ICP_OC_NONE;
+    for (uint32_t pass = 0; pass < 2u; ++pass) {
+        for (uint32_t c0 = 0; c0 < n; c0 += 1024u) {
+            const uint32_t nc = min (1024u, n - c0);
+            __syncthreads ();
+            for (uint32_t k = threadIdx.x; k < nc; k += 256u) s_e[k] = OLb[1u + c0 + k];
+            __syncthreads ();
+            if (!busy) continue;
+#pragma unroll 4
+            for (uint32_t e = 0; e < nc; ++e) {
+                const float4 v = s_e[e];
+                const float dr_ = qr - v.x, dg_ = qg - v.y, db_ = qb - v.z;
+                const float pho = __builtin_fmaf (db_, db_, __builtin_fmaf (dg_, dg_, dr_ * dr_));
+                const uint32_t idx = __float_as_uint (v.w);
+                if (pass == 0u) { if (pho < pho0 || (pho == pho0 && idx < e0)) { pho0 = pho; e0 = idx; } }
+                else if (idx < e0 && pho < pho_lo) pho_lo = pho;
+            }
+        }
+    }
+    if (hole) rec = make_float4 (__uint_as_float (e0), pho0, pho_lo, 0.f);
+    if (i < m) oc[(size_t) b * m + i] = rec;
+}
+
+bool icp_origin_cache_on (const icp_params &p) { return (p.search_bits & ICP_SEARCH_ORIGIN_CACHE) != 0u && icp_dense (p); }
+
+void icp_launch_origin_cache (const icp_params &p, hipStream_t s)
+{
+    hipLaunchKernelGGL (k_origin_cache, dim3 ((p.m + 255u) / 256u, p.batch), dim3 (256), 0, s, p.M, (const float4 *) p.OL, icp_origin_cache (p.rid, p.batch, p.m), p.m, p.nr);
+}
+
 void icp_launch_build_rbc (const icp_params &p, hipStream_t s)
 {
     build_rbc_lists (p, s);
diff --git a/icp_amd/csrc/icp_capi.hip b/icp_amd/csrc/icp_capi.hip
--- a/icp_amd/csrc/icp_capi.hip
+++ b/icp_amd/csrc/icp_capi.hip
@@ -334,7 +334,10 @@
     p.tbox = icp_tbox_of (p); p.n1k = (nr + p.tbox - 1u) / p.tbox;
     p.s2wave = icp_s2_wave_of (p);
     { const char *e = std::getenv ("ICP_AMD_XCDMAP"); p.xcdmap = e ? (e[0] == '1') : (B == 1u); }
-    { const char *e = std::getenv ("ICP_AMD_WARM_SEED"); p.warm_seed = (e && e[0] == '1') ? 1u : 0u; }
+    { const char *e = std::getenv ("ICP_AMD_WARM_SEED"); p.search_bits = (e && e[0] == '1') ? ICP_SEARCH_WARM_SEED : 0u; }
+    { const char *e = std::getenv ("ICP_AMD_ORIGIN_CACHE");
+      if (!(e && e[0] == '0')) p.search_bits |= ICP_SEARCH_ORIGIN_CACHE | ((e && !std::strcmp (e, "count")) ? ICP_SEARCH_ORIGIN_COUNT : 0u); }
+    h->origin_gen = 0; h->origin_M = nullptr; h->origin_OL = nullptr; h->origin_fills = 0;
     p.gtile = 0u;
     if (nrx % 4u == 0u && nry % 4u == 0u && !std::getenv ("ICP_AMD_STRIP_GROUPS")) { uint32_t lg = 0; while ((4u << lg) < nrx) ++lg; p.gtile = lg + 1u; }
     p.nlb = m / 16u + 2u;
@@ -343,7 +346,7 @@
         if ((rc = icp_rbc_for_each (s, p, [&] (const char *, void **q, size_t bytes) { return dalloc (h, reinterpret_cast<char **> (q), bytes); }))) return rc;
         icp_rbc_into (p, s);
     }
-    if ((rc = dalloc (h, &p.rid, B * m))) return rc;
+    if ((rc = dalloc (h, &p.rid, icp_rid_words (B, m)))) return rc;
     if ((rc = dalloc (h, &p.nn_id, B * m))) return rc;
     if ((rc = dalloc (h, &p.PF, B * m))) return rc;
     if ((rc = dalloc (h, &p.PM, B * m))) return rc;
@@ -517,7 +520,8 @@
     int rc = need (h, false); if (rc) return rc;
     if (!dptr) return fail (h, ICP_EINVAL, "null pointer");
     if (mem == ICP_MEM_F) { h->dF = static_cast<float *> (dptr); h->p.F = h->dF; h->ownF = false; h->built = false; }
-    else if (mem == ICP_MEM_M) { h->dM = static_cast<float *> (dptr); h->p.M = h->dM; h->ownM = false; h->recip.stale = true; }
+    else if (mem == ICP_MEM_M) { h->dM = static_cast<float *> (dptr); h->p.M = h->dM; h->ownM = false; h->recip.stale = true;
+                                 h->p.search_bits &= ~(ICP_SEARCH_ORIGIN_CACHE | ICP_SEARCH_ORIGIN_COUNT); }
     else return fail (h, ICP_EINVAL, "only ICP_MEM_F and ICP_MEM_M can be adopted");
     note_inputs_change (h);
     drop_graphs (h);
@@ -638,6 +642,21 @@
 }
 ICP_CATCH_ALL
 
+int icp_origin_cache_stats (icp_handle h, uint64_t *fills, uint64_t *fallbacks, int reset) try
+{
+    api_guard guard_ (h);
+    int rc = need (h, false); if (rc) return rc;
+    if ((rc = set_device (h))) return rc;
+    uint32_t n = 0u;
+    HIPCHK (h, hipStreamSynchronize (h->stream));
+    HIPCHK (h, hipMemcpy (&n, icp_origin_cache_counters (h->p), sizeof n, hipMemcpyDeviceToHost));
+    if (fills) *fills = h->origin_fills;
+    if (fallbacks) *fallbacks = n;
+    if (reset) { HIPCHK (h, hipMemset (icp_origin_cache_counters (h->p), 0, sizeof n)); h->origin_fills = 0; }
+    return ICP_OK;
+}
+ICP_CATCH_ALL
+
 int icp_set_output_mode (icp_handle h, int mode) try
 {
     api_guard guard_ (h);
@@ -1037,6 +1056,7 @@
     q.check = 0; q.emit = 1; q.fused = 0; q.weighted = 0; q.hmirror = nullptr; q.hstate = nullptr; q.dbg = nullptr;
     q.reject = 0u; q.reject_d2 = 0.f; q.reject_max_dist = 0.f; q.trim_keep = 0.f; q.metric = ICP_METRIC_POINT_TO_POINT; q.p2pl_mu = 0.f; q.gicp = 0u;
     q.nn_id = Q.nn_id; q.PF = Q.PF; q.PM = Q.PM; q.rid = Q.rid;
+    q.search_bits &= ~(ICP_SEARCH_ORIGIN_CACHE | ICP_SEARCH_ORIGIN_COUNT);
     if (icp_dense (q)) HIPCHK (h, hipMemcpyAsync (Q.rid, p.rid, n * sizeof (uint32_t), hipMemcpyDeviceToDevice, h->stream));
     icp_launch_search (q, h->stream);
     return ICP_OK;
diff --git a/icp_amd/csrc/icp_host.h b/icp_amd/csrc/icp_host.h
--- a/icp_amd/csrc/icp_host.h
+++ b/icp_amd/csrc/icp_host.h
@@ -114,6 +114,8 @@
         std::vector<uint32_t> n; bool valid = false;
     } pairs;
     icp_reciprocal_set recip;
+    uint64_t inputs_gen = 1, origin_gen = 0, origin_fills = 0;
+    const float *origin_M = nullptr; const float4 *origin_OL = nullptr;
     float *dCloud = nullptr, *dCloudOut = nullptr; uint32_t cloud_cap = 0;
     std::map<uint64_t, icp_host::graph_entry> graphs;
     uint32_t parity = 0;
@@ -202,6 +204,9 @@
 int materialize_outputs (icp_context *h, int mem);
 void normals_m_follow (icp_context *h, uint32_t b0, uint32_t nb);
 int reciprocal_ready (icp_context *h);
+void origin_cache_fill (icp_context *h, const icp_params &p, hipStream_t s, bool enqueue_only = false);
+void origin_cache_note_filled (icp_context *h, const icp_params &p);
+int origin_cache_ready (icp_context *h);
 
 template <typename Fn>
 int capture_graph (icp_context *h, Fn &&launches, graph_entry *out, bool instantiate = true)
@@ -251,6 +256,7 @@
     if (with_build) icp_launch_build_rbc (r.p, r.stream);
     if (other && other->active) (void) run_pump (h, *other);
     { int rc = between (); if (rc) return rc; }
+    if (with_build) origin_cache_fill (h, r.p, r.stream);
     if (fresh && !r.chained) icp_launch_reset_state (r.p, r.stream, 1);
     r.active = true;
     const uint32_t n = std::min (std::max (blind, 1u), r.maxit);
diff --git a/icp_amd/csrc/icp_kernels.h b/icp_amd/csrc/icp_kernels.h
--- a/icp_amd/csrc/icp_kernels.h
+++ b/icp_amd/csrc/icp_kernels.h
@@ -20,6 +20,7 @@
 #endif
 #define ICP_OL_MASKS(nr) ((nr) + 1u + 2u * (((nr) + 7u) / 8u))
 #define ICP_OL_STRIDE(nr) (ICP_OL_MASKS (nr) + ((nr) + 127u) / 128u)
+#define ICP_OC_NONE 0xFFFFFFFFu
 #define ICP_CHUNK 1024u
 
 struct icp_params {
@@ -47,7 +48,7 @@
     uint32_t tbox;
     uint32_t gtile;
     uint32_t xcdmap;
-    uint32_t warm_seed;
+    uint32_t search_bits;
     uint32_t s2wave;
     uint32_t nrm_grid;
     float *XP;
@@ -86,6 +87,9 @@
     float reject_max_dist;
     float trim_keep;
 };
+#define ICP_SEARCH_WARM_SEED 1u
+#define ICP_SEARCH_ORIGIN_CACHE 2u
+#define ICP_SEARCH_ORIGIN_COUNT 4u
 #define ICP_REJECT_DIST_ON 0x80000000u
 #define ICP_REJECT_TRIM_ON 0x40000000u
 #define ICP_REJECT_ROBUST_SHIFT 28u
@@ -173,6 +177,10 @@
 static inline uint32_t *icp_pair_filter_settings (const icp_params &p) { return icp_pair_filter_area (p) + 12u * (size_t) p.batch; }
 static inline uint32_t *icp_reciprocal_area (const icp_params &p) { return reinterpret_cast<uint32_t *> (p.mom + icp_mom_layout_of (p).recip); }
 static inline uint32_t *icp_reciprocal_gap (const icp_params &p) { return icp_reciprocal_area (p) + 4u * (size_t) p.batch; }
+static __host__ __device__ inline size_t icp_rid_pad (size_t batch, uint32_t m) { return (batch * m + 3u) & ~(size_t) 3u; }
+static __host__ __device__ inline size_t icp_rid_words (size_t batch, uint32_t m) { return icp_rid_pad (batch, m) + 4u * (batch * m + 1u); }
+static __host__ __device__ inline float4 *icp_origin_cache (uint32_t *rid, uint32_t batch, uint32_t m) { return reinterpret_cast<float4 *> (rid + icp_rid_pad (batch, m)); }
+static inline uint32_t *icp_origin_cache_counters (const icp_params &p) { return reinterpret_cast<uint32_t *> (icp_origin_cache (p.rid, p.batch, p.m) + (size_t) p.batch * p.m); }
 
 struct icp_xp_layout {
     size_t normals, color_grad, normals_m, total;
@@ -261,6 +269,8 @@
 icp_route icp_route_of (const icp_params &p);
 
 void icp_launch_build_rbc (const icp_params &p, hipStream_t s);
+bool icp_origin_cache_on (const icp_params &p);
+void icp_launch_origin_cache (const icp_params &p, hipStream_t s);
 void icp_launch_search (const icp_params &p, hipStream_t s);
 struct icp_reciprocal_set;
 void icp_launch_iteration (const icp_params &p, hipStream_t s, const icp_reciprocal_set *rs = nullptr);
diff --git a/icp_amd/csrc/icp_reciprocal.hip b/icp_amd/csrc/icp_reciprocal.hip
--- a/icp_amd/csrc/icp_reciprocal.hip
+++ b/icp_amd/csrc/icp_reciprocal.hip
@@ -89,6 +89,7 @@
     q.fused = 0; q.weighted = 0; q.emit = 1; q.hmirror = nullptr; q.hstate = nullptr; q.dbg = nullptr;
     q.reject = 0u; q.reject_d2 = 0.f; q.reject_max_dist = 0.f; q.trim_keep = 0.f; q.metric = 0u; q.p2pl_mu = 0.f; q.gicp = 0u; q.nrm_grid = 0u;
     q.run_flag = nullptr; q.track_seq = nullptr;
+    q.search_bits &= ~(ICP_SEARCH_ORIGIN_CACHE | ICP_SEARCH_ORIGIN_COUNT);
     return q;
 }
 
diff --git a/icp_amd/csrc/icp_run.hip b/icp_amd/csrc/icp_run.hip
--- a/icp_amd/csrc/icp_run.hip
+++ b/icp_amd/csrc/icp_run.hip
@@ -26,7 +26,8 @@
         if (hipSetDevice (h->device) != hipSuccess) return fail (h, ICP_EHIP, "hipSetDevice");
         int rc = run_close_all (h); if (rc) return rc;
     }
-    if (built && !keep_run && icp_reciprocal (h->p)) return reciprocal_ready (h);
+    if (built && !keep_run && icp_reciprocal (h->p)) { int rc = reciprocal_ready (h); if (rc) return rc; }
+    if (built && !keep_run) return origin_cache_ready (h);
     return ICP_OK;
 }
 
@@ -42,7 +43,7 @@
 {
     icp_params p = h->p;
     p.check = check; p.hmirror = nullptr; p.hstate = nullptr;
-    if (with_build) icp_launch_build_rbc (p, h->stream);
+    if (with_build) { icp_launch_build_rbc (p, h->stream); origin_cache_fill (h, p, h->stream, true); }
     if (icp_route_of (p).chained) icp_launch_chain (p, h->stream, iterations, fresh);
     else {
         if (fresh) icp_launch_reset_state (p, h->stream, 1);
@@ -219,6 +220,7 @@
         if (rc) return rc;
         HIPCHK (h, hipGraphLaunch (exec, h->stream));
     }
+    if (with_build) origin_cache_note_filled (h, h->p);
     h->hstate_fresh = check != 0; h->hstate_here = false;
     h->k_base = check ? -1 : (fresh || with_build) ? (long long) iterations : (h->k_base >= 0 ? h->k_base + iterations : -1);
     note_outputs_stored (h);
@@ -233,7 +235,31 @@
 
 void note_enqueue (icp_context *h) { h->hstate_fresh = false; h->hstate_here = false; h->k_base = -1; }
 
-void note_inputs_change (icp_context *h) { if (h->outputs_stale) { h->outputs_stale = false; h->outputs_lost = true; } }
+void note_inputs_change (icp_context *h) { ++h->inputs_gen; if (h->outputs_stale) { h->outputs_stale = false; h->outputs_lost = true; } }
+
+void origin_cache_note_filled (icp_context *h, const icp_params &p)
+{
+    if (!icp_origin_cache_on (p)) return;
+    h->origin_gen = h->inputs_gen; h->origin_M = p.M; h->origin_OL = p.OL; ++h->origin_fills;
+}
+
+void origin_cache_fill (icp_context *h, const icp_params &p, hipStream_t s, bool enqueue_only)
+{
+    if (!icp_origin_cache_on (p)) return;
+    icp_launch_origin_cache (p, s);
+    if (!enqueue_only) origin_cache_note_filled (h, p);
+}
+
+int origin_cache_ready (icp_context *h)
+{
+    const icp_params &p = h->p;
+    if (!icp_origin_cache_on (p)) return ICP_OK;
+    if (h->origin_gen == h->inputs_gen && h->origin_M == p.M && h->origin_OL == p.OL) return ICP_OK;
+    HIPCHK (h, hipSetDevice (h->device));
+    origin_cache_fill (h, p, h->stream);
+    HIPCHK (h, hipGetLastError ());
+    return ICP_OK;
+}
 void note_outputs_stored (icp_context *h) { h->outputs_stale = false; h->outputs_lost = false; }
 
 static bool is_query_output (int mem) { return mem == ICP_MEM_NN_ID || mem == ICP_MEM_W || mem == ICP_MEM_NN || mem == ICP_MEM_QT || mem == ICP_MEM_RID; }
diff --git a/icp_amd/csrc/icp_search.h b/icp_amd/csrc/icp_search.h
--- a/icp_amd/csrc/icp_search.h
+++ b/icp_amd/csrc/icp_search.h
@@ -138,13 +138,28 @@
     }
 }
 
-template <int LPQ, uint32_t PB_>
-static __device__ __forceinline__ void ks_origin_section (float4 *s_pair, uint32_t *s_ovote, uint32_t n_origin, uint32_t nr, uint32_t b, uint32_t slice, uint32_t tid,
+template <int LPQ, uint32_t PB_, bool CACHE>
+static __device__ __forceinline__ void ks_origin_section (float4 *s_pair, uint32_t *s_ovote, const float4 *s_oc, uint32_t qe, uint32_t check_flags, uint32_t n_origin, uint32_t nr, uint32_t b, uint32_t slice, uint32_t tid,
                                                           float qx, float qy, float qz, float qr, float qg, float qb, float alpha, float s1_lim,
                                                           uint32_t lane, uint32_t ss, float &best, uint32_t &bid)
 {
     const float qq = __builtin_fmaf (qz, qz, __builtin_fmaf (qy, qy, qx * qx));
-    const bool need = qq <= s1_lim;
+    bool need = qq <= s1_lim;
+    if constexpr (CACHE) if (__ballot (need)) {
+        const float4 oc = s_oc[qe];
+        const uint32_t e0 = __float_as_uint (oc.x);
+        if (need && e0 != ICP_OC_NONE) {
+            const float d0 = __builtin_fmaf (alpha, oc.y, qq);
+            if (d0 < best || (d0 == best && e0 < bid)) { best = d0; bid = e0; }
+            need = !(__builtin_fmaf (alpha, oc.z, qq) > d0);
+            if (__builtin_expect ((check_flags & 256u) != 0u, 0)) {
+                if (need && ss == 0u) {
+                    const icp_params *po = ks_params_from_kernarg ();
+                    atomicAdd (reinterpret_cast<uint32_t *> (icp_origin_cache (po->rid, po->batch, po->m) + (size_t) po->batch * po->m), 1u);
+                }
+            }
+        }
+    }
     auto list_base = [&] () -> const float4 * {
         const icp_params *po = ks_params_from_kernarg ();
         typedef float4 __attribute__ ((address_space (1))) *gf4;
@@ -900,6 +915,7 @@
     __shared__ float4 s_qa[64];
     __shared__ uint4 s_qb[64];
     __shared__ uint32_t s_slot[MINW == 4 ? 64 : 1];
+    __shared__ float4 s_oc[(MINW == 4 && !OWNER) ? 64 : 1];
     __shared__ double s_mom[FUSED ? ICP_NMOM : 1][64];
     __shared__ icp_fin_result s_fin;
     __shared__ double s_l1[CHAIN ? ICP_NMOM : 1][CHAIN ? 32 : 1];
@@ -974,10 +990,12 @@
     const bool prune = PRUNE && p.a > 0.f;
     const uint32_t gt_lg1 = p.gtile;
     uint32_t seed = 0u, seed_cell = 0xFFFFFFFFu;
+    float4 ocv = make_float4 (__uint_as_float (ICP_OC_NONE), 0.f, 0.f, 0.f);
     if (qwave && prune && p.side_magic) seed_cell = cell_rep_of (p, ic);
     if constexpr (OWNER) seed = (seed_cell == 0xFFFFFFFFu ? 0u : seed_cell) | (PRUNE ? 0x40000000u : 0u);
     else if (qwave && prune) {
         seed = p.rid[(size_t) b * m + ic];
+        if constexpr (MINW == 4) { if (check_flags & 128u) ocv = icp_origin_cache (p.rid, p.batch, m)[(size_t) b * m + ic]; }
         if ((check_flags & 32u) || seed_cell == 0xFFFFFFFFu) seed_cell = 0xFFFFFFFFu;
     }
     const float4 *GBt = p.GB + (size_t) b * 2 * (p.n16 + p.n1k) + (KS_SPLIT == 8 ? 0u : 2u * p.n16);
@@ -1062,11 +1080,13 @@
             const bool hole = mg.x == 0.f && mg.y == 0.f && mg.z == 0.f;
             const float4 ha = make_float4 (tx, ty, tz, __uint_as_float (iq)), hc = make_float4 (mc.x, mc.y, mc.z, __uint_as_float (hole ? (seed | 0x80000000u) : seed));
             s_qa[lane] = ha; s_qc[lane] = hc; s_slot[lane] = lane;
+            if constexpr (!OWNER) s_oc[lane] = ocv;
             const unsigned long long hb = __ballot (hole);
             if (__builtin_expect (hb != 0ull, 0)) {
                 const unsigned long long lt = (1ull << lane) - 1ull;
                 const uint32_t pos = hole ? 64u - (uint32_t) __builtin_popcountll (hb) + (uint32_t) __builtin_popcountll (hb & lt) : (uint32_t) __builtin_popcountll (~hb & lt);
                 s_qa[pos] = ha; s_qc[pos] = hc; s_slot[pos] = lane;
+                if constexpr (!OWNER) s_oc[pos] = ocv;
             }
         } else {
             s_qa[lane] = make_float4 (tx, ty, tz, __uint_as_float (iq));
@@ -1222,7 +1242,7 @@
     KS_STAMP (14)
     if constexpr (PRUNE) {
         if (prune && __builtin_expect (n_origin != 0u, 0))
-            ks_origin_section<KS_SPLIT, PB> (s_pair, &s_ovote, n_origin, nr, b, slice, tid, qx, qy, qz, qr, qg, qb, alpha, s1_lim, lane, ss, best, bid);
+            ks_origin_section<KS_SPLIT, PB, !OWNER> (s_pair, &s_ovote, s_oc, qe, check_flags, n_origin, nr, b, slice, tid, qx, qy, qz, qr, qg, qb, alpha, s1_lim, lane, ss, best, bid);
     }
     KS_KEEP (best, bid)
     KS_STAMP (2)
@@ -1259,7 +1279,8 @@
     const uint32_t tpr = side >> 3;
     return tpr ? (uint32_t) ((1ull << 32) / tpr + 1ull) : 0u;
 }
-#define KS_FLAGS(p) ((uint32_t) ((p).check ? 1u : 0u) | ((p).emit ? 8u : 0u) | ((p).warm_seed ? 32u : 0u) | ((p).xcdmap ? 64u : 0u))
+#define KS_FLAGS(p) ((uint32_t) ((p).check ? 1u : 0u) | ((p).emit ? 8u : 0u) | (((p).search_bits & ICP_SEARCH_WARM_SEED) ? 32u : 0u) | ((p).xcdmap ? 64u : 0u) | \
+                     (((p).search_bits & ICP_SEARCH_ORIGIN_CACHE) ? 128u : 0u) | (((p).search_bits & ICP_SEARCH_ORIGIN_COUNT) ? 256u : 0u))
 #define KS_ARGS p.M, p.R, p.st, (const double *) p.mom, p.m, p.nr, p.side, icp_tpr_magic (p.side), p.nb, KS_FLAGS (p), p
 #define KS_CHAIN_ARGS p.M, p.R, p.cst + p.slot, (const double *) p.mom + (size_t) p.slot * ICP_NMOM * p.nb, p.m, p.nr, p.side, icp_tpr_magic (p.side), p.nb, KS_FLAGS (p), p
 #define KS_OWNER_ARGS p.F, p.R, p.st, (const double *) p.mom, p.m, p.nr, p.side, icp_tpr_magic (p.side), p.nb, 0u, p
diff --git a/include/icp_amd.h b/include/icp_amd.h
--- a/include/icp_amd.h
+++ b/include/icp_amd.h
@@ -102,6 +102,8 @@
 int icp_run_stats (icp_handle h, uint32_t *launches, uint32_t *k, uint32_t *dead_launches);
 
 int icp_launch_stats (icp_handle h, double *max_us, uint64_t *slower_than_10us, uint64_t *total, int reset);
+
+int icp_origin_cache_stats (icp_handle h, uint64_t *fills, uint64_t *fallbacks, int reset);
 
 typedef enum { ICP_OUTPUTS_LAZY = 0, ICP_OUTPUTS_EVERY_ITERATION = 1 } icp_output_mode;
 int icp_set_output_mode (icp_handle h, int mode);
```

Result: no change. 117,000, median of 3 (+0.1%).
